# Rorisis/Co-Occ

Measured on AMD Instinct MI355X. Metric: samples/sec (6-cam frame + sweep -> occ+render), 200x200x16 grid, higher is better.
Workload: dtype f32 (split-f16 products, fp32 accumulate)

## Files before the change

### co_occ_amd/_lib.py

```python
import ctypes
import os
import threading
import time

import torch

_HERE = os.path.dirname(os.path.abspath(__file__))
LIB_PATH = os.path.join(_HERE, "libcoocc_hip.so")

c_int, c_float, c_void_p, c_size_t, c_int64 = (ctypes.c_int, ctypes.c_float, ctypes.c_void_p,
                                               ctypes.c_size_t, ctypes.c_int64)


class ConvDesc(ctypes.Structure):
    _fields_ = [(n, c_void_p) for n in ("in_", "w", "out", "scale", "bias", "res", "gather", "out_rows", "ws")] + \
               [("ws_floats", c_int64)] + \
               [(n, c_int) for n in ("M", "Cin", "Cout", "taps", "in_stride", "out_stride", "res_stride",
                                     "B", "Xi", "Yi", "Zi", "Xo", "Yo", "Zo", "ksize", "stride", "pad",
                                     "relu", "res_mode", "splitk", "tile_hint", "kx", "ky", "kz", "px", "py", "pz",
                                     "wgroup_rows", "mfma_dtype")] + [("alpha", ctypes.c_float), ("M_dev", c_void_p), ("gather_stride", c_int), ("out16", c_void_p), ("out16_stride", c_int), ("out_h2", c_int),
                                                                   ("out_h2_twin", c_void_p), ("tile_sem", c_void_p), ("tile_sem_ints", c_int),
                                                                  ("alpha_dev", c_void_p), ("sx", c_int), ("sy", c_int), ("sz", c_int)]


class SearchDesc(ctypes.Structure):
    _fields_ = [("cat4", c_void_p), ("pts", c_void_p), ("pts_rows", c_int), ("pts_stride", c_int)] + \
               [(n, c_int) for n in ("C", "X", "Y", "Z", "K", "fps_num", "max_cluster")] + \
               [("radius", ctypes.c_float), ("dist_thresh", ctypes.c_float), ("offsets", c_void_p), ("noff", c_int)] + \
               [(n, c_void_p) for n in ("lin", "counts", "near_img", "near_pts", "rows", "rows_p", "ws")] + \
               [("ws_bytes", ctypes.c_size_t), ("counts_host", c_void_p)]


P, I, F, Z, L = c_void_p, c_int, c_float, c_size_t, c_int64
SIGNATURES = {
    "coocc_last_error": (ctypes.c_char_p, []),
    "coocc_abi_version": (I, []),
    "coocc_device_cu_count": (I, [P]),
    "coocc_stream_create_cu_mask": (I, [P, I, P]),
    "coocc_stream_destroy": (I, [P]),
    "coocc_event_create": (I, [I, P]),
    "coocc_event_destroy": (I, [P]),
    "coocc_event_record": (I, [P, P]),
    "coocc_stream_wait_event": (I, [P, P]),
    "coocc_event_synchronize": (I, [P]),
    "coocc_event_query": (I, [P]),
    "coocc_event_elapsed_ms": (I, [P, P, P]),
    "coocc_ncdhw_to_ndhwc": (I, [P, P, I, I, I, I, I, P]),
    "coocc_rows_to_bf16": (I, [P, I, L, I, P, P]),
    "coocc_rows_to_h2": (I, [P, I, L, I, F, P, P]),
    "coocc_rows_to_h2_ex": (I, [P, I, L, I, F, P, P, P]),
    "coocc_rows_to_h2_gather": (I, [P, I, P, L, P, I, F, P, P]),
    "coocc_rows_to_f16": (I, [P, I, L, I, P, P]),
    "coocc_wino_input_h2": (I, [P, I, I, I, I, I, I, I, P, I, L, F, P]),
    "coocc_wino_input_h2_ex": (I, [P, I, I, I, I, I, I, I, P, I, L, F, P, P]),
    "coocc_ndhwc_to_ncdhw": (I, [P, P, I, I, I, I, I, P]),
    "coocc_fuser_prepare": (I, [P, P, P, P, P, I, I, I, P]),
    "coocc_fuser_prepare_rows": (I, [P, I, I, P, I, I, P, P, P, I, I, I, P]),
    "coocc_compact_flags": (I, [P, I, P, P, P, Z, P]),
    "coocc_compact_flags_ex": (I, [P, I, P, P, P, P, Z, P]),
    "coocc_lin_to_coords": (I, [P, I, I, I, I, P, P, P]),
    "coocc_furthest_point_sampling": (I, [I, I, I, P, P, P, P]),
    "coocc_fps_voxels_ws": (Z, [I, I, I]),
    "coocc_fps_voxels": (I, [P, I, I, I, I, I, P, P, Z, P]),
    "coocc_fps_voxels_pair": (I, [P, I, P, P, P, I, P, P, Z, I, I, I, I, P]),
    "coocc_ball_query": (I, [I, I, I, F, F, I, P, P, P, P]),
    "coocc_knn_topk": (I, [I, I, I, P, P, P, P, P]),
    "coocc_voxel_index_map": (I, [P, I, I, P, P]),
    "coocc_voxel_index_map_dev": (I, [P, I, P, I, P, P]),
    "coocc_fine_sample_voxel_dev": (I, [P, I, I, I, I, P, I, P, I, P, P, P, I, P]),
    "coocc_fine_sample_img_dev": (I, [P, I, I, I, I, P, P, L, P, P, I, I, P]),
    "coocc_fine_mlp_pre_dev": (I, [P, I, P, I, L, P, I, P, P, P, F, P, P, P, P, F, P, P, I, P, P]),
    "coocc_fine_fused": (I, [P, I, I, I, P, I, I, I, P, P, I, P, I, P, P, P, P, F, P, P, P, P, F, P, P, I, P, P, P]),
    "coocc_fine2_pack": (I, [P, P, I, P, P, P, P, P, P, P, P, P, P]),
    "coocc_fine2_h2": (I, [P, I, I, I, I, P, I, I, I, P, P, I, P, P, P, P, F, F, I, P, P, P, P]),
    "coocc_fine_sample_img_lin": (I, [P, I, I, I, I, P, P, I, I, I, P, P, I, I, P]),
    "coocc_scatter_fine_dev": (I, [P, L, P, I, I, I, P, P, I, I, I, F, P]),
    "coocc_scatter_fine_grouped": (I, [P, I, I, P, I, P, I, I, I, I, P, F, P, P]),
    "coocc_ball_query_voxels": (I, [I, F, F, I, I, I, I, P, P, P, P, P]),
    "coocc_knn_topk_voxels": (I, [I, I, I, I, I, I, P, P, P, P, I, P, P, P, P, P]),
    "coocc_knn_assign": (I, [I, I, I, I, F, P, P, P, P, P, P]),
    "coocc_knn_threshold": (I, [I, F, P, P, P, P]),
    "coocc_index_rows_i32": (I, [P, I, P, I, P, P]),
    "coocc_conv_pack_weights": (L, [P, I, I, I, I, P]),
    "coocc_conv_fwd": (I, [ctypes.POINTER(ConvDesc), P]),
    "coocc_fuser_search_ws": (Z, [ctypes.POINTER(SearchDesc)]),
    "coocc_fuser_search": (I, [ctypes.POINTER(SearchDesc), P, P]),
    "coocc_upsample_add_trilinear": (I, [P, P, I, I, I, I, I, I, I, I, P]),
    "coocc_upsample_add_trilinear_ex": (I, [P, P, I, I, I, I, I, I, I, I, P, P]),
    "coocc_occhead_mix": (I, [P, P, I, P, P, I, I, P]),
    "coocc_occhead_mix_ex": (I, [P, P, I, P, P, I, I, P, P]),
    "coocc_argmax_flags": (I, [P, I, I, I, I, P, P]),
    "coocc_fine_sample_voxel": (I, [P, I, I, I, I, P, I, I, P, P, P, I, P]),
    "coocc_fine_sample_img": (I, [P, I, I, I, I, P, P, L, P, I, I, P]),
    "coocc_fine_mlp_pre": (I, [P, I, P, I, L, P, P, P, F, P, P, P, P, F, P, P, I, P, P]),
    "coocc_fine_mlp": (I, [P, I, P, I, L, P, P, P, P, F, P, P, P, P, F, P, P, I, P, P]),
    "coocc_groupnorm_rows": (I, [P, L, I, I, I, P, P, F, I, P]),
    "coocc_groupnorm_nhwc": (I, [P, I, I, I, I, P, P, F, I, P]),
    "coocc_scatter_fine": (I, [P, L, I, I, P, P, I, I, I, F, P]),
    "coocc_camera_mats": (I, [P, P, P, P, P, P, I, I, I, I, P, P]),
    "coocc_get_geometry": (I, [P, P, P, P, I, I, I, I, P, P]),
    "coocc_bev_pool_forward": (I, [P, P, P, P, I, I, I, I, I, I, I, P, P]),
    "coocc_bev_pool_backward": (I, [P, P, P, P, I, I, I, I, I, I, I, P, P]),
    "coocc_voxel_pool_ws": (Z, [I, I]),
    "coocc_voxel_pool": (I, [P, P, I, I, I, P, I, I, I, I, P, I, P, Z, I, P]),
    "coocc_lift_splat": (I, [P, P, P, I, I, I, I, I, I, P, I, I, I, I, P, I, P, Z, I, P]),
    "coocc_lift_splat_cams": (I, [P, P, P, P, P, P, I, I, I, I, I, I, P, I, I, I, I, P, I, P, Z, I, P]),
    "coocc_lift_splat_reuse": (I, [P, P, I, I, I, I, I, I, I, I, I, P, I, P, Z, P]),
    "coocc_bev_pool_coords": (I, [P, P, I, I, I, I, I, I, P, I, P, Z, I, P]),
    "coocc_render_nearest": (I, [P, I, I, I, P, P, I, I, I, I, P, I, P, P]),
    "coocc_render_nearest_cams": (I, [P, I, I, I, P, P, P, P, P, I, I, I, I, P, I, P, P]),
    "coocc_render_activate_table": (I, [P, I, P]),
    "coocc_upsample_maps": (I, [P, I, I, I, I, P, P, P]),
    "coocc_volume_sampling": (I, [P, I, I, I, I, P, I, P, P, P, P]),
    "coocc_raw2outputs": (I, [P, P, I, I, I, F, F, P, P, P, P]),
    "coocc_render_losses": (I, [P, P, P, P, L, I, P, P, Z, P]),
    "coocc_conv_pack_weights_dev": (L, [P, I, I, I, I, P, P]),
    "coocc_wino_pack_weights_dev": (L, [P, I, I, I, I, P, P]),
    "coocc_wino_pack_weights_h2_dev": (L, [P, I, I, I, I, P, P]),
    "coocc_conv_pack_weights_h2_dev": (L, [P, I, I, I, I, P, P]),
    "coocc_wino_gradout": (I, [P, I, I, I, I, I, I, I, P, L, P]),
    "coocc_wino_ztap_table": (I, [L, I, P, P]),
    "coocc_wino_wgrad": (I, [P, P, L, I, I, I, I, P, P, I, P, L, P]),
    "coocc_rows_to_kh2": (I, [P, I, L, L, I, F, P, P, P]),
    "coocc_wino_operand_kh2": (I, [I, P, I, I, I, I, I, I, I, P, L, F, P, P]),
    "coocc_conv_wgrad_h2": (I, [P, P, L, I, I, F, P, P, I, P, L, P]),
    "coocc_wino_wgrad_h2": (I, [P, P, L, I, I, I, I, F, P, P, I, P, L, P]),
    "coocc_conv_tap_table": (I, [I, I, I, I, I, I, I, I, I, I, I, P, P]),
    "coocc_conv_epilogue_bwd": (I, [P, I, P, I, P, I, I, I, P, I, P, I, I, P, I, P, L, P]),
    "coocc_conv_epilogue_bwd_ex": (I, [P, I, P, I, P, I, I, I, P, I, P, I, I, P, I, P, L, P, P, F, P]),
    "coocc_conv_wgrad": (I, [P, I, I, P, I, P, I, I, I, I, P, I, P, L, P]),
    "coocc_conv_wgrad_h2t": (I, [P, I, I, P, I, P, I, I, I, I, P, P, I, P, L, P]),
    "coocc_gather_rows": (I, [P, I, P, I, I, P, I, P]),
    "coocc_scatter_add_rows": (I, [P, I, P, I, I, P, I, P]),
    "coocc_voxel_pool_bwd": (I, [P, I, P, I, I, I, P, I, I, I, I, P, P]),
    "coocc_lift_splat_bwd": (I, [P, I, P, P, P, I, I, I, I, I, I, P, I, I, I, I, P, P, P]),
    "coocc_render_nearest_bwd": (I, [P, I, I, I, P, P, I, I, I, I, P, P, P, P]),
    "coocc_upsample_maps_bwd": (I, [P, P, I, I, I, I, P, P]),
    "coocc_render_losses_bwd": (I, [P, P, P, P, L, I, P, P, P, P, P]),
    "coocc_upsample_trilinear_bwd": (I, [P, P, I, I, I, I, I, I, I, I, I, P]),
    "coocc_wino_input": (I, [P, I, I, I, I, I, I, I, P, L, P]),
    "coocc_wino_input_strided": (I, [P, I, I, I, I, I, I, I, P, I, L, P]),
    "coocc_sparse_tap_sum": (I, [P, P, I, I, I, I, I, P, P, I, I, P]),
    "coocc_wino_output": (I, [P, L, I, I, I, I, I, I, P, I, P, P, P, I, I, P]),
    "coocc_wino_output_ex": (I, [P, L, I, I, I, I, I, I, P, I, P, P, P, I, I, P, P]),
    "coocc_h2_overflow": (I, [I]),
    "coocc_device_fault": (I, [I]),
    "coocc_render_heads_h2": (I, [P, I, I, I, P, P, P, P, P, P, I, P, P, P, I, P]),
    "coocc_head_pred_h2": (I, [P, I, I, P, P, P, P, P, I, I, P, P, I, P, I, I, P, P]),
    "coocc_head_soft_h2": (I, [P, I, I, P, P, P, P, P, I, P, P, I, P, I, P]),
    "coocc_projection_params": (I, [P, P, P, P, P, P, I, P, P, P]),
    "coocc_occhead_mix_bwd": (I, [P, P, I, P, P, P, P, I, I, P]),
    "coocc_fine_sample_voxel_bwd": (I, [P, I, I, I, I, I, P, L, P, P, P]),
    "coocc_groupnorm_rows_bwd": (I, [P, P, P, L, I, I, I, P, F, I, P, P, P, P]),
    "coocc_fine_sample_img_bwd": (I, [P, I, I, I, I, I, P, P, L, P, P]),
    "coocc_groupnorm_nhwc_bwd": (I, [P, P, P, I, I, I, I, P, F, I, P, P, P, P]),
    "coocc_voxelize_ws": (Z, [I]),
    "coocc_voxelize_hard": (I, [P, I, I, P, P, I, I, P, P, P, P, P, Z, P]),
    "coocc_vfe_mean": (I, [P, P, I, I, I, I, P, I, P]),
    "coocc_sparse_index_map": (I, [P, I, I, I, I, P, P]),
    "coocc_sparse_conv_table": (I, [P, I, I, I, I, I, I, I, P, P, P]),
    "coocc_sparse_down_flags": (I, [P, I, I, I, I, I, I, I, P, P]),
    "coocc_sparse_conv_table3": (I, [P, I, I, I, I, I, I, I, I, I, I, I, I, I, P, P, P]),
    "coocc_sparse_down_flags3": (I, [P, I, I, I, I, I, I, I, I, I, I, I, I, I, I, I, I, P, P]),
    "coocc_sparse_lin_to_coors": (I, [P, I, I, I, I, P, P, P]),
    "coocc_bn_stats": (I, [P, I, I, I, P, P, P, Z, P]),
    "coocc_bn_apply": (I, [P, I, I, P, P, P, P, F, P, I, P, P]),
    "coocc_bn_backward": (I, [P, P, P, I, I, P, P, P, F, I, P, P, P, P, P, Z, P]),
    "coocc_bn_backward_sums": (I, [P, P, P, I, I, P, P, F, I, P, P, P, Z, P]),
    "coocc_bn_backward_dx": (I, [P, P, P, I, I, P, P, P, F, I, P, P, ctypes.c_double, P, P, P]),
    "coocc_predict_labels": (I, [P, L, L, L, L, I, I, I, I, I, I, I, P, P]),
    "coocc_eval_semantic": (I, [P, L, L, L, L, I, I, I, I, P, P, I, I, I, I, I, P, P]),
    "coocc_fpn_sum": (I, [P, P, I, I, I, I, I, I, P, I, P, P]),
    "coocc_zyx_to_rows": (I, [P, P, I, I, I, I, I, I, I, P]),
    "coocc_conv_tap_table3": (I, [I] * 17 + [P, P]),
    "coocc_fpn_sum_bwd": (I, [P, I, P, P, I, I, I, I, I, I, P]),
    "coocc_lidarseg_points": (I, [P, L, L, L, L, I, I, I, I, P, L, L, I, I, P, I, I, P, P, I, P, P]),
    "coocc_render_eval_stats": (L, [P, P, P, P, I, I, I, P, P, Z, P]),
    "coocc_render_panels": (I, [P, P, P, P, I, I, I, P, P]),
    "coocc_render_eval_ssim": (L, [P, P, I, I, I, ctypes.c_double, P, P, Z, P]),
    "coocc_sparse_dgrad_table3": (I, [P] + [I] * 16 + [P, P, P, P]),
    "coocc_bn_apply_ex": (I, [P, I, I, P, P, P, P, F, P, I, P, P, P]),
    "coocc_pool_labels": (I, [P, I, I, I, I, I, I, I, P, P]),
    "coocc_occ_loss_ws": (Z, [L, I]),
    "coocc_occ_loss_fwd": (I, [P, L, I, I, P, P, I, I, I, P, P, I, P, P, P, P, Z, P]),
    "coocc_occ_loss_bwd": (I, [P, L, I, I, P, P, I, P, P, P, P, I, P]),
    "coocc_depth_labels": (I, [P, I, I, I, I, F, F, I, P, P, P]),
    "coocc_depth_bce_ws": (Z, [L, I]),
    "coocc_depth_bce": (I, [P, P, I, I, I, I, F, P, P, P, Z, P]),
    "coocc_depth_bce_bwd": (I, [P, P, I, I, I, I, F, P, P, P, P]),
    "coocc_nbr_table2d": (I, [I, I, I, I, P, P]),
    "coocc_dcn_cols": (I, [P, I, P, I, I, I, I, I, I, I, I, P, P]),
    "coocc_se_gate2": (I, [P, I, I, I, I, P, P, P, P, P]),
    "coocc_cam_mean_ws": (Z, [I, I, I]),
    "coocc_cam_mean": (I, [P, I, I, I, I, P, P, Z, P]),
    "coocc_cam_bias_relu": (I, [P, I, I, I, I, P, I, P]),
    "coocc_dcn_cols_bwd": (I, [P, I, P, I, I, I, I, I, I, I, I, P, P, P, P]),
    "coocc_se_gate2_bwd_ws": (Z, [I, I, I]),
    "coocc_se_gate2_bwd": (I, [P, I, I, I, I, P, P, P, P, P, P, P, P, Z, P]),
    "coocc_cam_sum": (I, [P, I, I, I, I, P, P, Z, P]),
    "coocc_cam_add": (I, [P, P, I, I, I, P, F, P]),
    "coocc_dropout_rows": (I, [P, P, L, I, F, P, P]),
    "coocc_img_stem": (I, [P, I, I, I, P, P, P, I, I, I, P, I, P, P]),
    "coocc_maxpool2d_rows": (I, [P, I, I, I, I, I, P, I, P, P]),
    "coocc_maxpool2d_rows_bwd": (I, [P, I, P, I, I, I, I, I, P, I, P]),
    "coocc_img_stem_wgrad_ws": (Z, [I, I, I]),
    "coocc_img_stem_wgrad": (I, [P, I, I, I, P, I, I, P, P, Z, P]),
    "coocc_optim_chunk": (I, []),
    "coocc_optim_sumsq": (I, [P, P, I, P, I, P, P]),
    "coocc_optim_clip_coef": (I, [P, I, F, P, P, P, P]),
    "coocc_optim_adamw": (I, [P, P, I, P, I, P, I, P]),
    "coocc_optim_scale": (I, [P, P, I, P, I, P, P]),
    "coocc_optim_pack": (I, [P, P, I, P, I, P, L, I, P]),
    "coocc_optim_unpack": (I, [P, P, I, P, I, P, L, P]),
    "coocc_optim_flag_check": (I, [P, I, P, I, P, P]),
    "coocc_frames_to_imgs": (I, [P, P, I, I, I, P, P, P, L, I, I, P, P, P]),
    "coocc_points_to_depth_maps": (I, [P, L, I, P, I, I, I, P, P]),
    "coocc_occ_scatter_labels": (I, [P, L, I, I, I, I, P, P, P]),
    "coocc_occ_rows_to_voxels": (I, [P, L, P, P, I, I, I, P, P, P, P]),
    "coocc_occ_points_to_voxels": (I, [P, L, I, P, P, P, P, I, I, I, I, P, P, P, P]),
    "coocc_occ_vote_ws": (Z, [L]),
    "coocc_occ_vote_labels": (I, [P, P, L, L, I, I, P, P, Z, P]),
    "coocc_occ_visible_rows": (I, [P, L, P, I, I, I, P, P, P]),
    "coocc_occ_cloud_aabb": (I, [P, L, I, P, P, P, P]),
    "coocc_sweeps_merge_ws": (Z, [L]),
    "coocc_sweeps_merge": (I, [P, L, I, P, P, I, P, I, F, P, L, P, P, Z, P]),
}

_lib = None


class KernelTimer:

    def __init__(self):
        self.enabled = False
        self.only = None
        self.records = []

    class _Region:
        def __init__(self, owner, tag, work):
            self.o, self.tag, self.work = owner, tag, work

        def __enter__(self):
            lvl = int(self.o.enabled)
            self.on = lvl >= 2 or (lvl == 1 and self.work > 0 and (self.o.only is None or self.tag.startswith(self.o.only)))
            if self.on:
                self.s = torch.cuda.Event(enable_timing=True)
                self.e = torch.cuda.Event(enable_timing=True)
                self.s.record()
            return self

        def __exit__(self, *a):
            if self.on:
                self.e.record()
                self.o.records.append((self.tag, self.work, self.s, self.e))
            return False

    def region(self, tag, work=0.0):
        return KernelTimer._Region(self, tag, work)

    def summary(self):
        out = {}
        for tag, work, s, e in self.records:
            d = out.setdefault(tag, dict(launches=0, ms=0.0, work=0.0))
            d["launches"] += 1
            d["ms"] += s.elapsed_time(e)
            d["work"] += work
        return out

    def reset(self):
        self.records = []


TIMER = KernelTimer()



def load():
    global _lib
    if _lib is not None:
        return _lib
    if not os.path.exists(LIB_PATH):
        raise ImportError(
            "co_occ_amd: %s is missing -- build it with `python -c 'import __graft_entry__ as g; g.build()'` "
            "(hipcc --offload-arch=gfx950).  There is no CPU fallback." % LIB_PATH)
    lib = ctypes.CDLL(LIB_PATH)
    for name, (res, args) in SIGNATURES.items():
        fn = getattr(lib, name)
        fn.restype, fn.argtypes = res, args
    if os.environ.get("COOCC_FPS_THREADS"):
        lib.coocc_fps_voxels_set_threads(int(os.environ["COOCC_FPS_THREADS"]))
    _lib = lib
    return lib


class CooccError(RuntimeError):
    code = None


class CooccArgError(CooccError):
    """COOCC_EINVAL / COOCC_ENOMEM: the library REFUSED the call (an argument or shape an entry point does not take, a
    workspace that is too small) before launching anything -- nothing ran, the caller may take another route."""


class CooccRangeError(CooccError):
    """The split-f16 engine's range guard fired (``core.check_h2_overflow``): kernels ran and their result is not trustworthy.
    Never a reason to fall back silently."""


def check(rc):
    if rc != 0:
        cls = CooccArgError if rc in (-1, -3) else CooccError
        e = cls("libcoocc_hip: %s (code %d)" % (load().coocc_last_error().decode(), rc))
        e.code = rc
        raise e


def _device_of(args):
    for a in args:
        t = getattr(a, "_keep", None)
        if t is not None:
            return t.device
    return None


_fns = {}


def call(name, *args):
    fn = _fns.get(name)
    if fn is None:
        fn = _fns[name] = getattr(load(), name)
    dev = _device_of(args)
    if dev is not None and dev.index != torch.cuda.current_device():
        with torch.cuda.device(dev):
            with TIMER.region(name):
                check(fn(*args, stream(dev)))
        return
    if not TIMER.enabled:
        rc = fn(*args, stream(dev))
        if rc:
            check(rc)
        return
    with TIMER.region(name):
        check(fn(*args, stream(dev)))


def conv_fwd(desc, device):
    fn = load().coocc_conv_fwd
    if device.index != torch.cuda.current_device():
        with torch.cuda.device(device):
            check(fn(ctypes.byref(desc), stream(device)))
    else:
        check(fn(ctypes.byref(desc), stream(device)))


_raw_stream = getattr(torch._C, "_cuda_getCurrentRawStream", None)


def stream(device=None):
    if _raw_stream is not None:
        idx = device.index if device is not None and device.index is not None else torch.cuda.current_device()
        return c_void_p(_raw_stream(idx))
    return c_void_p(torch.cuda.current_stream(device).cuda_stream)


class DevPtr(ctypes.c_void_p):
    """c_void_p that keeps its tensor alive until the foreign call has been issued, so that
    temporaries such as ``ptr(x.contiguous())`` cannot be recycled by the caching allocator
    while later arguments of the same call are still being built."""


def require_gpu(what, name=None):
    if isinstance(what, torch.Tensor):
        if not what.is_cuda:
            raise CooccError("co_occ_amd ops run on the GPU only; %s a %s tensor (no CPU fallback)" % ("%s is" % name if name else "got", what.device))
    elif torch.device(what).type != "cuda":
        raise CooccError("co_occ_amd ops run on the GPU only; got device %s (no CPU fallback)" % (what,))


def ptr(t, dtype=None, strided=False, offset=0):
    if t is None:
        return c_void_p(0)
    if not t.is_cuda:
        require_gpu(t)
    if dtype is not None and t.dtype != dtype:
        raise CooccError("expected %s, got %s" % (dtype, t.dtype))
    if not strided and not t.is_contiguous():
        raise CooccError("tensor must be contiguous")
    p = DevPtr(t.data_ptr() + offset * t.element_size())
    p._keep = t
    return p


_blocked = threading.local()


def host_read(t):
    t0 = time.perf_counter()
    v = t.tolist()
    _blocked.s = getattr(_blocked, "s", 0.0) + time.perf_counter() - t0
    return v


def blocked_seconds():
    return getattr(_blocked, "s", 0.0)


def host_f32(vals):
    return (c_float * len(vals))(*[float(v) for v in vals])


def host_i32(vals):
    return (c_int * len(vals))(*[int(v) for v in vals])
```

### co_occ_amd/csrc/knn.hip

```cpp
#include "common.h"

typedef unsigned long long u64;

__device__ __forceinline__ u64 shfl_xor_u64(u64 v, int m) {
  unsigned lo = (unsigned)v, hi = (unsigned)(v >> 32);
  lo = __shfl_xor(lo, m);
  hi = __shfl_xor(hi, m);
  return ((u64)hi << 32) | lo;
}
template <int CTRL>
__device__ __forceinline__ u64 dpp_u64(u64 v) {
  int lo = (int)(unsigned)v, hi = (int)(unsigned)(v >> 32);
  lo = __builtin_amdgcn_update_dpp(lo, lo, CTRL, 0xF, 0xF, false);
  hi = __builtin_amdgcn_update_dpp(hi, hi, CTRL, 0xF, 0xF, false);
  return ((u64)(unsigned)hi << 32) | (unsigned)lo;
}
__device__ __forceinline__ u64 readlane_u64(u64 v, int l) {
  unsigned lo = __builtin_amdgcn_readlane((int)(unsigned)v, l);
  unsigned hi = __builtin_amdgcn_readlane((int)(unsigned)(v >> 32), l);
  return ((u64)hi << 32) | lo;
}
#define U64MAX(a, b) ((a) > (b) ? (a) : (b))
#define U64MIN(a, b) ((a) < (b) ? (a) : (b))
__device__ __forceinline__ u64 wave_max_u64(u64 v) {
  u64 o;
  o = dpp_u64<0xB1>(v); v = U64MAX(v, o);
  o = dpp_u64<0x4E>(v); v = U64MAX(v, o);
  o = dpp_u64<0x141>(v); v = U64MAX(v, o);
  o = dpp_u64<0x140>(v); v = U64MAX(v, o);
  u64 a = readlane_u64(v, 0), b = readlane_u64(v, 16), c = readlane_u64(v, 32), d = readlane_u64(v, 48);
  a = U64MAX(a, b); c = U64MAX(c, d);
  return U64MAX(a, c);
}
__device__ __forceinline__ u64 wave_min_u64(u64 v) {
  u64 o;
  o = dpp_u64<0xB1>(v); v = U64MIN(v, o);
  o = dpp_u64<0x4E>(v); v = U64MIN(v, o);
  o = dpp_u64<0x141>(v); v = U64MIN(v, o);
  o = dpp_u64<0x140>(v); v = U64MIN(v, o);
  u64 a = readlane_u64(v, 0), b = readlane_u64(v, 16), c = readlane_u64(v, 32), d = readlane_u64(v, 48);
  a = U64MIN(a, b); c = U64MIN(c, d);
  return U64MIN(a, c);
}

#define FPS_THREADS 1024
#define FPS_KBITS 22

__device__ __forceinline__ unsigned fps_tiebreak(int k, int L, unsigned blockmask) {
  unsigned r = L ? (__brev((unsigned)k & blockmask) >> (32 - L)) : 0u;
  return (r << FPS_KBITS) | (unsigned)k;
}

template <int PPT>
__global__ __launch_bounds__(FPS_THREADS) void k_fps_f32(int n, int m, const float* __restrict__ pts_all,
                                                          float* __restrict__ temp_all,
                                                          int32_t* __restrict__ idx_all, int L) {
  __shared__ u64 wbest[2][FPS_THREADS / 64];
  const int tid = threadIdx.x;
  const float* pts = pts_all + (size_t)blockIdx.x * n * 3;
  float* temp = temp_all + (size_t)blockIdx.x * n;
  int32_t* idx = idx_all + (size_t)blockIdx.x * m;
  const unsigned blockmask = (1u << L) - 1u;

  float px[PPT], py[PPT], pz[PPT], pt[PPT];
  unsigned ntb[PPT];
#pragma unroll
  for (int i = 0; i < PPT; ++i) {
    int k = tid + i * FPS_THREADS;
    bool v = k < n;
    px[i] = v ? pts[k * 3 + 0] : 0.f;
    py[i] = v ? pts[k * 3 + 1] : 0.f;
    pz[i] = v ? pts[k * 3 + 2] : 0.f;
    pt[i] = v ? 1e10f : 0.f;
    ntb[i] = v ? ~fps_tiebreak(k, L, blockmask) : 0u;
  }
  for (int k = tid + PPT * FPS_THREADS; k < n; k += FPS_THREADS) temp[k] = 1e10f;

  int old = 0;
  if (tid == 0) idx[0] = 0;
  for (int j = 1; j < m; ++j) {
    const float x1 = pts[old * 3 + 0], y1 = pts[old * 3 + 1], z1 = pts[old * 3 + 2];
    u64 best = 0;
#pragma unroll
    for (int i = 0; i < PPT; ++i) {
      float d = sqdist3(x1, y1, z1, px[i], py[i], pz[i]);
      float t = fminf(d, pt[i]);
      pt[i] = t;
      u64 key = ((u64)__float_as_uint(t) << 32) | (u64)ntb[i];
      best = key > best ? key : best;
    }
#pragma unroll 2
    for (int k = tid + PPT * FPS_THREADS; k < n; k += FPS_THREADS) {
      float d = sqdist3(x1, y1, z1, pts[k * 3 + 0], pts[k * 3 + 1], pts[k * 3 + 2]);
      float t = fminf(d, temp[k]);
      temp[k] = t;
      u64 key = ((u64)__float_as_uint(t) << 32) | (u64)(~fps_tiebreak(k, L, blockmask));
      best = key > best ? key : best;
    }
    best = wave_max_u64(best);
    if ((tid & 63) == 0) wbest[j & 1][tid >> 6] = best;
    __syncthreads();
    u64 b = wbest[j & 1][tid & 15];
#pragma unroll
    for (int mm = 8; mm > 0; mm >>= 1) {
      u64 o = shfl_xor_u64(b, mm);
      b = o > b ? o : b;
    }
    old = (int)((~(unsigned)b) & ((1u << FPS_KBITS) - 1u));
    if (tid == 0) idx[j] = old;
  }
}

extern "C" int coocc_furthest_point_sampling(int b, int n, int m, const float* points, float* temp,
                                             int32_t* idx, void* stream) {
  COOCC_CHECK_ARG(points && temp && idx && b > 0 && n > 0 && m >= 0, "fps: bad args");
  COOCC_CHECK_ARG(n < (1 << FPS_KBITS), "fps: n must be < 2^22");
  if (m == 0) return COOCC_OK;
  int L = 0;
  while ((2 << L) <= n && L < 10) ++L;
  if (n <= 8 * FPS_THREADS)
    hipLaunchKernelGGL(k_fps_f32<8>, dim3(b), dim3(FPS_THREADS), 0, as_stream(stream), n, m, points, temp, idx, L);
  else
    hipLaunchKernelGGL(k_fps_f32<10>, dim3(b), dim3(FPS_THREADS), 0, as_stream(stream), n, m, points, temp, idx, L);
  COOCC_LAUNCH_CHECK("k_fps_f32");
  return COOCC_OK;
}

#define FT_X 4
#define FT_Y 4
#define FT_Z 8
#define FT_P 128

struct FpsCell { int temp; int r; };

__global__ __launch_bounds__(256) void k_fpsv_scatter(const int32_t* __restrict__ lin, int n, int Y, int Z, int NBY,
                                                       int NBZ, int L, int q, int tinit, FpsCell* __restrict__ cell) {
  int k = blockIdx.x * blockDim.x + threadIdx.x;
  if (k >= n) return;
  int l = lin[k];
  int z = l % Z; l /= Z;
  int y = l % Y; int x = l / Y;
  int b = ((x / FT_X) * NBY + y / FT_Y) * NBZ + z / FT_Z;
  int p = ((x % FT_X) * FT_Y + (y % FT_Y)) * FT_Z + (z % FT_Z);
  unsigned rev = L ? (__brev((unsigned)k & ((1u << L) - 1u)) >> (32 - L)) : 0u;
  cell[(size_t)b * FT_P + p] = FpsCell{tinit, (int)(rev * (unsigned)q + ((unsigned)k >> L))};
}

__device__ __forceinline__ void lds_barrier() { asm volatile("s_waitcnt lgkmcnt(0)\n\ts_barrier" ::: "memory"); }

template <int CTRL>
__device__ __forceinline__ unsigned dpp_u32(unsigned v) {
  return (unsigned)__builtin_amdgcn_update_dpp((int)v, (int)v, CTRL, 0xF, 0xF, false);
}
__device__ __forceinline__ unsigned wave_max_key(unsigned v) {
  v = max(v, dpp_u32<0xB1>(v));
  v = max(v, dpp_u32<0x4E>(v));
  v = max(v, dpp_u32<0x141>(v));
  v = max(v, dpp_u32<0x140>(v));
  unsigned a = __builtin_amdgcn_readlane((int)v, 0), b = __builtin_amdgcn_readlane((int)v, 16);
  unsigned c = __builtin_amdgcn_readlane((int)v, 32), d = __builtin_amdgcn_readlane((int)v, 48);
  return max(max(a, b), max(c, d));
}
__device__ __forceinline__ u64 wave_max_key(u64 v) { return wave_max_u64(v); }
__device__ __forceinline__ unsigned row_max_key(unsigned v) {
  v = max(v, dpp_u32<0xB1>(v));
  v = max(v, dpp_u32<0x4E>(v));
  v = max(v, dpp_u32<0x141>(v));
  v = max(v, dpp_u32<0x140>(v));
  return v;
}
__device__ __forceinline__ u64 row_max_key(u64 v) {
  u64 o;
  o = dpp_u64<0xB1>(v); v = U64MAX(v, o);
  o = dpp_u64<0x4E>(v); v = U64MAX(v, o);
  o = dpp_u64<0x141>(v); v = U64MAX(v, o);
  o = dpp_u64<0x140>(v); v = U64MAX(v, o);
  return v;
}
__device__ __forceinline__ unsigned first_lane_key(unsigned v) { return (unsigned)__builtin_amdgcn_readfirstlane((int)v); }
__device__ __forceinline__ u64 first_lane_key(u64 v) {
  return ((u64)(unsigned)__builtin_amdgcn_readfirstlane((int)(v >> 32)) << 32) | (unsigned)__builtin_amdgcn_readfirstlane((int)(unsigned)v);
}

template <int THREADS, int FPS_RMAX, typename KT>
__global__ __launch_bounds__(THREADS) void k_fps_voxels(int n, int m, int Y, int Z, int NBY, int NBZ, int NB,
                                                         const int32_t* __restrict__ lin, FpsCell* __restrict__ cell,
                                                         int32_t* __restrict__ idx, int L, int q, int RB, long long* dbg) {
  constexpr int NW = THREADS / 64;
  __builtin_amdgcn_s_setprio(3);
  __shared__ KT wbest[2][NW];
  __shared__ int wloc[2][NW];
  const int tid = threadIdx.x, lane = tid & 63, wave = tid >> 6;
  const KT rmask = (KT)(((KT)1 << RB) - 1);
  const int tmax = sizeof(KT) == 4 ? (int)((1u << (32 - RB)) - 1u) : 0x7FFFFFFF;
  long long tA = 0, tM = 0, tB = 0, tT = 0, nd = 0;

  KT key[FPS_RMAX];
  int org[FPS_RMAX];
  int pos[FPS_RMAX];
#pragma unroll
  for (int r = 0; r < FPS_RMAX; ++r) {
    const int b = (lane + 64 * r) * NW + wave;
    key[r] = 0; pos[r] = 0; org[r] = 0;
    if (b < NB) {
      int bz = b % NBZ; int qq = b / NBZ;
      org[r] = ((qq / NBY) * FT_X) | (((qq % NBY) * FT_Y) << 10) | ((bz * FT_Z) << 20);
    }
  }
#pragma unroll
  for (int r = 0; r < FPS_RMAX; ++r) {
    for (int src = 0; src < 64; ++src) {
      const int b = (src + 64 * r) * NW + wave;
      if (b >= NB) break;
      KT best = 0;
      int bp = 0;
#pragma unroll
      for (int h = 0; h < 2; ++h) {
        int rr = cell[(size_t)b * FT_P + lane + 64 * h].r;
        KT kk = rr >= 0 ? (KT)(((KT)tmax << RB) | (rmask - (KT)rr)) : (KT)0;
        if (kk > best) { best = kk; bp = lane + 64 * h; }
      }
      KT wb = wave_max_key(best);
      u64 own = __ballot(best == wb);
      int wp = __builtin_amdgcn_readlane(bp, (int)__ffsll((long long)own) - 1);
      if (lane == src) { key[r] = wb; pos[r] = wp; }
    }
  }
  if (tid == 0) idx[0] = 0;
  int sx, sy, sz;
  {
    int l = lin[0];
    sz = l % Z; l /= Z;
    sy = l % Y; sx = l / Y;
  }

  auto refresh = [&](FpsCell* cp, const FpsCell& c0_, const FpsCell& c1_, int o, KT& best, int& bp) {
    const int x0 = o & 1023, y0 = (o >> 10) & 1023, z0 = o >> 20;
    best = 0; bp = 0;
#pragma unroll
    for (int h = 0; h < 2; ++h) {
      const FpsCell c = h ? c1_ : c0_;
      const int p = lane + 64 * h;
      if (c.r >= 0) {
        int ex = x0 + (p >> 5) - sx, ey = y0 + ((p >> 3) & 3) - sy, ez = z0 + (p & 7) - sz;
        int t = min(__mul24(ex, ex) + __mul24(ey, ey) + __mul24(ez, ez), c.temp);
        cp[p].temp = t;
        KT kk = (KT)(((KT)t << RB) | (rmask - (KT)c.r));
        if (kk > best) { best = kk; bp = p; }
      }
    }
  };

  for (int j = 1; j < m; ++j) {
    long long c0 = dbg ? clock64() : 0;
#pragma unroll
    for (int r = 0; r < FPS_RMAX; ++r) {
      if (r * 64 * NW >= NB) break;
      bool d = false;
      if (key[r]) {
        int x0 = org[r] & 1023, y0 = (org[r] >> 10) & 1023, z0 = org[r] >> 20;
        int dx = max(max(x0 - sx, sx - (x0 + FT_X - 1)), 0);
        int dy = max(max(y0 - sy, sy - (y0 + FT_Y - 1)), 0);
        int dz = max(max(z0 - sz, sz - (z0 + FT_Z - 1)), 0);
        d = (__mul24(dx, dx) + __mul24(dy, dy) + __mul24(dz, dz)) < (int)(key[r] >> RB);
      }
      u64 bal = __ballot(d);
      nd += __popcll(bal);
      while (bal) {
        const int s0 = (int)__ffsll((long long)bal) - 1;
        bal &= bal - 1;
        const bool two = bal != 0;
        const int s1 = two ? (int)__ffsll((long long)bal) - 1 : s0;
        bal &= bal - 1;
        FpsCell* cp0 = cell + (size_t)((s0 + 64 * r) * NW + wave) * FT_P;
        FpsCell* cp1 = cell + (size_t)((s1 + 64 * r) * NW + wave) * FT_P;
        const FpsCell a0 = cp0[lane], a1 = cp0[lane + 64];
        FpsCell b0 = a0, b1 = a1;
        if (two) { b0 = cp1[lane]; b1 = cp1[lane + 64]; }
        KT best0, best1 = 0;
        int bp0, bp1 = 0;
        refresh(cp0, a0, a1, __builtin_amdgcn_readlane(org[r], s0), best0, bp0);
        if (two) refresh(cp1, b0, b1, __builtin_amdgcn_readlane(org[r], s1), best1, bp1);
        const KT wb0 = wave_max_key(best0);
        const KT wb1 = two ? wave_max_key(best1) : (KT)0;
        const int wp0 = __builtin_amdgcn_readlane(bp0, (int)__ffsll((long long)__ballot(best0 == wb0)) - 1);
        if (lane == s0) { key[r] = wb0; pos[r] = wp0; }
        if (two) {
          const int wp1 = __builtin_amdgcn_readlane(bp1, (int)__ffsll((long long)__ballot(best1 == wb1)) - 1);
          if (lane == s1) { key[r] = wb1; pos[r] = wp1; }
        }
      }
    }
    long long c1 = dbg ? clock64() : 0;
    KT best = 0;
    int bo = 0, bpz = 0;
#pragma unroll
    for (int r = 0; r < FPS_RMAX; ++r) {
      if (key[r] > best) { best = key[r]; bo = org[r]; bpz = pos[r]; }
    }
    const int loc = bo + (bpz >> 5) + (((bpz >> 3) & 3) << 10) + ((bpz & 7) << 20);
    KT wb = wave_max_key(best);
    if (best == wb && wb) { wbest[j & 1][wave] = wb; wloc[j & 1][wave] = loc; }
    if (!wb && lane == 0) wbest[j & 1][wave] = 0;
    long long c2 = dbg ? clock64() : 0;
    lds_barrier();
    long long c3 = dbg ? clock64() : 0;
    KT g;
    int gl;
    if constexpr (NW <= 16) {
      const int li = lane & 15;
      const KT mine = li < NW ? wbest[j & 1][li] : (KT)0;
      const int ml = li < NW ? wloc[j & 1][li] : 0;
      g = first_lane_key(row_max_key(mine));
      const u64 own = __ballot(mine == g) & 0xFFFFull;
      gl = __builtin_amdgcn_readlane(ml, (int)__ffsll((long long)own) - 1);
    } else {
      g = wbest[j & 1][0];
      int gw = 0;
#pragma unroll
      for (int w = 1; w < NW; ++w) {
        KT o = wbest[j & 1][w];
        if (o > g) { g = o; gw = w; }
      }
      gl = wloc[j & 1][gw];
    }
    sx = gl & 1023; sy = (gl >> 10) & 1023; sz = gl >> 20;
    if (tid == 0) {
      const unsigned rr = (unsigned)(rmask - (g & rmask));
      const unsigned hi = rr / (unsigned)q, lo = rr - hi * (unsigned)q;
      const unsigned rev = L ? (__brev(hi) >> (32 - L)) : 0u;
      idx[j] = (int)((lo << L) | rev);
    }
    if (dbg) { long long c4 = clock64(); tA += c1 - c0; tM += c2 - c1; tB += c3 - c2; tT += c4 - c3; }
  }
  if (dbg && lane == 0) {
    long long* o = dbg + wave * 8;
    o[0] = tA; o[1] = tM; o[2] = tB; o[3] = tT; o[4] = 0; o[5] = nd;
  }
}

#define FPSR_SLOTS 40
struct FpsRegProblem { const int32_t* lin; const FpsCell* cell; int32_t* idx; int n, L, q, RB; };
struct FpsRegArgs { FpsRegProblem p[2]; int m, Y, Z, NBY, NBZ, NB; long long* dbg; };

__global__ __launch_bounds__(1024) void k_fps_voxels_reg(FpsRegArgs a) {
  constexpr int NW = 16;
  __builtin_amdgcn_s_setprio(3);
  __shared__ unsigned wbest[2][NW];
  __shared__ int wloc[2][NW];
  const FpsRegProblem pr = a.p[blockIdx.x];
  const int tid = threadIdx.x, lane = tid & 63, wave = __builtin_amdgcn_readfirstlane(tid >> 6);
  const int RB = pr.RB, Y = a.Y, Z = a.Z, NB = a.NB, m = a.m;
  const unsigned rmask = (1u << RB) - 1u;
  const unsigned tmax = (1u << (32 - RB)) - 1u;
  long long* dbg = a.dbg;
  long long tA = 0, tM = 0, tB = 0, tT = 0, nd = 0;

  typedef unsigned u32x32 __attribute__((ext_vector_type(32)));
  typedef unsigned u32x8 __attribute__((ext_vector_type(8)));
  u32x32 ca0, ca1;
  u32x8 cb0, cb1;
  unsigned key = 0;
  int org = 0, pos = 0;
  {
    const int b = lane * NW + wave;
    if (lane < FPSR_SLOTS && b < NB) {
      int bz = b % a.NBZ; int qq = b / a.NBZ;
      org = ((qq / a.NBY) * FT_X) | (((qq % a.NBY) * FT_Y) << 10) | ((bz * FT_Z) << 20);
    }
  }
#pragma unroll
  for (int i = 0; i < FPSR_SLOTS; ++i) {
    const int b = i * NW + wave;
    unsigned k0 = 0, k1 = 0;
    if (b < NB) {
      const int r0 = pr.cell[(size_t)b * FT_P + lane].r, r1 = pr.cell[(size_t)b * FT_P + lane + 64].r;
      k0 = r0 >= 0 ? ((tmax << RB) | (rmask - (unsigned)r0)) : 0u;
      k1 = r1 >= 0 ? ((tmax << RB) | (rmask - (unsigned)r1)) : 0u;
      const unsigned best = max(k0, k1);
      const int bp = k1 > k0 ? lane + 64 : lane;
      const unsigned wb = wave_max_key(best);
      const u64 own = __ballot(best == wb);
      const int wp = __builtin_amdgcn_readlane(bp, (int)__ffsll((long long)own) - 1);
      if (lane == i) { key = wb; pos = wp; }
    }
    if (i < 32) { ca0[i] = k0; ca1[i] = k1; }
    else { cb0[i - 32] = k0; cb1[i - 32] = k1; }
  }
  if (tid == 0) pr.idx[0] = 0;
  int sx, sy, sz;
  {
    int l = pr.lin[0];
    sz = l % Z; l /= Z;
    sy = l % Y; sx = l / Y;
  }

  for (int j = 1; j < m; ++j) {
    long long c0 = dbg ? clock64() : 0;
    bool d = false;
    if (key) {
      const int x0 = org & 1023, y0 = (org >> 10) & 1023, z0 = org >> 20;
      const int dx = max(max(x0 - sx, sx - (x0 + FT_X - 1)), 0);
      const int dy = max(max(y0 - sy, sy - (y0 + FT_Y - 1)), 0);
      const int dz = max(max(z0 - sz, sz - (z0 + FT_Z - 1)), 0);
      d = (unsigned)(__mul24(dx, dx) + __mul24(dy, dy) + __mul24(dz, dz)) < (key >> RB);
    }
    u64 bal = __ballot(d);
    nd += __popcll(bal);
    const int exb = (lane >> 5) - sx, eyb = ((lane >> 3) & 3) - sy, ezb = (lane & 7) - sz;
    while (bal) {
      const int s0 = __builtin_amdgcn_readfirstlane((int)__ffsll((long long)bal) - 1);
      bal &= bal - 1;
      const int o = __builtin_amdgcn_readlane(org, s0);
      const int ex = (o & 1023) + exb, ey = ((o >> 10) & 1023) + eyb, ez = (o >> 20) + ezb;
      const int yz = __mul24(ey, ey) + __mul24(ez, ez);
      const unsigned d0 = (unsigned)(__mul24(ex, ex) + yz), d1 = (unsigned)(__mul24(ex + 2, ex + 2) + yz);
      unsigned k0, k1;
      if (s0 < 32) { k0 = ca0[s0]; k1 = ca1[s0]; }
      else { k0 = cb0[s0 - 32]; k1 = cb1[s0 - 32]; }
      if (k0) k0 = (min(d0, k0 >> RB) << RB) | (k0 & rmask);
      if (k1) k1 = (min(d1, k1 >> RB) << RB) | (k1 & rmask);
      if (s0 < 32) { ca0[s0] = k0; ca1[s0] = k1; }
      else { cb0[s0 - 32] = k0; cb1[s0 - 32] = k1; }
      const unsigned best = max(k0, k1);
      const int bp = k1 > k0 ? lane + 64 : lane;
      const unsigned wb = wave_max_key(best);
      const int wp = __builtin_amdgcn_readlane(bp, (int)__ffsll((long long)__ballot(best == wb)) - 1);
      if (lane == s0) { key = wb; pos = wp; }
    }
    long long c1 = dbg ? clock64() : 0;
    const int loc = org + (pos >> 5) + (((pos >> 3) & 3) << 10) + ((pos & 7) << 20);
    const unsigned wb = wave_max_key(key);
    if (key == wb && wb) { wbest[j & 1][wave] = wb; wloc[j & 1][wave] = loc; }
    if (!wb && lane == 0) wbest[j & 1][wave] = 0;
    long long c2 = dbg ? clock64() : 0;
    lds_barrier();
    long long c3 = dbg ? clock64() : 0;
    const int li = lane & 15;
    const unsigned mine = wbest[j & 1][li];
    const int ml = wloc[j & 1][li];
    unsigned v = mine;
    v = max(v, dpp_u32<0xB1>(v));
    v = max(v, dpp_u32<0x4E>(v));
    v = max(v, dpp_u32<0x141>(v));
    v = max(v, dpp_u32<0x140>(v));
    const unsigned g = (unsigned)__builtin_amdgcn_readfirstlane((int)v);
    const u64 own = __ballot(mine == g) & 0xFFFFull;
    const int gl = __builtin_amdgcn_readlane(ml, (int)__ffsll((long long)own) - 1);
    sx = gl & 1023; sy = (gl >> 10) & 1023; sz = gl >> 20;
    if (tid == 0) pr.idx[j] = (int)(g & rmask);
    if (dbg) { long long c4 = clock64(); tA += c1 - c0; tM += c2 - c1; tB += c3 - c2; tT += c4 - c3; }
  }
  __syncthreads();
  for (int j = 1 + tid; j < m; j += 1024) {
    const unsigned rr = rmask - (unsigned)pr.idx[j];
    const unsigned hi = rr / (unsigned)pr.q, lo = rr - hi * (unsigned)pr.q;
    const unsigned rev = pr.L ? (__brev(hi) >> (32 - pr.L)) : 0u;
    pr.idx[j] = (int)((lo << pr.L) | rev);
  }
  if (dbg && lane == 0 && blockIdx.x == 0) {
    long long* o = dbg + wave * 8;
    o[0] = tA; o[1] = tM; o[2] = tB; o[3] = tT; o[4] = 0; o[5] = nd;
  }
}

extern "C" size_t coocc_fps_voxels_ws(int X, int Y, int Z) {
  size_t nb = (size_t)((X + FT_X - 1) / FT_X) * ((Y + FT_Y - 1) / FT_Y) * ((Z + FT_Z - 1) / FT_Z);
  return nb * FT_P * sizeof(FpsCell);
}

static int g_fps_threads = 1024;
static long long* g_fps_dbg = nullptr;
extern "C" void coocc_fps_voxels_set_debug(long long* p) { g_fps_dbg = p; }
extern "C" void coocc_fps_voxels_set_threads(int t) { g_fps_threads = t; }

struct FpsPrep { int NBX, NBY, NBZ, L, q, RB, tinit, threads, R; long long NB; bool key32; };

static int fps_prepare(const int32_t* lin, int n, int X, int Y, int Z, int m, const int32_t* idx, void* ws, size_t ws_bytes,
                       hipStream_t s, FpsPrep* o) {
  COOCC_CHECK_ARG(lin && idx && ws && n > 0 && m >= 0 && X > 0 && Y > 0 && Z > 0, "fps_voxels: bad args");
  COOCC_CHECK_ARG(n < (1 << FPS_KBITS), "fps_voxels: n must be < 2^22");
  COOCC_CHECK_ARG(X <= 1020 && Y <= 1020 && Z <= 1016, "fps_voxels: grid dims must fit 10-bit packed coordinates");
  o->NBX = (X + FT_X - 1) / FT_X; o->NBY = (Y + FT_Y - 1) / FT_Y; o->NBZ = (Z + FT_Z - 1) / FT_Z;
  o->NB = (long long)o->NBX * o->NBY * o->NBZ;
  int threads = g_fps_threads;
  while (o->NB > 8ll * threads && threads < 1024) threads *= 2;
  COOCC_CHECK_ARG(o->NB <= 8ll * threads, "fps_voxels: grid has too many buckets (use coocc_furthest_point_sampling)");
  if (ws_bytes < coocc_fps_voxels_ws(X, Y, Z)) return coocc_set_error(COOCC_ENOMEM, "fps_voxels: workspace too small");
  o->threads = threads;
  o->R = (int)((o->NB + threads - 1) / threads);
  int L = 0;
  while ((2 << L) <= n && L < 10) ++L;
  const int q = (n + (1 << L) - 1) >> L;
  int RB = L;
  while ((1ll << RB) <= ((long long)q << L)) ++RB;
  const long long d2max = (long long)(X - 1) * (X - 1) + (long long)(Y - 1) * (Y - 1) + (long long)(Z - 1) * (Z - 1);
  o->key32 = RB < 31 && d2max + 1 < (1ll << (32 - RB)) - 1;
  o->tinit = o->key32 ? (int)((1u << (32 - RB)) - 1u) : 0x7FFFFFFF;
  o->L = L; o->q = q; o->RB = RB;
  if (m == 0) return COOCC_OK;
  FpsCell* cell = (FpsCell*)ws;
  COOCC_HIP(hipMemsetAsync(cell, 0xFF, sizeof(FpsCell) * (size_t)o->NB * FT_P, s));
  hipLaunchKernelGGL(k_fpsv_scatter, dim3(cdiv(n, 256)), dim3(256), 0, s, lin, n, Y, Z, o->NBY, o->NBZ, L, q, o->tinit, cell);
  COOCC_LAUNCH_CHECK("k_fpsv_scatter");
  return COOCC_OK;
}

static int g_fps_reg = -1;
static bool fps_reg_ok(const FpsPrep& o) {
  if (g_fps_reg < 0) g_fps_reg = getenv("COOCC_FPS_REG") ? atoi(getenv("COOCC_FPS_REG")) : 1;
  return g_fps_reg && o.key32 && o.NB <= (long long)FPSR_SLOTS * 16;
}

extern "C" int coocc_fps_voxels(const int32_t* lin, int n, int X, int Y, int Z, int m, int32_t* idx, void* ws,
                                size_t ws_bytes, void* stream) {
  hipStream_t s = as_stream(stream);
  FpsPrep o;
  int rc = fps_prepare(lin, n, X, Y, Z, m, idx, ws, ws_bytes, s, &o);
  if (rc != COOCC_OK || m == 0) return rc;
  FpsCell* cell = (FpsCell*)ws;
  const int NBY = o.NBY, NBZ = o.NBZ, L = o.L, q = o.q, RB = o.RB, R = o.R, threads = o.threads;
  const long long NB = o.NB;
  const bool key32 = o.key32;
  if (fps_reg_ok(o)) {
    FpsRegArgs a = {};
    a.p[0] = FpsRegProblem{lin, cell, idx, n, L, q, RB};
    a.m = m; a.Y = Y; a.Z = Z; a.NBY = NBY; a.NBZ = NBZ; a.NB = (int)NB; a.dbg = g_fps_dbg;
    hipLaunchKernelGGL(k_fps_voxels_reg, dim3(1), dim3(1024), 0, s, a);
    COOCC_LAUNCH_CHECK("k_fps_voxels_reg");
    return COOCC_OK;
  }
#define FPS_LAUNCH(T, RM, KT) \
  hipLaunchKernelGGL((k_fps_voxels<T, RM, KT>), dim3(1), dim3(T), 0, s, n, m, Y, Z, NBY, NBZ, (int)NB, lin, cell, idx, L, q, \
                     key32 ? RB : 32, g_fps_dbg)
#define FPS_PICK_R(T, KT)                     \
  do {                                        \
    if (R <= 2) FPS_LAUNCH(T, 2, KT);         \
    else if (R <= 3) FPS_LAUNCH(T, 3, KT);    \
    else if (R <= 4) FPS_LAUNCH(T, 4, KT);    \
    else if (R <= 5) FPS_LAUNCH(T, 5, KT);    \
    else if (R <= 6) FPS_LAUNCH(T, 6, KT);    \
    else FPS_LAUNCH(T, 8, KT);                \
  } while (0)
#define FPS_PICK(T)                           \
  do {                                        \
    if (key32) FPS_PICK_R(T, unsigned);       \
    else FPS_PICK_R(T, u64);                  \
  } while (0)
  if (threads == 256) FPS_PICK(256);
  else if (threads == 512) FPS_PICK(512);
  else FPS_PICK(1024);
  COOCC_LAUNCH_CHECK("k_fps_voxels");
  return COOCC_OK;
}

extern "C" int coocc_fps_voxels_pair(const int32_t* lin0, int n0, int32_t* idx0, void* ws0, const int32_t* lin1, int n1, int32_t* idx1,
                                     void* ws1, size_t ws_bytes_each, int X, int Y, int Z, int m, void* stream) {
  COOCC_CHECK_ARG(X > 0 && Y > 0 && Z > 0 && n0 > 0 && n1 > 0, "fps_voxels_pair: bad args");
  {
    const long long NB = (long long)((X + FT_X - 1) / FT_X) * ((Y + FT_Y - 1) / FT_Y) * ((Z + FT_Z - 1) / FT_Z);
    if (NB > (long long)FPSR_SLOTS * 16) return 2;
    const long long d2max = (long long)(X - 1) * (X - 1) + (long long)(Y - 1) * (Y - 1) + (long long)(Z - 1) * (Z - 1);
    for (int n : {n0, n1}) {
      int L = 0;
      while ((2 << L) <= n && L < 10) ++L;
      const int q = (n + (1 << L) - 1) >> L;
      int RB = L;
      while ((1ll << RB) <= ((long long)q << L)) ++RB;
      if (!(RB < 31 && d2max + 1 < (1ll << (32 - RB)) - 1)) return 2;
    }
    if (g_fps_reg < 0) g_fps_reg = getenv("COOCC_FPS_REG") ? atoi(getenv("COOCC_FPS_REG")) : 1;
    if (!g_fps_reg) return 2;
  }
  hipStream_t s = as_stream(stream);
  FpsPrep o0, o1;
  int rc = fps_prepare(lin0, n0, X, Y, Z, m, idx0, ws0, ws_bytes_each, s, &o0);
  if (rc != COOCC_OK) return rc;
  rc = fps_prepare(lin1, n1, X, Y, Z, m, idx1, ws1, ws_bytes_each, s, &o1);
  if (rc != COOCC_OK || m == 0) return rc;
  FpsRegArgs a = {};
  a.p[0] = FpsRegProblem{lin0, (const FpsCell*)ws0, idx0, n0, o0.L, o0.q, o0.RB};
  a.p[1] = FpsRegProblem{lin1, (const FpsCell*)ws1, idx1, n1, o1.L, o1.q, o1.RB};
  a.m = m; a.Y = Y; a.Z = Z; a.NBY = o0.NBY; a.NBZ = o0.NBZ; a.NB = (int)o0.NB; a.dbg = g_fps_dbg;
  hipLaunchKernelGGL(k_fps_voxels_reg, dim3(2), dim3(1024), 0, s, a);
  COOCC_LAUNCH_CHECK("k_fps_voxels_reg");
  return COOCC_OK;
}

__global__ __launch_bounds__(256) void k_ball_query(int n, int m, float min_r2, float max_r2, int nsample,
                                                     const float* __restrict__ new_xyz_all,
                                                     const float* __restrict__ xyz_all,
                                                     int32_t* __restrict__ idx_all) {
  const int lane = threadIdx.x & 63;
  const int c = blockIdx.x * 4 + (threadIdx.x >> 6);
  if (c >= m) return;
  const float* new_xyz = new_xyz_all + ((size_t)blockIdx.y * m + c) * 3;
  const float* xyz = xyz_all + (size_t)blockIdx.y * n * 3;
  int32_t* idx = idx_all + ((size_t)blockIdx.y * m + c) * nsample;
  const float cx = new_xyz[0], cy = new_xyz[1], cz = new_xyz[2];
  int cnt = 0, first = 0;
  for (int base = 0; base < n && cnt < nsample; base += 64) {
    int k = base + lane;
    bool hit = false;
    if (k < n) {
      float d2 = sqdist3(xyz[k * 3 + 0], xyz[k * 3 + 1], xyz[k * 3 + 2], cx, cy, cz);
      hit = (d2 == 0.f) || (d2 >= min_r2 && d2 < max_r2);
    }
    u64 bal = __ballot(hit);
    if (bal) {
      if (cnt == 0) first = base + (int)__ffsll((long long)bal) - 1;
      int slot = cnt + __popcll(bal & ((1ull << lane) - 1ull));
      if (hit && slot < nsample) idx[slot] = k;
      cnt += __popcll(bal);
    }
  }
  if (cnt > nsample) cnt = nsample;
  for (int l = cnt + lane; l < nsample; l += 64) idx[l] = first;
}

extern "C" int coocc_ball_query(int b, int n, int m, float min_radius, float max_radius, int nsample,
                                const float* new_xyz, const float* xyz, int32_t* idx, void* stream) {
  COOCC_CHECK_ARG(new_xyz && xyz && idx && b > 0 && n > 0 && m > 0 && nsample > 0, "ball_query: bad args");
  dim3 grid(cdiv(m, 4), b);
  hipLaunchKernelGGL(k_ball_query, grid, dim3(256), 0, as_stream(stream), n, m, min_radius * min_radius,
                     max_radius * max_radius, nsample, new_xyz, xyz, idx);
  COOCC_LAUNCH_CHECK("k_ball_query");
  return COOCC_OK;
}

template <int K>
__global__ __launch_bounds__(256) void k_knn_topk(int nq, int nk, const float* __restrict__ q,
                                                   const float* __restrict__ key, float* __restrict__ val,
                                                   int32_t* __restrict__ idx) {
  const int lane = threadIdx.x & 63;
  const int r = blockIdx.x * 4 + (threadIdx.x >> 6);
  if (r >= nq) return;
  const float qx = q[r * 3 + 0], qy = q[r * 3 + 1], qz = q[r * 3 + 2];
  u64 best[K];
#pragma unroll
  for (int j = 0; j < K; ++j) best[j] = ~0ull;
  for (int k = lane; k < nk; k += 64) {
    float d2 = sqdist3(qx, qy, qz, key[k * 3 + 0], key[k * 3 + 1], key[k * 3 + 2]);
    u64 kk = ((u64)__float_as_uint(d2) << 32) | (unsigned)k;
    if (kk < best[K - 1]) {
      best[K - 1] = kk;
#pragma unroll
      for (int j = K - 1; j > 0; --j) {
        if (best[j] < best[j - 1]) { u64 t = best[j]; best[j] = best[j - 1]; best[j - 1] = t; }
      }
    }
  }
#pragma unroll
  for (int o = 0; o < K; ++o) {
    u64 mn = wave_min_u64(best[0]);
    if (best[0] == mn) {
#pragma unroll
      for (int j = 0; j < K - 1; ++j) best[j] = best[j + 1];
      best[K - 1] = ~0ull;
    }
    if (lane == 0) {
      val[(size_t)r * K + o] = (float)__dsqrt_rn((double)__uint_as_float((unsigned)(mn >> 32)));
      idx[(size_t)r * K + o] = (int32_t)(unsigned)mn;
    }
  }
}

extern "C" int coocc_knn_topk(int nq, int nk, int K, const float* q, const float* key, float* val,
                              int32_t* idx, void* stream) {
  COOCC_CHECK_ARG(q && key && val && idx && nq > 0 && nk > 0, "knn_topk: bad args");
  COOCC_CHECK_ARG(K >= 1 && K <= 8 && K <= nk, "knn_topk: need 1 <= K <= min(8, nk)");
  dim3 grid(cdiv(nq, 4)), block(256);
  hipStream_t s = as_stream(stream);
  switch (K) {
    case 1: hipLaunchKernelGGL(k_knn_topk<1>, grid, block, 0, s, nq, nk, q, key, val, idx); break;
    case 2: hipLaunchKernelGGL(k_knn_topk<2>, grid, block, 0, s, nq, nk, q, key, val, idx); break;
    case 3: hipLaunchKernelGGL(k_knn_topk<3>, grid, block, 0, s, nq, nk, q, key, val, idx); break;
    case 4: hipLaunchKernelGGL(k_knn_topk<4>, grid, block, 0, s, nq, nk, q, key, val, idx); break;
    case 5: hipLaunchKernelGGL(k_knn_topk<5>, grid, block, 0, s, nq, nk, q, key, val, idx); break;
    case 6: hipLaunchKernelGGL(k_knn_topk<6>, grid, block, 0, s, nq, nk, q, key, val, idx); break;
    case 7: hipLaunchKernelGGL(k_knn_topk<7>, grid, block, 0, s, nq, nk, q, key, val, idx); break;
    default: hipLaunchKernelGGL(k_knn_topk<8>, grid, block, 0, s, nq, nk, q, key, val, idx); break;
  }
  COOCC_LAUNCH_CHECK("k_knn_topk");
  return COOCC_OK;
}

__global__ __launch_bounds__(256) void k_index_map_scatter(const int32_t* __restrict__ lin, int n, int32_t* __restrict__ map,
                                                            const int32_t* __restrict__ n_dev) {
  if (n_dev) n = min(n, *n_dev);
  int i = blockIdx.x * blockDim.x + threadIdx.x;
  if (i < n) map[lin[i]] = i;
}

__global__ __launch_bounds__(256) void k_fill_i32(int32_t* __restrict__ p, int n, int32_t v) {
  const int i = blockIdx.x * blockDim.x + threadIdx.x;
  if (i < n) p[i] = v;
}

extern "C" int coocc_voxel_index_map_dev(const int32_t* lin, int n_cap, const int32_t* n_dev, int nvox, int32_t* map, void* stream) {
  COOCC_CHECK_ARG(map && nvox > 0 && n_cap > 0 && lin && n_dev, "voxel_index_map_dev: bad args");
  static const bool fill_kernel = !(getenv("COOCC_MAP_MEMSET") && atoi(getenv("COOCC_MAP_MEMSET")) == 1);
  if (fill_kernel) hipLaunchKernelGGL(k_fill_i32, dim3(cdiv(nvox, 256)), dim3(256), 0, as_stream(stream), map, nvox, -1);
  else COOCC_HIP(hipMemsetAsync(map, 0xFF, (size_t)nvox * 4, as_stream(stream)));
  hipLaunchKernelGGL(k_index_map_scatter, dim3(cdiv(n_cap, 256)), dim3(256), 0, as_stream(stream), lin, n_cap, map, n_dev);
  COOCC_LAUNCH_CHECK("k_index_map_scatter");
  return COOCC_OK;
}

extern "C" int coocc_voxel_index_map(const int32_t* lin, int n, int nvox, int32_t* map, void* stream) {
  COOCC_CHECK_ARG(map && nvox > 0 && n >= 0 && (lin || n == 0), "voxel_index_map: bad args");
  COOCC_HIP(hipMemsetAsync(map, 0xFF, (size_t)nvox * 4, as_stream(stream)));
  if (n) {
    hipLaunchKernelGGL(k_index_map_scatter, dim3(cdiv(n, 256)), dim3(256), 0, as_stream(stream), lin, n, map, (const int32_t*)nullptr);
    COOCC_LAUNCH_CHECK("k_index_map_scatter");
  }
  return COOCC_OK;
}

__global__ __launch_bounds__(256) void k_ball_query_vox(int m, float min_r2, float max_r2, int R, int nsample, int X, int Y, int Z,
                                                         const int32_t* __restrict__ centre_ord, const int32_t* __restrict__ lin_q,
                                                         const int32_t* __restrict__ map_q, int32_t* __restrict__ idx_all) {
  const int lane = threadIdx.x & 63;
  const int c = blockIdx.x * 4 + (threadIdx.x >> 6);
  if (c >= m) return;
  int32_t* idx = idx_all + (size_t)c * nsample;
  const int v0 = lin_q[centre_ord[c]];
  const int cz = v0 % Z, cy = (v0 / Z) % Y, cx = v0 / (Z * Y);
  const int x0 = max(cx - R, 0), x1 = min(cx + R, X - 1);
  const int y0 = max(cy - R, 0), y1 = min(cy + R, Y - 1);
  const int z0 = max(cz - R, 0), z1 = min(cz + R, Z - 1);
  const int wy = y1 - y0 + 1, wz = z1 - z0 + 1;
  const int total = (x1 - x0 + 1) * wy * wz;
  int cnt = 0, first = 0;
  for (int base = 0; base < total && cnt < nsample; base += 64) {
    const int t = base + lane;
    bool hit = false;
    int ord = -1;
    if (t < total) {
      const int iz = z0 + t % wz, r = t / wz;
      const int iy = y0 + r % wy, ix = x0 + r / wy;
      ord = map_q[(ix * Y + iy) * Z + iz];
      const float d2 = sqdist3((float)ix, (float)iy, (float)iz, (float)cx, (float)cy, (float)cz);
      hit = ord >= 0 && ((d2 == 0.f) || (d2 >= min_r2 && d2 < max_r2));
    }
    const u64 bal = __ballot(hit);
    if (bal) {
      if (cnt == 0) first = __shfl(ord, (int)__ffsll((long long)bal) - 1);
      const int slot = cnt + __popcll(bal & ((1ull << lane) - 1ull));
      if (hit && slot < nsample) idx[slot] = ord;
      cnt += __popcll(bal);
    }
  }
  if (cnt > nsample) cnt = nsample;
  for (int l = cnt + lane; l < nsample; l += 64) idx[l] = first;
}

extern "C" int coocc_ball_query_voxels(int m, float min_radius, float max_radius, int nsample, int X, int Y, int Z,
                                       const int32_t* centre_ord, const int32_t* lin_q, const int32_t* map_q, int32_t* idx,
                                       void* stream) {
  COOCC_CHECK_ARG(m > 0 && nsample > 0 && X > 0 && Y > 0 && Z > 0 && centre_ord && lin_q && map_q && idx, "ball_query_voxels: bad args");
  COOCC_CHECK_ARG(max_radius >= 0.f && max_radius < 4096.f, "ball_query_voxels: bad radius");
  const float max_r2 = max_radius * max_radius;
  int R = (int)ceilf(max_radius);
  while (R > 0 && (float)(R * R) >= max_r2) --R;
  hipLaunchKernelGGL(k_ball_query_vox, dim3(cdiv(m, 4)), dim3(256), 0, as_stream(stream), m, min_radius * min_radius, max_r2, R,
                     nsample, X, Y, Z, centre_ord, lin_q, map_q, idx);
  COOCC_LAUNCH_CHECK("k_ball_query_vox");
  return COOCC_OK;
}

template <int K>
__global__ __launch_bounds__(256) void k_knn_topk_vox(int nq, int X, int Y, int Z, const int32_t* __restrict__ rep_ord,
                                                       const int32_t* __restrict__ lin_q, const int32_t* __restrict__ map_k,
                                                       const uint32_t* __restrict__ offsets, int noff, float* __restrict__ val,
                                                       int32_t* __restrict__ idx) {
  const int lane = threadIdx.x & 63;
  const int r = blockIdx.x * 4 + (threadIdx.x >> 6);
  if (r >= nq) return;
  const int v0 = lin_q[rep_ord[r]];
  const int cz = v0 % Z, cy = (v0 / Z) % Y, cx = v0 / (Z * Y);
  int found = 0;
  for (int base = 0; base < noff && found < K; base += 64) {
    const int t = base + lane;
    int ord = -1;
    float d2 = 0.f;
    if (t < noff) {
      const uint32_t o = offsets[t];
      const int dx = (int)(o & 255u) - 128, dy = (int)((o >> 8) & 255u) - 128, dz = (int)((o >> 16) & 255u) - 128;
      const int ix = cx + dx, iy = cy + dy, iz = cz + dz;
      if ((unsigned)ix < (unsigned)X && (unsigned)iy < (unsigned)Y && (unsigned)iz < (unsigned)Z) {
        ord = map_k[(ix * Y + iy) * Z + iz];
        d2 = sqdist3((float)cx, (float)cy, (float)cz, (float)ix, (float)iy, (float)iz);
      }
    }
    const u64 bal = __ballot(ord >= 0);
    const int p = found + __popcll(bal & ((1ull << lane) - 1ull));
    if (ord >= 0 && p < K) {
      val[(size_t)r * K + p] = (float)__dsqrt_rn((double)d2);
      idx[(size_t)r * K + p] = ord;
    }
    found += __popcll(bal);
  }
  if (found < K && lane == 0) idx[(size_t)r * K] = -2;
}

template <int K>
__global__ __launch_bounds__(256) void k_knn_topk_unresolved(int nq, int nk, const float* __restrict__ q,
                                                              const float* __restrict__ key, float* __restrict__ val,
                                                              int32_t* __restrict__ idx) {
  const int lane = threadIdx.x & 63;
  const int r = blockIdx.x * 4 + (threadIdx.x >> 6);
  if (r >= nq || idx[(size_t)r * K] != -2) return;
  const float qx = q[r * 3 + 0], qy = q[r * 3 + 1], qz = q[r * 3 + 2];
  u64 best[K];
#pragma unroll
  for (int j = 0; j < K; ++j) best[j] = ~0ull;
  for (int k = lane; k < nk; k += 64) {
    float d2 = sqdist3(qx, qy, qz, key[k * 3 + 0], key[k * 3 + 1], key[k * 3 + 2]);
    u64 kk = ((u64)__float_as_uint(d2) << 32) | (unsigned)k;
    if (kk < best[K - 1]) {
      best[K - 1] = kk;
#pragma unroll
      for (int j = K - 1; j > 0; --j) {
        if (best[j] < best[j - 1]) { u64 t = best[j]; best[j] = best[j - 1]; best[j - 1] = t; }
      }
    }
  }
#pragma unroll
  for (int o = 0; o < K; ++o) {
    u64 mn = wave_min_u64(best[0]);
    if (best[0] == mn) {
#pragma unroll
      for (int j = 0; j < K - 1; ++j) best[j] = best[j + 1];
      best[K - 1] = ~0ull;
    }
    if (lane == 0) {
      val[(size_t)r * K + o] = (float)__dsqrt_rn((double)__uint_as_float((unsigned)(mn >> 32)));
      idx[(size_t)r * K + o] = (int32_t)(unsigned)mn;
    }
  }
}

template <int K>
static void launch_topk_vox(int nq, int nk, int X, int Y, int Z, const int32_t* rep_ord, const int32_t* lin_q, const int32_t* map_k,
                            const uint32_t* offsets, int noff, const float* q, const float* key, float* val, int32_t* idx,
                            hipStream_t s) {
  hipLaunchKernelGGL(k_knn_topk_vox<K>, dim3(cdiv(nq, 4)), dim3(256), 0, s, nq, X, Y, Z, rep_ord, lin_q, map_k, offsets, noff, val, idx);
  hipLaunchKernelGGL(k_knn_topk_unresolved<K>, dim3(cdiv(nq, 4)), dim3(256), 0, s, nq, nk, q, key, val, idx);
}

extern "C" int coocc_knn_topk_voxels(int nq, int nk, int K, int X, int Y, int Z, const int32_t* rep_ord, const int32_t* lin_q,
                                     const int32_t* map_k, const uint32_t* offsets, int noff, const float* q, const float* key,
                                     float* val, int32_t* idx, void* stream) {
  COOCC_CHECK_ARG(nq > 0 && nk > 0 && X > 0 && Y > 0 && Z > 0 && rep_ord && lin_q && map_k && offsets && noff > 0 && q && key &&
                      val && idx, "knn_topk_voxels: bad args");
  COOCC_CHECK_ARG(K >= 1 && K <= 8 && K <= nk, "knn_topk_voxels: need 1 <= K <= min(8, nk)");
  hipStream_t s = as_stream(stream);
  switch (K) {
    case 1: launch_topk_vox<1>(nq, nk, X, Y, Z, rep_ord, lin_q, map_k, offsets, noff, q, key, val, idx, s); break;
    case 2: launch_topk_vox<2>(nq, nk, X, Y, Z, rep_ord, lin_q, map_k, offsets, noff, q, key, val, idx, s); break;
    case 3: launch_topk_vox<3>(nq, nk, X, Y, Z, rep_ord, lin_q, map_k, offsets, noff, q, key, val, idx, s); break;
    case 4: launch_topk_vox<4>(nq, nk, X, Y, Z, rep_ord, lin_q, map_k, offsets, noff, q, key, val, idx, s); break;
    case 5: launch_topk_vox<5>(nq, nk, X, Y, Z, rep_ord, lin_q, map_k, offsets, noff, q, key, val, idx, s); break;
    case 6: launch_topk_vox<6>(nq, nk, X, Y, Z, rep_ord, lin_q, map_k, offsets, noff, q, key, val, idx, s); break;
    case 7: launch_topk_vox<7>(nq, nk, X, Y, Z, rep_ord, lin_q, map_k, offsets, noff, q, key, val, idx, s); break;
    default: launch_topk_vox<8>(nq, nk, X, Y, Z, rep_ord, lin_q, map_k, offsets, noff, q, key, val, idx, s); break;
  }
  COOCC_LAUNCH_CHECK("k_knn_topk_vox");
  return COOCC_OK;
}

__global__ void k_assign_winner(int nc, int K, int ns, int nq, float thresh, const float* __restrict__ val,
                                const int32_t* __restrict__ group, int32_t* __restrict__ winner) {
  int i = blockIdx.x * blockDim.x + threadIdx.x;
  if (i >= nc * ns) return;
  int c = i / ns;
  int qi = group[i];
  if (i != c * ns && qi == group[c * ns]) return;
  for (int k = 0; k < K; ++k)
    if (val[c * K + k] < thresh) atomicMax(&winner[(size_t)k * nq + qi], c);
}

__global__ void k_assign_lookup(int K, int nq, const int32_t* __restrict__ nn,
                                const int32_t* __restrict__ winner, int32_t* __restrict__ out) {
  int i = blockIdx.x * blockDim.x + threadIdx.x;
  if (i >= K * nq) return;
  int k = i / nq;
  int w = winner[i];
  out[i] = w >= 0 ? nn[w * K + k] : -1;
}

extern "C" int coocc_knn_assign(int nc, int K, int ns, int nq, float dist_thresh, const float* val,
                                const int32_t* nn, const int32_t* group, int32_t* winner, int32_t* out,
                                void* stream) {
  COOCC_CHECK_ARG(val && nn && group && winner && out && nc > 0 && K > 0 && ns > 0 && nq > 0, "knn_assign: bad args");
  hipStream_t s = as_stream(stream);
  COOCC_HIP(hipMemsetAsync(winner, 0xFF, sizeof(int32_t) * (size_t)K * nq, s));
  hipLaunchKernelGGL(k_assign_winner, dim3(cdiv((long long)nc * ns, 256)), dim3(256), 0, s, nc, K, ns, nq,
                     dist_thresh, val, group, winner);
  hipLaunchKernelGGL(k_assign_lookup, dim3(cdiv((long long)K * nq, 256)), dim3(256), 0, s, K, nq, nn, winner, out);
  COOCC_LAUNCH_CHECK("knn_assign");
  return COOCC_OK;
}

__global__ void k_knn_threshold(int nq, float thresh, const float* __restrict__ val,
                                const int32_t* __restrict__ nn, int32_t* __restrict__ out) {
  int i = blockIdx.x * blockDim.x + threadIdx.x;
  if (i < nq) out[i] = val[i] < thresh ? nn[i] : -1;
}

extern "C" int coocc_knn_threshold(int nq, float dist_thresh, const float* val, const int32_t* nn,
                                   int32_t* out, void* stream) {
  COOCC_CHECK_ARG(val && nn && out && nq > 0, "knn_threshold: bad args");
  hipLaunchKernelGGL(k_knn_threshold, dim3(cdiv(nq, 256)), dim3(256), 0, as_stream(stream), nq, dist_thresh, val, nn, out);
  COOCC_LAUNCH_CHECK("k_knn_threshold");
  return COOCC_OK;
}

__global__ void k_index_rows(const int32_t* __restrict__ base, int nbase, const int32_t* __restrict__ sel, int n,
                             int32_t* __restrict__ rows) {
  int i = blockIdx.x * blockDim.x + threadIdx.x;
  if (i >= n) return;
  int s = sel[i];
  if (s < 0) s += nbase;
  rows[i] = (s >= 0 && s < nbase) ? base[s] : -1;
}

extern "C" int coocc_index_rows_i32(const int32_t* base, int nbase, const int32_t* sel, int n, int32_t* rows,
                                    void* stream) {
  COOCC_CHECK_ARG(base && sel && rows && nbase > 0 && n >= 0, "index_rows: bad args");
  if (n == 0) return COOCC_OK;
  hipLaunchKernelGGL(k_index_rows, dim3(cdiv(n, 256)), dim3(256), 0, as_stream(stream), base, nbase, sel, n, rows);
  COOCC_LAUNCH_CHECK("k_index_rows");
  return COOCC_OK;
}
```

### co_occ_amd/csrc/layout.hip

```cpp
#include <stdarg.h>
#include <stdlib.h>

#include "common.h"

typedef float f32x4 __attribute__((ext_vector_type(4)));

static thread_local char g_err[512] = "";

int coocc_set_error(int code, const char* fmt, ...) {
  va_list ap;
  va_start(ap, fmt);
  vsnprintf(g_err, sizeof(g_err), fmt, ap);
  va_end(ap);
  return code;
}

extern "C" const char* coocc_last_error(void) { return g_err; }
extern "C" int coocc_abi_version(void) { return 1; }

#define TV 64
#define TC 128

__global__ __launch_bounds__(256) void k_ncdhw_to_ndhwc(const float* __restrict__ src,
                                                         float* __restrict__ dst, int C, int V,
                                                         int dst_stride, int dst_coff) {
  __shared__ float tile[TV][TC + 1];
  const int b = blockIdx.y;
  const int v0 = blockIdx.x * TV;
  const int t = threadIdx.x;
  const int c0 = blockIdx.z * TC;
  const int cn = min(TC, C - c0);
  if (cn == TC) {
    const int v = v0 + (t & 63);
    const float* sp = src + ((size_t)b * C + c0 + (t >> 6)) * V + v;
    float r[TC / 4];
#pragma unroll
    for (int k = 0; k < TC / 4; ++k) r[k] = v < V ? sp[(size_t)(4 * k) * V] : 0.f;
#pragma unroll
    for (int k = 0; k < TC / 4; ++k) tile[t & 63][(t >> 6) + 4 * k] = r[k];
    __syncthreads();
#pragma unroll 8
    for (int i = t; i < TV * TC; i += 256) {
      const int vv = i >> 7, c = i & (TC - 1);
      if (v0 + vv < V) dst[((size_t)b * V + v0 + vv) * dst_stride + dst_coff + c0 + c] = tile[vv][c];
    }
    return;
  }
  for (int c = t >> 6; c < cn; c += 4) {
    int v = v0 + (t & 63);
    tile[t & 63][c] = v < V ? src[((size_t)b * C + c0 + c) * V + v] : 0.f;
  }
  __syncthreads();
  for (int i = t; i < TV * cn; i += 256) {
    int v = i / cn, c = i - v * cn;
    if (v0 + v < V) dst[((size_t)b * V + v0 + v) * dst_stride + dst_coff + c0 + c] = tile[v][c];
  }
}

__global__ __launch_bounds__(256) void k_ndhwc_to_ncdhw(const float* __restrict__ src,
                                                         float* __restrict__ dst, int C, int V,
                                                         int src_stride, int src_coff) {
  __shared__ float tile[TV][TC + 1];
  const int b = blockIdx.y;
  const int v0 = blockIdx.x * TV;
  const int t = threadIdx.x;
  for (int c0 = 0; c0 < C; c0 += TC) {
    const int cn = min(TC, C - c0);
    for (int i = t; i < TV * cn; i += 256) {
      int v = i / cn, c = i - v * cn;
      tile[v][c] = (v0 + v < V) ? src[((size_t)b * V + v0 + v) * src_stride + src_coff + c0 + c] : 0.f;
    }
    __syncthreads();
    for (int c = t >> 6; c < cn; c += 4) {
      int v = v0 + (t & 63);
      if (v < V) dst[((size_t)b * C + c0 + c) * V + v] = tile[t & 63][c];
    }
    __syncthreads();
  }
}

extern "C" int coocc_ncdhw_to_ndhwc(const float* src, float* dst, int B, int C, int V, int dst_stride,
                                    int dst_coff, void* stream) {
  COOCC_CHECK_ARG(src && dst && B > 0 && C > 0 && V > 0 && dst_stride >= dst_coff + C, "ncdhw_to_ndhwc: bad args");
  dim3 grid(cdiv(V, TV), B, cdiv(C, TC));
  hipLaunchKernelGGL(k_ncdhw_to_ndhwc, grid, dim3(256), 0, as_stream(stream), src, dst, C, V, dst_stride, dst_coff);
  COOCC_LAUNCH_CHECK("k_ncdhw_to_ndhwc");
  return COOCC_OK;
}

extern "C" int coocc_ndhwc_to_ncdhw(const float* src, float* dst, int B, int C, int V, int src_stride,
                                    int src_coff, void* stream) {
  COOCC_CHECK_ARG(src && dst && B > 0 && C > 0 && V > 0 && src_stride >= src_coff + C, "ndhwc_to_ncdhw: bad args");
  dim3 grid(cdiv(V, TV), B);
  hipLaunchKernelGGL(k_ndhwc_to_ncdhw, grid, dim3(256), 0, as_stream(stream), src, dst, C, V, src_stride, src_coff);
  COOCC_LAUNCH_CHECK("k_ndhwc_to_ncdhw");
  return COOCC_OK;
}

__global__ __launch_bounds__(256) void k_fuser_prepare(const float* __restrict__ img,
                                                        const float* __restrict__ pts,
                                                        float* __restrict__ cat4,
                                                        uint8_t* __restrict__ flag_img,
                                                        uint8_t* __restrict__ flag_pts, int C, int V) {
  __shared__ float tile[TV][TC + 1];
  const int b = blockIdx.y;
  const int v0 = blockIdx.x * TV;
  const int t = threadIdx.x;
  const int stride = 4 * C;
  for (int mod = 0; mod < 2; ++mod) {
    const float* src = mod ? pts : img;
    uint8_t* flags = mod ? flag_pts : flag_img;
    float rsum = 0.f;
    for (int c0 = 0; c0 < C; c0 += TC) {
      const int cn = min(TC, C - c0);
      for (int c = t >> 6; c < cn; c += 4) {
        int v = v0 + (t & 63);
        tile[t & 63][c] = v < V ? src[((size_t)b * C + c0 + c) * V + v] : 0.f;
      }
      __syncthreads();
      if (t < TV)
        for (int c = 0; c < cn; ++c) rsum += tile[t][c];
      for (int i = t; i < TV * cn; i += 256) {
        int v = i / cn, c = i - v * cn;
        if (v0 + v < V) cat4[((size_t)b * V + v0 + v) * stride + mod * C + c0 + c] = tile[v][c];
      }
      __syncthreads();
    }
    if (t < TV && v0 + t < V) flags[(size_t)b * V + v0 + t] = rsum != 0.f ? 1 : 0;
  }
  for (int i = t; i < TV * 2 * C; i += 256) {
    int v = i / (2 * C), c = i - v * 2 * C;
    if (v0 + v < V) cat4[((size_t)b * V + v0 + v) * stride + 2 * C + c] = 0.f;
  }
}

extern "C" int coocc_fuser_prepare(const float* img, const float* pts, float* cat4, uint8_t* flag_img,
                                   uint8_t* flag_pts, int B, int C, int V, void* stream) {
  COOCC_CHECK_ARG(img && pts && cat4 && flag_img && flag_pts && B > 0 && C > 0 && V > 0, "fuser_prepare: bad args");
  dim3 grid(cdiv(V, TV), B);
  hipLaunchKernelGGL(k_fuser_prepare, grid, dim3(256), 0, as_stream(stream), img, pts, cat4, flag_img, flag_pts, C, V);
  COOCC_LAUNCH_CHECK("k_fuser_prepare");
  return COOCC_OK;
}

__global__ __launch_bounds__(256) void k_fuser_prepare_rows(const float* __restrict__ img, int img_rows, int img_stride,
                                                             const float* __restrict__ pts, int pts_rows, int pts_stride,
                                                             float* __restrict__ cat4, uint8_t* __restrict__ flag_img,
                                                             uint8_t* __restrict__ flag_pts, int C, int V) {
  __shared__ float tile[TV][TC + 1];
  const int b = blockIdx.y;
  const int v0 = blockIdx.x * TV;
  const int t = threadIdx.x;
  const int stride = 4 * C;
  for (int mod = 0; mod < 2; ++mod) {
    const float* src = mod ? pts : img;
    const int rows = mod ? pts_rows : img_rows, sstride = mod ? pts_stride : img_stride;
    uint8_t* flags = mod ? flag_pts : flag_img;
    const bool in_place = rows && src == cat4 + mod * C && sstride == stride;
    float rsum = 0.f;
    for (int c0 = 0; c0 < C; c0 += TC) {
      const int cn = min(TC, C - c0);
      if (rows) {
        if (cn == TC) {
          for (int i = t; i < TV * (TC / 4); i += 256) {
            const int v = i / (TC / 4), c = (i % (TC / 4)) * 4;
            f32x4 q = {0.f, 0.f, 0.f, 0.f};
            if (v0 + v < V) q = *(const f32x4*)(src + ((size_t)b * V + v0 + v) * sstride + c0 + c);
            tile[v][c] = q[0]; tile[v][c + 1] = q[1]; tile[v][c + 2] = q[2]; tile[v][c + 3] = q[3];
          }
        } else {
          for (int i = t; i < TV * cn; i += 256) {
            int v = i / cn, c = i - v * cn;
            tile[v][c] = v0 + v < V ? src[((size_t)b * V + v0 + v) * sstride + c0 + c] : 0.f;
          }
        }
      } else {
        for (int c = t >> 6; c < cn; c += 4) {
          int v = v0 + (t & 63);
          tile[t & 63][c] = v < V ? src[((size_t)b * C + c0 + c) * V + v] : 0.f;
        }
      }
      __syncthreads();
      if (t < TV)
        for (int c = 0; c < cn; ++c) rsum += tile[t][c];
      if (!in_place)
        for (int i = t; i < TV * cn; i += 256) {
          int v = i / cn, c = i - v * cn;
          if (v0 + v < V) cat4[((size_t)b * V + v0 + v) * stride + mod * C + c0 + c] = tile[v][c];
        }
      __syncthreads();
    }
    if (t < TV && v0 + t < V) flags[(size_t)b * V + v0 + t] = rsum != 0.f ? 1 : 0;
  }
  for (int i = t; i < TV * 2 * C; i += 256) {
    int v = i / (2 * C), c = i - v * 2 * C;
    if (v0 + v < V) cat4[((size_t)b * V + v0 + v) * stride + 2 * C + c] = 0.f;
  }
}

constexpr int FV = 256, FC = 32;
__global__ __launch_bounds__(256) void k_fuser_prepare_rows_fast(const float* __restrict__ img, int img_rows, int img_stride,
                                                                  const float* __restrict__ pts, int pts_rows, int pts_stride,
                                                                  float* __restrict__ cat4, uint8_t* __restrict__ flag_img,
                                                                  uint8_t* __restrict__ flag_pts, int C, int V) {
  __shared__ float tile[FV][FC + 1];
  const int b = blockIdx.y;
  const int v0 = blockIdx.x * FV;
  const int t = threadIdx.x;
  const int stride = 4 * C;
  const int rv = t >> 3, rc = (t & 7) * 4;
  for (int mod = 0; mod < 2; ++mod) {
    const float* src = mod ? pts : img;
    const int rows = mod ? pts_rows : img_rows, sstride = mod ? pts_stride : img_stride;
    uint8_t* flags = mod ? flag_pts : flag_img;
    const bool in_place = rows && src == cat4 + mod * C && sstride == stride;
    float rsum = 0.f;
    for (int c0 = 0; c0 < C; c0 += FC) {
      if (rows) {
#pragma unroll
        for (int ps = 0; ps < FV / 32; ++ps) {
          const int v = ps * 32 + rv;
          f32x4 q = {0.f, 0.f, 0.f, 0.f};
          if (v0 + v < V) q = *(const f32x4*)(src + ((size_t)b * V + v0 + v) * sstride + c0 + rc);
          tile[v][rc] = q[0]; tile[v][rc + 1] = q[1]; tile[v][rc + 2] = q[2]; tile[v][rc + 3] = q[3];
        }
        __syncthreads();
#pragma unroll
        for (int c = 0; c < FC; ++c) rsum += tile[t][c];
      } else {
#pragma unroll 8
        for (int c = 0; c < FC; ++c) {
          const float x = v0 + t < V ? src[((size_t)b * C + c0 + c) * V + v0 + t] : 0.f;
          rsum += x;
          tile[t][c] = x;
        }
        __syncthreads();
      }
      if (!in_place) {
#pragma unroll
        for (int ps = 0; ps < FV / 32; ++ps) {
          const int v = ps * 32 + rv;
          if (v0 + v < V) {
            const f32x4 q = {tile[v][rc], tile[v][rc + 1], tile[v][rc + 2], tile[v][rc + 3]};
            *(f32x4*)(cat4 + ((size_t)b * V + v0 + v) * stride + mod * C + c0 + rc) = q;
          }
        }
      }
      __syncthreads();
    }
    if (v0 + t < V) flags[(size_t)b * V + v0 + t] = rsum != 0.f ? 1 : 0;
  }
  const int vec_per_row = C >> 1;
  const f32x4 z = {0.f, 0.f, 0.f, 0.f};
  if (vec_per_row <= 256 && 256 % vec_per_row == 0) {
    const int vpp = 256 / vec_per_row, tv = t / vec_per_row, c = (t - tv * vec_per_row) * 4;
    for (int v = tv; v < FV; v += vpp)
      if (v0 + v < V) *(f32x4*)(cat4 + ((size_t)b * V + v0 + v) * stride + 2 * C + c) = z;
  } else {
    for (int i = t; i < FV * vec_per_row; i += 256) {
      const int v = i / vec_per_row, c = (i - v * vec_per_row) * 4;
      if (v0 + v < V) *(f32x4*)(cat4 + ((size_t)b * V + v0 + v) * stride + 2 * C + c) = z;
    }
  }
}

extern "C" int coocc_fuser_prepare_rows(const float* img, int img_rows, int img_stride, const float* pts, int pts_rows,
                                        int pts_stride, float* cat4, uint8_t* flag_img, uint8_t* flag_pts, int B, int C, int V,
                                        void* stream) {
  COOCC_CHECK_ARG(img && pts && cat4 && flag_img && flag_pts && B > 0 && C > 0 && V > 0, "fuser_prepare_rows: bad args");
  COOCC_CHECK_ARG((!img_rows || img_stride >= C) && (!pts_rows || pts_stride >= C), "fuser_prepare_rows: row stride < C");
  const bool vec_ok = C % FC == 0 && ((uintptr_t)cat4 & 15) == 0 && (!img_rows || (img_stride % 4 == 0 && ((uintptr_t)img & 15) == 0)) &&
                      (!pts_rows || (pts_stride % 4 == 0 && ((uintptr_t)pts & 15) == 0));
  if (vec_ok) {
    hipLaunchKernelGGL(k_fuser_prepare_rows_fast, dim3(cdiv(V, FV), B), dim3(256), 0, as_stream(stream), img, img_rows, img_stride,
                       pts, pts_rows, pts_stride, cat4, flag_img, flag_pts, C, V);
    COOCC_LAUNCH_CHECK("k_fuser_prepare_rows_fast");
    return COOCC_OK;
  }
  dim3 grid(cdiv(V, TV), B);
  hipLaunchKernelGGL(k_fuser_prepare_rows, grid, dim3(256), 0, as_stream(stream), img, img_rows, img_stride, pts, pts_rows,
                     pts_stride, cat4, flag_img, flag_pts, C, V);
  COOCC_LAUNCH_CHECK("k_fuser_prepare_rows");
  return COOCC_OK;
}

#define CB 1024

__global__ __launch_bounds__(256) void k_flag_count(const uint8_t* __restrict__ flags, int total,
                                                     int32_t* __restrict__ blk) {
  __shared__ int wsum[4];
  int base = blockIdx.x * CB + threadIdx.x * 4;
  int c = 0;
  for (int j = 0; j < 4; ++j)
    if (base + j < total) c += flags[base + j] != 0;
  for (int o = 32; o > 0; o >>= 1) c += __shfl_down(c, o);
  if ((threadIdx.x & 63) == 0) wsum[threadIdx.x >> 6] = c;
  __syncthreads();
  if (threadIdx.x == 0) blk[blockIdx.x] = wsum[0] + wsum[1] + wsum[2] + wsum[3];
}

__global__ __launch_bounds__(1024) void k_scan_blocks(int32_t* __restrict__ blk, int nblk,
                                                       int32_t* __restrict__ count) {
  __shared__ int wsum[16];
  __shared__ int carry_s;
  if (threadIdx.x == 0) carry_s = 0;
  __syncthreads();
  for (int base = 0; base < nblk; base += 1024) {
    int i = base + threadIdx.x;
    int v = i < nblk ? blk[i] : 0;
    int inc = v;
    for (int o = 1; o < 64; o <<= 1) {
      int n = __shfl_up(inc, o);
      if ((threadIdx.x & 63) >= o) inc += n;
    }
    if ((threadIdx.x & 63) == 63) wsum[threadIdx.x >> 6] = inc;
    __syncthreads();
    int woff = 0;
    for (int w = 0; w < (int)(threadIdx.x >> 6); ++w) woff += wsum[w];
    int carry = carry_s;
    if (i < nblk) blk[i] = carry + woff + inc - v;
    __syncthreads();
    if (threadIdx.x == 1023) carry_s = carry + woff + inc;
    __syncthreads();
  }
  if (threadIdx.x == 0) *count = carry_s;
}

__global__ __launch_bounds__(256) void k_flag_write(const uint8_t* __restrict__ flags, int total,
                                                     const int32_t* __restrict__ blk,
                                                     int32_t* __restrict__ lin, int32_t* __restrict__ map) {
  __shared__ int wsum[4];
  int base = blockIdx.x * CB + threadIdx.x * 4;
  int f[4], c = 0;
  for (int j = 0; j < 4; ++j) {
    f[j] = (base + j < total) && flags[base + j] != 0;
    c += f[j];
  }
  int inc = c;
  for (int o = 1; o < 64; o <<= 1) {
    int n = __shfl_up(inc, o);
    if ((threadIdx.x & 63) >= o) inc += n;
  }
  if ((threadIdx.x & 63) == 63) wsum[threadIdx.x >> 6] = inc;
  __syncthreads();
  int off = blk[blockIdx.x] + inc - c;
  for (int w = 0; w < (int)(threadIdx.x >> 6); ++w) off += wsum[w];
  for (int j = 0; j < 4; ++j) {
    if (map && base + j < total) map[base + j] = f[j] ? off : -1;
    if (f[j]) lin[off++] = base + j;
  }
}

__device__ __forceinline__ int block_sum256(int v, int* s) {
  for (int o = 32; o > 0; o >>= 1) v += __shfl_xor(v, o);
  __syncthreads();
  if ((threadIdx.x & 63) == 0) s[threadIdx.x >> 6] = v;
  __syncthreads();
  return s[0] + s[1] + s[2] + s[3];
}

__device__ __forceinline__ int nonzero_bytes(uint32_t x) {
  return __popc((((x & 0x7f7f7f7fu) + 0x7f7f7f7fu) | x) & 0x80808080u);
}

#define ONE_PASS_MAX (128 * CB)
#define TWO_PASS_MAX_BLOCKS 2048
template <bool FROM_FLAGS>
__global__ __launch_bounds__(256) void k_flag_write_px(const uint8_t* __restrict__ flags, int total,
                                                        const int32_t* __restrict__ blk, int32_t* __restrict__ count,
                                                        int32_t* __restrict__ lin, int32_t* __restrict__ map) {
  __shared__ int wsum[4], psum[4];
  int before = 0;
  if (FROM_FLAGS) {
    const uint4* w = (const uint4*)flags;
    const int nw = blockIdx.x * (CB / 16);
    for (int i0 = threadIdx.x; i0 < nw; i0 += 256 * 8) {
      uint4 x[8];
#pragma unroll
      for (int k = 0; k < 8; ++k) x[k] = i0 + k * 256 < nw ? w[i0 + k * 256] : make_uint4(0u, 0u, 0u, 0u);
#pragma unroll
      for (int k = 0; k < 8; ++k) before += nonzero_bytes(x[k].x) + nonzero_bytes(x[k].y) + nonzero_bytes(x[k].z) + nonzero_bytes(x[k].w);
    }
  } else {
    for (int i = threadIdx.x; i < (int)blockIdx.x; i += 256) before += blk[i];
  }
  before = block_sum256(before, psum);
  int base = blockIdx.x * CB + threadIdx.x * 4;
  int f[4], c = 0;
  for (int j = 0; j < 4; ++j) {
    f[j] = (base + j < total) && flags[base + j] != 0;
    c += f[j];
  }
  int inc = c;
  for (int o = 1; o < 64; o <<= 1) {
    int n = __shfl_up(inc, o);
    if ((threadIdx.x & 63) >= o) inc += n;
  }
  if ((threadIdx.x & 63) == 63) wsum[threadIdx.x >> 6] = inc;
  __syncthreads();
  int off = before + inc - c;
  for (int w = 0; w < (int)(threadIdx.x >> 6); ++w) off += wsum[w];
  if (blockIdx.x == gridDim.x - 1 && threadIdx.x == 255) *count = off + c;
  for (int j = 0; j < 4; ++j) {
    if (map && base + j < total) map[base + j] = f[j] ? off : -1;
    if (f[j]) lin[off++] = base + j;
  }
}

extern "C" int coocc_compact_flags_ex(const uint8_t* flags, int total, int32_t* lin, int32_t* count, int32_t* map, void* ws,
                                      size_t ws_bytes, void* stream);
extern "C" int coocc_compact_flags(const uint8_t* flags, int total, int32_t* lin, int32_t* count, void* ws,
                                   size_t ws_bytes, void* stream) {
  return coocc_compact_flags_ex(flags, total, lin, count, nullptr, ws, ws_bytes, stream);
}
extern "C" int coocc_compact_flags_ex(const uint8_t* flags, int total, int32_t* lin, int32_t* count, int32_t* map, void* ws,
                                      size_t ws_bytes, void* stream) {
  COOCC_CHECK_ARG(flags && lin && count && ws && total > 0, "compact_flags: bad args");
  int nblk = (int)cdiv(total, CB);
  if (ws_bytes < sizeof(int32_t) * (size_t)nblk) return coocc_set_error(COOCC_ENOMEM, "compact_flags: workspace too small");
  int32_t* blk = (int32_t*)ws;
  const char* e = getenv("COOCC_COMPACT_SCAN");
  if (e && e[0] == '1') {
    hipLaunchKernelGGL(k_flag_count, dim3(nblk), dim3(256), 0, as_stream(stream), flags, total, blk);
    hipLaunchKernelGGL(k_scan_blocks, dim3(1), dim3(1024), 0, as_stream(stream), blk, nblk, count);
    hipLaunchKernelGGL(k_flag_write, dim3(nblk), dim3(256), 0, as_stream(stream), flags, total, blk, lin, map);
  } else if (total <= ONE_PASS_MAX && ((uintptr_t)flags & 15) == 0) {
    hipLaunchKernelGGL(k_flag_write_px<true>, dim3(nblk), dim3(256), 0, as_stream(stream), flags, total, blk, count, lin, map);
  } else if (nblk <= TWO_PASS_MAX_BLOCKS) {
    hipLaunchKernelGGL(k_flag_count, dim3(nblk), dim3(256), 0, as_stream(stream), flags, total, blk);
    hipLaunchKernelGGL(k_flag_write_px<false>, dim3(nblk), dim3(256), 0, as_stream(stream), flags, total, blk, count, lin, map);
  } else {
    hipLaunchKernelGGL(k_flag_count, dim3(nblk), dim3(256), 0, as_stream(stream), flags, total, blk);
    hipLaunchKernelGGL(k_scan_blocks, dim3(1), dim3(1024), 0, as_stream(stream), blk, nblk, count);
    hipLaunchKernelGGL(k_flag_write, dim3(nblk), dim3(256), 0, as_stream(stream), flags, total, blk, lin, map);
  }
  COOCC_LAUNCH_CHECK("compact_flags");
  return COOCC_OK;
}

__global__ void k_lin_to_coords(const int32_t* __restrict__ lin, int n, int X, int Y, int Z,
                                float* __restrict__ xyz, int64_t* __restrict__ bxyz) {
  int i = blockIdx.x * blockDim.x + threadIdx.x;
  if (i >= n) return;
  int l = lin[i];
  int z = l % Z; l /= Z;
  int y = l % Y; l /= Y;
  int x = l % X; int b = l / X;
  if (xyz) { xyz[i * 3 + 0] = (float)x; xyz[i * 3 + 1] = (float)y; xyz[i * 3 + 2] = (float)z; }
  if (bxyz) { bxyz[i * 4 + 0] = b; bxyz[i * 4 + 1] = x; bxyz[i * 4 + 2] = y; bxyz[i * 4 + 3] = z; }
}

extern "C" int coocc_lin_to_coords(const int32_t* lin, int n, int X, int Y, int Z, float* xyz, int64_t* bxyz,
                                   void* stream) {
  COOCC_CHECK_ARG(lin && n >= 0 && X > 0 && Y > 0 && Z > 0, "lin_to_coords: bad args");
  if (n == 0) return COOCC_OK;
  hipLaunchKernelGGL(k_lin_to_coords, dim3(cdiv(n, 256)), dim3(256), 0, as_stream(stream), lin, n, X, Y, Z, xyz, bxyz);
  COOCC_LAUNCH_CHECK("k_lin_to_coords");
  return COOCC_OK;
}

extern "C" int coocc_device_cu_count(int* n) {
  COOCC_CHECK_ARG(n, "device_cu_count: null");
  int dev = 0;
  COOCC_HIP(hipGetDevice(&dev));
  hipDeviceProp_t prop;
  COOCC_HIP(hipGetDeviceProperties(&prop, dev));
  *n = prop.multiProcessorCount;
  return COOCC_OK;
}

extern "C" int coocc_stream_create_cu_mask(const uint32_t* mask_host, int nwords, void** stream_out) {
  COOCC_CHECK_ARG(mask_host && nwords > 0 && stream_out, "stream_create_cu_mask: bad args");
  hipStream_t s = nullptr;
  COOCC_HIP(hipExtStreamCreateWithCUMask(&s, (uint32_t)nwords, mask_host));
  *stream_out = (void*)s;
  return COOCC_OK;
}

extern "C" int coocc_stream_destroy(void* stream) {
  COOCC_CHECK_ARG(stream, "stream_destroy: null");
  COOCC_HIP(hipStreamDestroy(as_stream(stream)));
  return COOCC_OK;
}

extern "C" int coocc_event_create(int flags, void** event_out) {
  COOCC_CHECK_ARG(event_out && (flags & ~3) == 0, "event_create: bad args");
  hipEvent_t e = nullptr;
  COOCC_HIP(hipEventCreateWithFlags(&e, hipEventDisableSystemFence | ((flags & 1) ? 0u : hipEventDisableTiming) |
                                            ((flags & 2) ? hipEventBlockingSync : 0u)));
  *event_out = (void*)e;
  return COOCC_OK;
}
extern "C" int coocc_event_destroy(void* event) {
  COOCC_CHECK_ARG(event, "event_destroy: null");
  COOCC_HIP(hipEventDestroy((hipEvent_t)event));
  return COOCC_OK;
}
extern "C" int coocc_event_record(void* event, void* stream) {
  COOCC_CHECK_ARG(event, "event_record: null");
  COOCC_HIP(hipEventRecord((hipEvent_t)event, as_stream(stream)));
  return COOCC_OK;
}
extern "C" int coocc_stream_wait_event(void* stream, void* event) {
  COOCC_CHECK_ARG(event, "stream_wait_event: null");
  COOCC_HIP(hipStreamWaitEvent(as_stream(stream), (hipEvent_t)event, 0));
  return COOCC_OK;
}
extern "C" int coocc_event_synchronize(void* event) {
  COOCC_CHECK_ARG(event, "event_synchronize: null");
  COOCC_HIP(hipEventSynchronize((hipEvent_t)event));
  return COOCC_OK;
}
extern "C" int coocc_event_query(void* event) {
  COOCC_CHECK_ARG(event, "event_query: null");
  const hipError_t e = hipEventQuery((hipEvent_t)event);
  if (e == hipSuccess) return 1;
  if (e == hipErrorNotReady) { (void)hipGetLastError(); return 0; }
  return coocc_set_error(COOCC_EHIP, "hipEventQuery failed: %s", hipGetErrorString(e));
}
extern "C" int coocc_event_elapsed_ms(void* start, void* stop, float* ms) {
  COOCC_CHECK_ARG(start && stop && ms, "event_elapsed_ms: null");
  COOCC_HIP(hipEventElapsedTime(ms, (hipEvent_t)start, (hipEvent_t)stop));
  return COOCC_OK;
}
```

### co_occ_amd/csrc/search.hip

```cpp
#include <stdlib.h>
#include <string.h>

#include "common.h"

__global__ __launch_bounds__(256) void k_gather_xyz(const float* __restrict__ xyz, const int32_t* __restrict__ idx, int m,
                                                     float* __restrict__ out) {
  const int i = blockIdx.x * blockDim.x + threadIdx.x;
  if (i >= m) return;
  const int s = idx[i];
  out[i * 3 + 0] = xyz[s * 3 + 0]; out[i * 3 + 1] = xyz[s * 3 + 1]; out[i * 3 + 2] = xyz[s * 3 + 2];
}

struct SearchWs {
  uint8_t* flags;
  int32_t* cws;
  float* xyz;
  int32_t* maps;
  int32_t* rep[2];
  float* rep_xyz[2];
  float* val[2];
  int32_t* nn[2];
  int32_t* group[2];
  int32_t* winner[2];
  void* fps[2];
  size_t fps_bytes;
  size_t total;
};

static SearchWs carve(char* base, int V, int K, int fps_num, int max_cluster, int X, int Y, int Z) {
  SearchWs w;
  size_t o = 0;
  auto take = [&](size_t bytes) { char* p = base ? base + o : nullptr; o += al256(bytes); return p; };
  w.flags = (uint8_t*)take((size_t)2 * V);
  w.cws = (int32_t*)take((size_t)2 * (V / 1024 + 2) * 4);
  w.xyz = (float*)take((size_t)2 * V * 3 * 4);
  w.maps = (int32_t*)take((size_t)2 * V * 4);
  w.fps_bytes = coocc_fps_voxels_ws(X, Y, Z);
  for (int d = 0; d < 2; ++d) {
    w.rep[d] = (int32_t*)take((size_t)fps_num * 4);
    w.rep_xyz[d] = (float*)take((size_t)fps_num * 3 * 4);
    w.val[d] = (float*)take((size_t)fps_num * K * 4);
    w.nn[d] = (int32_t*)take((size_t)fps_num * K * 4);
    w.group[d] = (int32_t*)take((size_t)fps_num * max_cluster * 4);
    w.winner[d] = (int32_t*)take((size_t)K * V * 4);
    w.fps[d] = take(w.fps_bytes);
  }
  w.total = o;
  return w;
}

extern "C" size_t coocc_fuser_search_ws(const coocc_search_desc* d) {
  if (!d || d->X <= 0 || d->Y <= 0 || d->Z <= 0 || d->K <= 0) return 0;
  return carve(nullptr, d->X * d->Y * d->Z, d->K, d->fps_num, d->max_cluster, d->X, d->Y, d->Z).total;
}

#define SRC(call)                    \
  do {                               \
    int rc__ = (call);               \
    if (rc__ != COOCC_OK) return rc__; \
  } while (0)

extern "C" int coocc_fuser_search(coocc_search_desc* d, void* stream, void* side_stream) {
  COOCC_CHECK_ARG(d && d->cat4 && d->pts && d->lin && d->counts && d->rows && d->rows_p && d->near_img && d->near_pts && d->ws &&
                      d->offsets && d->counts_host, "fuser_search: null pointer");
  COOCC_CHECK_ARG(d->C > 0 && d->X > 0 && d->Y > 0 && d->Z > 0 && d->K >= 1 && d->K <= 8 && d->fps_num > 0 && d->max_cluster > 0 &&
                      d->noff > 0, "fuser_search: bad sizes");
  COOCC_CHECK_ARG(stream != side_stream && side_stream, "fuser_search: needs a second stream for the img <- pts direction");
  const int V = d->X * d->Y * d->Z, K = d->K, C = d->C;
  SearchWs w = carve((char*)d->ws, V, K, d->fps_num, d->max_cluster, d->X, d->Y, d->Z);
  COOCC_CHECK_ARG(d->ws_bytes >= w.total, "fuser_search: workspace smaller than coocc_fuser_search_ws()");
  hipStream_t s0 = as_stream(stream), s1 = as_stream(side_stream);
  static const int sdiag = [] { const char* e = getenv("COOCC_SEARCH_DIAG_SKIP"); return e ? atoi(e) : 0; }();
  int32_t* lin_img = d->lin;
  int32_t* lin_pts = d->lin + V;

  SRC(coocc_fuser_prepare_rows(d->cat4, 1, 4 * C, d->pts, d->pts_rows, d->pts_stride, d->cat4, w.flags, w.flags + V, 1, C, V, stream));
  SRC(coocc_compact_flags(w.flags, V, lin_img, d->counts, w.cws, (size_t)(V / 1024 + 2) * 4, stream));
  SRC(coocc_compact_flags(w.flags + V, V, lin_pts, d->counts + 1, w.cws + (V / 1024 + 2), (size_t)(V / 1024 + 2) * 4, stream));
  if (!((sdiag & 4) && d->counts_host[0] > 0)) COOCC_HIP(hipMemcpyAsync(d->counts_host, d->counts, 8, hipMemcpyDeviceToHost, s0));
  if (!((sdiag & 4) && d->counts_host[0] > 0)) {
    static const bool fence = [] { const char* e = getenv("COOCC_SEARCH_COUNT_FENCE"); return e && e[0] == '1'; }();
    hipEvent_t got;
    COOCC_HIP(hipEventCreateWithFlags(&got, hipEventBlockingSync | hipEventDisableTiming | (fence ? 0u : hipEventDisableSystemFence)));
    const hipError_t e1 = hipEventRecord(got, s0);
    const hipError_t e2 = e1 == hipSuccess ? hipEventSynchronize(got) : e1;
    (void)hipEventDestroy(got);
    if (e2 != hipSuccess) return coocc_set_error(COOCC_EHIP, "fuser_search: waiting for the voxel counts failed: %s", hipGetErrorString(e2));
  }
  const int Ni = d->counts_host[0], Np = d->counts_host[1];
  if (Ni <= d->fps_num || Np <= d->fps_num) return COOCC_SEARCH_SMALL;

  float* xyz_img = w.xyz;
  float* xyz_pts = w.xyz + (size_t)V * 3;
  SRC(coocc_lin_to_coords(lin_img, Ni, d->X, d->Y, d->Z, xyz_img, nullptr, stream));
  SRC(coocc_lin_to_coords(lin_pts, Np, d->X, d->Y, d->Z, xyz_pts, nullptr, stream));
  int32_t* map_img = w.maps;
  int32_t* map_pts = w.maps + V;
  SRC(coocc_voxel_index_map(lin_img, Ni, V, map_img, stream));
  SRC(coocc_voxel_index_map(lin_pts, Np, V, map_pts, stream));

  const int pair_rc = (sdiag & 1) ? COOCC_OK
                                  : coocc_fps_voxels_pair(lin_pts, Np, w.rep[0], w.fps[0], lin_img, Ni, w.rep[1], w.fps[1], w.fps_bytes, d->X, d->Y,
                                                          d->Z, d->fps_num, stream);
  if (pair_rc != COOCC_OK && pair_rc != 2) return pair_rc;
  const bool paired = pair_rc == COOCC_OK;
  hipEvent_t fork = nullptr, join = nullptr;
  COOCC_HIP(hipEventCreateWithFlags(&fork, hipEventDisableTiming | hipEventDisableSystemFence));
  if (hipEventCreateWithFlags(&join, hipEventDisableTiming | hipEventDisableSystemFence) != hipSuccess) {
    (void)hipEventDestroy(fork);
    return coocc_set_error(COOCC_EHIP, "fuser_search: hipEventCreate failed");
  }
  bool forked = false;
  auto finish = [&](int rc) -> int {
    if (forked) {
      if (hipEventRecord(join, s1) != hipSuccess || hipStreamWaitEvent(s0, join, 0) != hipSuccess) {
        if (rc == COOCC_OK) rc = coocc_set_error(COOCC_EHIP, "fuser_search: joining the side stream failed");
      }
    }
    (void)hipEventDestroy(fork);
    (void)hipEventDestroy(join);
    return rc;
  };
#define SRF(call)                                \
  do {                                           \
    int rc__ = (call);                           \
    if (rc__ != COOCC_OK) return finish(rc__);   \
  } while (0)
  void* side_q = paired ? stream : side_stream;
  if (!paired) {
    if (hipEventRecord(fork, s0) != hipSuccess || hipStreamWaitEvent(s1, fork, 0) != hipSuccess)
      return finish(coocc_set_error(COOCC_EHIP, "fuser_search: forking the side stream failed"));
    forked = true;
  }

  auto direction = [&](int dd, void* st, const int32_t* lin_q, int Q, const float* xyz_q, const int32_t* map_q, int Nk,
                       const float* xyz_k, const int32_t* map_k, int32_t* near) -> int {
    if (sdiag & 2) return COOCC_OK;
    if (!paired) SRC(coocc_fps_voxels(lin_q, Q, d->X, d->Y, d->Z, d->fps_num, w.rep[dd], w.fps[dd], w.fps_bytes, st));
    hipLaunchKernelGGL(k_gather_xyz, dim3(cdiv(d->fps_num, 256)), dim3(256), 0, as_stream(st), xyz_q, w.rep[dd], d->fps_num, w.rep_xyz[dd]);
    COOCC_LAUNCH_CHECK("k_gather_xyz");
    SRC(coocc_knn_topk_voxels(d->fps_num, Nk, K, d->X, d->Y, d->Z, w.rep[dd], lin_q, map_k, d->offsets, d->noff, w.rep_xyz[dd], xyz_k,
                              w.val[dd], w.nn[dd], st));
    SRC(coocc_ball_query_voxels(d->fps_num, 0.f, d->radius, d->max_cluster, d->X, d->Y, d->Z, w.rep[dd], lin_q, map_q, w.group[dd], st));
    SRC(coocc_knn_assign(d->fps_num, K, d->max_cluster, Q, d->dist_thresh, w.val[dd], w.nn[dd], w.group[dd], w.winner[dd], near, st));
    return COOCC_OK;
  };
  SRF(direction(1, side_q, lin_img, Ni, xyz_img, map_img, Np, xyz_pts, map_pts, d->near_pts));
  for (int k = 0; k < K && !(sdiag & 2); ++k)
    SRF(coocc_index_rows_i32(K == 1 ? lin_pts : lin_img, K == 1 ? Np : Ni, d->near_pts + (size_t)k * Ni, Ni, d->rows_p + (size_t)k * V, side_q));
  SRF(direction(0, stream, lin_pts, Np, xyz_pts, map_pts, Ni, xyz_img, map_img, d->near_img));
  for (int k = 0; k < K && !(sdiag & 2); ++k)
    SRF(coocc_index_rows_i32(lin_img, Ni, d->near_img + (size_t)k * Np, Np, d->rows + (size_t)k * V, stream));
#undef SRF
  return finish(COOCC_OK);
}
```

### include/coocc_hip.h

```cpp
#ifndef COOCC_HIP_H
#define COOCC_HIP_H

#include <stddef.h>
#include <stdint.h>

#ifdef __cplusplus
extern "C" {
#endif

#define COOCC_OK 0
#define COOCC_EINVAL (-1)
#define COOCC_EHIP (-2)
#define COOCC_ENOMEM (-3)

const char* coocc_last_error(void);
int coocc_abi_version(void);

int coocc_device_cu_count(int* n);
int coocc_stream_create_cu_mask(const uint32_t* mask_host, int nwords, void** stream_out);
int coocc_stream_destroy(void* stream);

int coocc_event_create(int flags, void** event_out);
int coocc_event_destroy(void* event);
int coocc_event_record(void* event, void* stream);
int coocc_stream_wait_event(void* stream, void* event);
int coocc_event_synchronize(void* event);
int coocc_event_query(void* event);
int coocc_event_elapsed_ms(void* start, void* stop, float* ms);


int coocc_ncdhw_to_ndhwc(const float* src, float* dst, int B, int C, int V, int dst_stride,
                         int dst_coff, void* stream);
int coocc_ndhwc_to_ncdhw(const float* src, float* dst, int B, int C, int V, int src_stride,
                         int src_coff, void* stream);

int coocc_fuser_prepare(const float* img, const float* pts, float* cat4, uint8_t* flag_img,
                        uint8_t* flag_pts, int B, int C, int V, void* stream);
int coocc_fuser_prepare_rows(const float* img, int img_rows, int img_stride, const float* pts, int pts_rows,
                             int pts_stride, float* cat4, uint8_t* flag_img, uint8_t* flag_pts, int B, int C, int V,
                             void* stream);

int coocc_compact_flags(const uint8_t* flags, int total, int32_t* lin, int32_t* count, void* ws,
                        size_t ws_bytes, void* stream);
int coocc_compact_flags_ex(const uint8_t* flags, int total, int32_t* lin, int32_t* count, int32_t* map, void* ws,
                           size_t ws_bytes, void* stream);
int coocc_lin_to_coords(const int32_t* lin, int n, int X, int Y, int Z, float* xyz, int64_t* bxyz,
                        void* stream);


int coocc_furthest_point_sampling(int b, int n, int m, const float* points, float* temp,
                                  int32_t* idx, void* stream);

size_t coocc_fps_voxels_ws(int X, int Y, int Z);
int coocc_fps_voxels(const int32_t* lin, int n, int X, int Y, int Z, int m, int32_t* idx, void* ws,
                     size_t ws_bytes, void* stream);
int coocc_fps_voxels_pair(const int32_t* lin0, int n0, int32_t* idx0, void* ws0, const int32_t* lin1, int n1, int32_t* idx1,
                          void* ws1, size_t ws_bytes_each, int X, int Y, int Z, int m, void* stream);

int coocc_ball_query(int b, int n, int m, float min_radius, float max_radius, int nsample,
                     const float* new_xyz, const float* xyz, int32_t* idx, void* stream);

#define COOCC_SEARCH_SMALL 1
typedef struct coocc_search_desc {
  float* cat4;
  const float* pts;
  int pts_rows, pts_stride;
  int C, X, Y, Z, K;
  int fps_num, max_cluster;
  float radius, dist_thresh;
  const uint32_t* offsets;
  int noff;
  int32_t* lin;
  int32_t* counts;
  int32_t* near_img;
  int32_t* near_pts;
  int32_t* rows;
  int32_t* rows_p;
  void* ws;
  size_t ws_bytes;
  int32_t* counts_host;
} coocc_search_desc;
size_t coocc_fuser_search_ws(const coocc_search_desc* d);
int coocc_fuser_search(coocc_search_desc* d, void* stream, void* side_stream);

int coocc_voxel_index_map(const int32_t* lin, int n, int nvox, int32_t* map, void* stream);
int coocc_voxel_index_map_dev(const int32_t* lin, int n_cap, const int32_t* n_dev, int nvox, int32_t* map, void* stream);
int coocc_ball_query_voxels(int m, float min_radius, float max_radius, int nsample, int X, int Y, int Z,
                            const int32_t* centre_ord, const int32_t* lin_q, const int32_t* map_q, int32_t* idx,
                            void* stream);
int coocc_knn_topk_voxels(int nq, int nk, int K, int X, int Y, int Z, const int32_t* rep_ord, const int32_t* lin_q,
                          const int32_t* map_k, const uint32_t* offsets, int noff, const float* q, const float* key,
                          float* val, int32_t* idx, void* stream);

int coocc_knn_topk(int nq, int nk, int K, const float* q, const float* key, float* val,
                   int32_t* idx, void* stream);

int coocc_knn_assign(int nc, int K, int ns, int nq, float dist_thresh, const float* val,
                     const int32_t* nn, const int32_t* group, int32_t* winner, int32_t* out,
                     void* stream);
int coocc_knn_threshold(int nq, float dist_thresh, const float* val, const int32_t* nn,
                        int32_t* out, void* stream);
int coocc_index_rows_i32(const int32_t* base, int nbase, const int32_t* sel, int n, int32_t* rows,
                         void* stream);


int64_t coocc_conv_pack_weights(const float* w_host, int Cout, int Cin, int taps, int tap_major,
                                float* packed_host);

typedef struct coocc_conv_desc {
  const float* in;
  const float* w;
  float* out;
  const float* scale;
  const float* bias;
  const float* res;
  const int32_t* gather;
  const int32_t* out_rows;
  float* ws;
  int64_t ws_floats;
  int M, Cin, Cout, taps;
  int in_stride, out_stride, res_stride;
  int B, Xi, Yi, Zi, Xo, Yo, Zo, ksize, stride, pad;
  int relu, res_mode;
  int splitk;
  int tile_hint;
  int kx, ky, kz;
  int px, py, pz;
  int wgroup_rows;
  int mfma_dtype;
  float alpha;
  const int32_t* M_dev;
  int gather_stride;
  void* out16;
  int out16_stride;
  int out_h2;
  void* out_h2_twin;
  int32_t* tile_sem;
  int tile_sem_ints;
  const float* alpha_dev;
  int sx, sy, sz;
} coocc_conv_desc;

int coocc_conv_fwd(const coocc_conv_desc* d, void* stream);

int coocc_rows_to_bf16(const float* in, int in_stride, int64_t rows, int C, void* out_bf16, void* stream);

int coocc_rows_to_h2(const float* in, int in_stride, int64_t rows, int C, float scale, void* out_h2, void* stream);
int coocc_rows_to_h2_ex(const float* in, int in_stride, int64_t rows, int C, float scale, const float* scale_dev, void* out_h2,
                        void* stream);
int coocc_rows_to_f16(const float* in, int in_stride, int64_t rows, int C, void* out_f16, void* stream);
int coocc_rows_to_h2_gather(const float* in, int in_stride, const int32_t* row_ids, int64_t n_cap, const int32_t* n_dev,
                            int C, float scale, void* out_h2, void* stream);

int coocc_wino_input(const float* in, int in_stride, int B, int X, int Y, int Z, int C, int tile, float* V,
                     int64_t group_rows, void* stream);
int coocc_wino_input_strided(const float* in, int in_stride, int B, int X, int Y, int Z, int C, int tile, float* V,
                             int vstride, int64_t group_rows, void* stream);
int coocc_wino_input_h2(const float* in, int in_stride, int B, int X, int Y, int Z, int C, int tile, void* V,
                        int vstride, int64_t group_rows, float scale, void* stream);
int coocc_wino_input_h2_ex(const float* in, int in_stride, int B, int X, int Y, int Z, int C, int tile, void* V,
                           int vstride, int64_t group_rows, float scale, const float* scale_dev, void* stream);
int coocc_sparse_tap_sum(const float* P, const int32_t* map, int B, int X, int Y, int Z, int Cout, const float* scale,
                         float* S, int s_stride, int p_rows, void* stream);
int coocc_wino_output(const float* Mb, int64_t group_rows, int B, int X, int Y, int Z, int C, int tile, float* out,
                      int out_stride, const float* scale, const float* bias, const float* res, int res_stride,
                      int relu, void* stream);
int coocc_wino_output_ex(const float* Mb, int64_t group_rows, int B, int X, int Y, int Z, int C, int tile, float* out,
                         int out_stride, const float* scale, const float* bias, const float* res, int res_stride,
                         int relu, void* out_h2_twin, void* stream);
int coocc_render_heads_h2(const void* x_h2, int V, int Cin, int width, const void* ws0_pack, const float* bs0,
                          const float* ws1, const float* bs1, const void* const* wr_packs_host,
                          const float* const* br_host, int n_rgb_hidden, const float* wr_out, const float* br_out,
                          float* table, int activate, void* stream);
int coocc_head_pred_h2(const void* x_h2, int in_stride, int rows, const int32_t* rows_dev, const void* w1_pack,
                       const float* scale1, const float* bias1, float* hq, int hq_stride, int write_hidden,
                       const void* w2_pack, const float* bias2, int ncls, float* logits, int logit_stride,
                       int empty_idx, uint8_t* flags, void* stream);
int coocc_head_soft_h2(const void* x_h2, int in_stride, int rows, const int32_t* rows_dev, const void* w1_pack,
                       const float* scale1, const float* bias1, float* hidden, int hidden_stride, const void* w2_pack,
                       const float* bias2, int L, float* wlogit, int wlogit_stride, void* stream);
int64_t coocc_wino_pack_weights_h2_dev(const float* w, int Cout, int Cin, int tile, int dgrad, void* packed, void* stream);
int64_t coocc_conv_pack_weights_h2_dev(const float* w, int Cout, int Cin, int taps, int mode, void* packed, void* stream);
int coocc_h2_overflow(int reset);
#define COOCC_FAULT_SPARSE_ORDINAL 1
int coocc_device_fault(int reset);
int64_t coocc_wino_pack_weights_dev(const float* w, int Cout, int Cin, int tile, int dgrad, float* packed, void* stream);
int coocc_wino_gradout(const float* dy, int dy_stride, int B, int X, int Y, int Z, int C, int tile, float* dM,
                       int64_t group_rows, void* stream);
int coocc_wino_ztap_table(int64_t rows_total, int Z, int32_t* table, void* stream);
int coocc_wino_wgrad(const float* V, const float* dM, int64_t group_rows, int Z, int Cin, int Cout, int tile,
                     const int32_t* ztap_table, float* dw, int accumulate, float* ws, int64_t ws_floats,
                     void* stream);
int coocc_rows_to_kh2(const float* x, int stride, int64_t rows, int64_t rows_pad, int C, float scale, const float* scale_dev,
                      void* out_kh2, void* stream);
int coocc_wino_operand_kh2(int which, const float* x, int x_stride, int B, int X, int Y, int Z, int C, int tile, void* out_kh2,
                           int64_t group_rows, float scale, const float* scale_dev, void* stream);
int coocc_conv_wgrad_h2(const void* x_kh2, const void* dy_kh2, int64_t rows_pad, int Cin, int Cout, float alpha,
                        const float* alpha_dev, float* dw, int accumulate, float* ws, int64_t ws_floats, void* stream);
int coocc_wino_wgrad_h2(const void* V_kh2, const void* dM_kh2, int64_t group_rows, int Z, int Cin, int Cout, int tile,
                        float alpha, const float* alpha_dev, float* dw, int accumulate, float* ws, int64_t ws_floats,
                        void* stream);

int64_t coocc_conv_pack_weights_dev(const float* w, int Cout, int Cin, int taps, int mode, float* packed,
                                    void* stream);
int coocc_conv_tap_table(int B, int Xi, int Yi, int Zi, int Xo, int Yo, int Zo, int ksize, int stride, int pad,
                         int dgrad, int32_t* table, void* stream);
int coocc_conv_epilogue_bwd(const float* dout, int dout_stride, const float* out, int out_stride,
                            const float* scale, int M, int C, int relu, float* dacc, int dacc_stride,
                            float* dres, int dres_stride, int dres_accumulate, float* dbias,
                            int dbias_accumulate, float* ws, int64_t ws_floats, void* stream);
#define COOCC_AMAX_WORDS 2048
int coocc_conv_epilogue_bwd_ex(const float* dout, int dout_stride, const float* out, int out_stride,
                               const float* scale, int M, int C, int relu, float* dacc, int dacc_stride,
                               float* dres, int dres_stride, int dres_accumulate, float* dbias,
                               int dbias_accumulate, float* ws, int64_t ws_floats, uint32_t* amax_word, float* scale2,
                               float target, void* stream);
int coocc_conv_wgrad(const float* in, int in_rows, int in_stride, const float* dacc, int dacc_stride,
                     const int32_t* table, int M, int Cin, int Cout, int taps, float* dw, int accumulate,
                     float* ws, int64_t ws_floats, void* stream);
int coocc_conv_wgrad_h2t(const float* in, int in_rows, int in_stride, const float* dacc, int dacc_stride,
                         const int32_t* table, int M, int Cin, int Cout, int taps, const float* scale2,
                         float* dw, int accumulate, float* ws, int64_t ws_floats, void* stream);

int coocc_gather_rows(const float* src, int src_stride, const int32_t* idx, int n, int C, float* dst,
                      int dst_stride, void* stream);
int coocc_scatter_add_rows(const float* src, int src_stride, const int32_t* idx, int n, int C, float* dst,
                           int dst_stride, void* stream);
int coocc_voxel_pool_bwd(const float* dout, int dout_stride, const float* geom, int npts, int pts_per_batch,
                         int C, const float* lo_dx_host, int B, int X, int Y, int Z, float* dx, void* stream);
int coocc_lift_splat_bwd(const float* dout, int dout_stride, const float* depth, const float* feat_nhwc,
                         const float* geom, int N, int D, int H, int W, int C, int pts_per_batch,
                         const float* lo_dx_host, int B, int X, int Y, int Z, float* d_depth,
                         float* d_feat_nhwc, void* stream);
int coocc_render_nearest_bwd(const float* table, int X, int Y, int Z, const float* geom, const float* zvals,
                             int N, int D, int H, int W, const float* bounds_host, const float* dmaps,
                             float* dtable, void* stream);
int coocc_upsample_maps_bwd(const float* drgbs, const float* ddepths, int N, int H, int W, int scale,
                            float* dmaps, void* stream);
int coocc_render_losses_bwd(const float* rgbs, const float* depths, const float* rgb_gt, const float* depth_gt,
                            int64_t npix, int D, const float* losses_out, const float* gl, float* drgbs,
                            float* ddepths, void* stream);

int coocc_upsample_trilinear_bwd(const float* dfine, float* dcoarse, int B, int C, int Xc, int Yc, int Zc, int Xf,
                                 int Yf, int Zf, int accumulate, void* stream);

int coocc_occhead_mix_bwd(const float* const* levels_host, const int* dims_host, int L, const float* wlogit,
                          const float* dout, float* const* glevels_host, float* dwlogit, int B, int C,
                          void* stream);

int coocc_fine_sample_voxel_bwd(const float* dfeat, int dfeat_stride, int C, int X, int Y, int Z,
                                const int64_t* fine_xyz, int64_t nfine, const int* final_size_host, float* dvol,
                                void* stream);
int coocc_groupnorm_rows_bwd(const float* x, const float* y, const float* dy, int64_t n, int C, int stride, int groups,
                             const float* gamma, float eps, int relu, float* dx, float* dgamma, float* dbeta,
                             void* stream);

int coocc_fine_sample_img_bwd(const float* dfeat, int dfeat_stride, int ncam, int Ci, int Hf, int Wf,
                              const float* params, const int64_t* fine_xyz, int64_t nfine, float* dimg,
                              void* stream);
int coocc_groupnorm_nhwc_bwd(const float* x, const float* y, const float* dy, int N, int HW, int C, int groups,
                             const float* gamma, float eps, int relu, float* dx, float* dgamma, float* dbeta,
                             void* stream);

int coocc_bn_stats(const float* x, int stride, int M, int C, float* mean, float* var, void* ws, size_t ws_bytes,
                   void* stream);
int coocc_bn_apply(const float* x, int M, int C, const float* mean, const float* var, const float* gamma,
                   const float* beta, float eps, const float* res, int relu, float* y, void* stream);
int coocc_bn_backward(const float* x, const float* y, const float* dy, int M, int C, const float* mean, const float* var,
                      const float* gamma, float eps, int relu, float* dx, float* dres, float* dgamma, float* dbeta,
                      void* ws, size_t ws_bytes, void* stream);
int coocc_bn_backward_sums(const float* x, const float* y, const float* dy, int M, int C, const float* mean,
                           const float* var, float eps, int relu, float* dgamma, float* dbeta, void* ws,
                           size_t ws_bytes, void* stream);
int coocc_bn_backward_dx(const float* x, const float* y, const float* dy, int M, int C, const float* mean,
                         const float* var, const float* gamma, float eps, int relu, const float* sum_dgamma,
                         const float* sum_dbeta, double count, float* dx, float* dres, void* stream);

int coocc_upsample_add_trilinear(const float* coarse, float* fine, int B, int C, int Xc, int Yc,
                                 int Zc, int Xf, int Yf, int Zf, void* stream);
int coocc_upsample_add_trilinear_ex(const float* coarse, float* fine, int B, int C, int Xc, int Yc,
                                    int Zc, int Xf, int Yf, int Zf, void* fine_h2_twin, void* stream);

int coocc_occhead_mix(const float* const* levels_host, const int* dims_host , int L,
                      const float* wlogit , float* out, int B, int C, void* stream);
int coocc_occhead_mix_ex(const float* const* levels_host, const int* dims_host , int L,
                         const float* wlogit , float* out, int B, int C, void* out_h2_twin, void* stream);

int coocc_argmax_flags(const float* logits, int V, int ncls, int stride, int empty_idx,
                       uint8_t* flags, void* stream);
int coocc_fine_sample_voxel(const float* vol, int C, int X, int Y, int Z, const int32_t* coarse_lin,
                            int n, int ratio, const int* final_size_host, int64_t* fine_xyz,
                            float* feat, int out_stride, void* stream);
int coocc_fine_sample_img(const float* img_nhwc, int ncam, int Ci, int Hf, int Wf,
                          const float* params, const int64_t* fine_xyz, int64_t nfine, float* feat,
                          int out_stride, int group, void* stream);
int coocc_projection_params(const float* rots, const float* trans, const float* intrins, const float* post_rots,
                            const float* post_trans, const float* bda, int ncam, const float* hdr_host,
                            float* params, void* stream);
int coocc_fine_mlp(const float* samp, int samp_stride, const float* vox, int vox_stride, int64_t nfine,
                   const float* w_img, const float* b_img, const float* gn_img_w, const float* gn_img_b,
                   float eps_img, const float* w_f0, const float* b_f0, const float* gn_f0_w,
                   const float* gn_f0_b, float eps_f0, const float* w_f3, const float* b_f3, int ncls,
                   float* out, void* stream);
int coocc_fine_mlp_pre(const float* samp64, int samp_stride, const float* vox64, int vox_stride, int64_t nfine,
                       const float* b_img, const float* gn_img_w, const float* gn_img_b, float eps_img,
                       const float* w_f0, const float* b_f0, const float* gn_f0_w, const float* gn_f0_b,
                       float eps_f0, const float* w_f3, const float* b_f3, int ncls, float* out, void* stream);
int coocc_fine_sample_voxel_dev(const float* vol, int C, int X, int Y, int Z, const int32_t* coarse_lin, int n_cap,
                                const int32_t* n_dev, int ratio, const int* final_size_host, int64_t* fine_xyz,
                                float* feat, int out_stride, void* stream);
int coocc_fine_sample_img_dev(const float* img_nhwc, int ncam, int Ci, int Hf, int Wf, const float* params,
                              const int64_t* fine_xyz, int64_t nfine_cap, const int32_t* n_dev, float* feat,
                              int out_stride, int group, void* stream);
int coocc_fine_mlp_pre_dev(const float* samp64, int samp_stride, const float* vox64, int vox_stride, int64_t nfine_cap,
                           const int32_t* n_dev, int n_mul, const float* b_img, const float* gn_img_w,
                           const float* gn_img_b, float eps_img, const float* w_f0, const float* b_f0,
                           const float* gn_f0_w, const float* gn_f0_b, float eps_f0, const float* w_f3, const float* b_f3,
                           int ncls, float* out, void* stream);
int coocc_scatter_fine_dev(const float* fine_logits, int64_t nfine_cap, const int32_t* n_dev, int n_mul, int ncls, int stride,
                           const int64_t* fine_xyz, float* grid, int Xf, int Yf, int Zf, float empty_val, void* stream);
int coocc_scatter_fine_grouped(const float* fine_logits, int ncls, int stride, const int32_t* coarse_lin, int n_cap,
                               const int32_t* n_dev, int R, int Xc, int Yc, int Zc, float* grid, float empty_val,
                               int32_t* map_ws, void* stream);
int coocc_groupnorm_rows(float* x, int64_t n, int C, int stride, int groups, const float* gamma,
                         const float* beta, float eps, int relu, void* stream);
int coocc_groupnorm_nhwc(float* x, int N, int HW, int C, int groups, const float* gamma,
                         const float* beta, float eps, int relu, void* stream);
int coocc_scatter_fine(const float* fine_logits, int64_t nfine, int ncls, int stride,
                       const int64_t* fine_xyz, float* grid, int Xf, int Yf, int Zf, float empty_val,
                       void* stream);

#define COOCC_CAM_FLOATS 39
int coocc_camera_mats(const float* rots, const float* trans, const float* intrins, const float* post_rots,
                      const float* post_trans, const float* bda, int B, int N, int intrin_dim, int bda_dim,
                      float* mats, void* stream);
int coocc_get_geometry(const float* mats, const float* xs, const float* ys, const float* ds, int BN,
                       int D, int fH, int fW, float* geom, void* stream);

int coocc_bev_pool_forward(const float* x, const int32_t* geom, const int32_t* interval_lengths,
                           const int32_t* interval_starts, int b, int d, int h, int w, int n, int c,
                           int n_intervals, float* out, void* stream);
int coocc_bev_pool_backward(const float* out_grad, const int32_t* geom,
                            const int32_t* interval_lengths, const int32_t* interval_starts, int b,
                            int d, int h, int w, int n, int c, int n_intervals, float* x_grad,
                            void* stream);
size_t coocc_voxel_pool_ws(int npts, int nvox);
int coocc_voxel_pool(const float* x, const float* geom, int npts, int pts_per_batch, int C,
                     const float* lo_dx_host, int B, int X, int Y, int Z, float* out, int out_stride,
                     void* ws, size_t ws_bytes, int ws_clean, void* stream);
int coocc_lift_splat(const float* depth, const float* feat_nhwc, const float* geom, int N, int D, int H, int W,
                     int C, int pts_per_batch, const float* lo_dx_host, int B, int X, int Y, int Z, float* out,
                     int out_stride, void* ws, size_t ws_bytes, int ws_clean, void* stream);
int coocc_lift_splat_cams(const float* depth, const float* feat_nhwc, const float* mats, const float* xs,
                          const float* ys, const float* ds, int N, int D, int H, int W, int C,
                          int pts_per_batch, const float* lo_dx_host, int B, int X, int Y, int Z, float* out,
                          int out_stride, void* ws, size_t ws_bytes, int ws_clean, void* stream);
int coocc_lift_splat_reuse(const float* depth, const float* feat_nhwc, int N, int D, int H, int W, int C, int B, int X,
                           int Y, int Z, float* out, int out_stride, void* ws, size_t ws_bytes, void* stream);
int coocc_bev_pool_coords(const float* x, const int64_t* coords, int n, int C, int B, int X, int Y,
                          int Z, float* out, int out_stride, void* ws, size_t ws_bytes, int ws_clean, void* stream);

int coocc_fine_fused(const float* Q, int X, int Y, int Z, const float* P, int ncam, int Hf, int Wf, const float* params,
                     const int32_t* coarse_lin, int n_cap, const int32_t* n_dev, int ratio, const int* final_size_host,
                     const float* b_img, const float* gn_img_w, const float* gn_img_b, float eps_img, const float* w_f0,
                     const float* b_f0, const float* gn_f0_w, const float* gn_f0_b, float eps_f0, const float* w_f3,
                     const float* b_f3, int ncls, int64_t* fine_xyz, float* out, void* stream);

int coocc_fine2_pack(const float* w_f0, const float* w_f3, int ncls, const float* b_img, const float* gn_img_w,
                     const float* gn_img_b, const float* b_f0, const float* gn_f0_w, const float* gn_f0_b, const float* b_f3,
                     void* wpack, float* consts, void* stream);
int coocc_fine2_h2(const float* Q, int q_stride, int X, int Y, int Z, const float* P, int ncam, int Hf, int Wf, const float* params,
                   const int32_t* coarse_lin, int n_cap, const int32_t* n_dev, const int* final_size_host, const void* wpack,
                   const float* consts, float eps_img, float eps_f0, int ncls, int64_t* fine_xyz, float* out,
                   const float* img_samples, void* stream);
int coocc_fine_sample_img_lin(const float* img_nhwc, int ncam, int Ci, int Hf, int Wf, const float* params,
                              const int32_t* coarse_lin, int Yc, int Zc, int n_cap, const int32_t* n_dev, float* feat,
                              int out_stride, int ratio, void* stream);

int coocc_render_nearest(const float* table, int X, int Y, int Z, const float* geom,
                         const float* zvals, int N, int D, int H, int W, const float* bounds_host,
                         int activated, float* maps, void* stream);
int coocc_render_nearest_cams(const float* table, int X, int Y, int Z, const float* mats, const float* xs, const float* ys,
                              const float* ds, const float* zvals, int N, int D, int H, int W,
                              const float* bounds_host, int activated, float* maps, void* stream);
int coocc_render_activate_table(float* table, int V, void* stream);
int coocc_upsample_maps(const float* maps, int N, int H, int W, int scale, float* rgbs,
                        float* depths, void* stream);
int coocc_volume_sampling(const float* vol, int C, int d0, int d1, int d2, const float* pts, int n,
                          const float* aabb_host, float* feat, uint8_t* mask, void* stream);
int coocc_raw2outputs(const float* raw, const float* z, int R, int S, int white_bkgd, float zmin,
                      float zmax, float* rgb, float* depth, float* weights, void* stream);
int coocc_render_losses(const float* rgbs, const float* depths, const float* rgb_gt,
                        const float* depth_gt, int64_t npix, int D, float* out, void* ws, size_t ws_bytes,
                        void* stream);

int coocc_eval_semantic(const float* pred, int64_t stride_c, int64_t stride_x, int64_t stride_y,
                        int64_t stride_z, int C, int h, int w, int d, const uint8_t* gt,
                        const uint8_t* visible, int H, int W, int D, int empty_idx, int accumulate,
                        int64_t* hist, void* stream);
int coocc_predict_labels(const float* pred, int64_t stride_c, int64_t stride_x, int64_t stride_y,
                         int64_t stride_z, int C, int h, int w, int d, int H, int W, int D, uint8_t* labels,
                         void* stream);

int coocc_lidarseg_points(const float* logits, int64_t stride_c, int64_t stride_x, int64_t stride_y, int64_t stride_z,
                          int C, int X, int Y, int Z, const float* points, int64_t n, int64_t point_stride, int point_cols,
                          int label_col, const float* range_host, int padding_mode, int mode, float* probs, int64_t* labels,
                          int accumulate, int64_t* hist, void* stream);

int64_t coocc_render_eval_stats(const float* rgbs, const float* depths, const float* gt_img, const float* gt_depth, int N, int H,
                                int W, double* block, void* ws, size_t ws_bytes, void* stream);
int coocc_render_panels(const float* rgbs, const float* depths, const float* gt_img, const double* block, int N, int H, int W,
                        uint8_t* panels, void* stream);
int64_t coocc_render_eval_ssim(const float* rgbs, const float* gt_img, int N, int H, int W, double data_range, double* block,
                               void* ws, size_t ws_bytes, void* stream);

size_t coocc_voxelize_ws(int n);
int coocc_voxelize_hard(const float* points, int n, int F, const float* range_host, const float* voxel_size_host,
                        int max_points, int max_voxels, float* voxels, int32_t* coors, int32_t* num_points,
                        int32_t* count, void* ws, size_t ws_bytes, void* stream);
int coocc_vfe_mean(const float* voxels, const int32_t* num_points, int M, int max_points, int F, int nf, float* out,
                   int out_stride, void* stream);
int coocc_sparse_index_map(const int32_t* coors, int M, int D, int H, int W, int32_t* map ,
                           void* stream);
int coocc_sparse_conv_table(const int32_t* out_coors, int Mo, int Di, int Hi, int Wi, int ksize, int stride, int pad,
                            const int32_t* in_map, int32_t* table , void* stream);
int coocc_sparse_down_flags(const int32_t* coors, int M, int ksize, int stride, int pad, int Do, int Ho, int Wo,
                            uint8_t* flags , void* stream);
int coocc_sparse_conv_table3(const int32_t* out_coors, int Mo, int Di, int Hi, int Wi, int kz, int ky, int kx, int sz, int sy,
                             int sx, int pz, int py, int px, const int32_t* in_map, int32_t* table, void* stream);
int coocc_sparse_down_flags3(const int32_t* coors, int M, int Di, int Hi, int Wi, int kz, int ky, int kx, int sz, int sy, int sx,
                             int pz, int py, int px, int Do, int Ho, int Wo, uint8_t* flags, void* stream);
int coocc_sparse_lin_to_coors(const int32_t* lin, int n, int D, int H, int W, int32_t* coors, int32_t* dense_rows,
                              void* stream);


int coocc_fpn_sum(const float* const* ups, const int* strides, int levels, int B, int X, int Y, int Z, int C, float* out,
                  int out_stride, void* out_h2_twin, void* stream);
int coocc_zyx_to_rows(const float* src, float* dst, int B, int C, int Z, int Y, int X, int dst_stride, int dst_coff,
                      void* stream);

int coocc_conv_tap_table3(int B, int Xi, int Yi, int Zi, int Xo, int Yo, int Zo, int kx, int ky, int kz, int sx, int sy, int sz,
                          int px, int py, int pz, int dgrad, int32_t* table, void* stream);
int coocc_fpn_sum_bwd(const float* dout, int dout_stride, float* const* dups, const int* strides, int levels, int B, int X, int Y,
                      int Z, int C, void* stream);

int coocc_sparse_dgrad_table3(const int32_t* in_coors, int Mi, int Di, int Hi, int Wi, int kz, int ky, int kx, int sz, int sy, int sx,
                              int pz, int py, int px, int Do, int Ho, int Wo, const int32_t* out_map, int32_t* table, int32_t* classes,
                              void* stream);
int coocc_bn_apply_ex(const float* x, int M, int C, const float* mean, const float* var, const float* gamma, const float* beta,
                      float eps, const float* res, int relu, float* y, void* out_h2, void* stream);

#define COOCC_OCC_LOSS_STATS 208
int coocc_pool_labels(const uint8_t* vol, int B, int H, int W, int D, int ratio, int empty_idx, int num_cls, uint8_t* out,
                      void* stream);
size_t coocc_occ_loss_ws(int64_t P, int C);
int coocc_occ_loss_fwd(const float* logits, int64_t P, int C, int ld, const uint8_t* labels, const int64_t* coords, int VX, int VY,
                       int VZ, uint8_t* row_labels, const float* class_w, int empty_idx, float* out, double* stats, float* lov_w,
                       void* ws, size_t ws_bytes, void* stream);
int coocc_occ_loss_bwd(const float* logits, int64_t P, int C, int ld, const uint8_t* row_labels, const float* class_w, int empty_idx,
                       const double* stats, const float* lov_w, const float* gout, float* dlogits, int ldg, void* stream);

#define COOCC_DEPTH_BCE_STATS 2
int coocc_depth_labels(const float* gt, int BN, int H, int W, int ds, float c0, float step, int D, float* vals, int32_t* labels,
                       void* stream);
size_t coocc_depth_bce_ws(int64_t P, int D);
int coocc_depth_bce(const float* prob, const int32_t* labels, int BN, int D, int h, int w, float weight, float* loss, double* stats,
                    void* ws, size_t ws_bytes, void* stream);
int coocc_depth_bce_bwd(const float* prob, const int32_t* labels, int BN, int D, int h, int w, float weight, const double* stats,
                        const float* gout, float* dprob, void* stream);

int coocc_nbr_table2d(int BN, int H, int W, int dil, int32_t* table, void* stream);
int coocc_dcn_cols(const float* x, int x_stride, const float* off, int off_stride, int BN, int H, int W, int C, int groups, int m0,
                   int n, float* cols, void* stream);
int coocc_se_gate2(const float* x, int x_stride, int BN, int rows_per_cam, int C, const float* gate_a, const float* gate_b,
                   float* out_a, float* out_b, void* stream);
size_t coocc_cam_mean_ws(int BN, int HW, int C);
int coocc_cam_mean(const float* x, int stride, int BN, int HW, int C, float* mean, void* ws, size_t ws_bytes, void* stream);
int coocc_cam_bias_relu(float* y, int y_stride, int BN, int rows_per_cam, int C, const float* bias, int relu, void* stream);

int coocc_dcn_cols_bwd(const float* x, int x_stride, const float* off, int off_stride, int BN, int H, int W, int C, int groups,
                       int m0, int n, const float* dcols, float* dx, float* doff, void* stream);
size_t coocc_se_gate2_bwd_ws(int BN, int HW, int C);
int coocc_se_gate2_bwd(const float* x, int x_stride, int BN, int rows_per_cam, int C, const float* gate_a, const float* gate_b,
                       const float* d_out_a, const float* d_out_b, float* dx, float* dgate_a, float* dgate_b, void* ws,
                       size_t ws_bytes, void* stream);
int coocc_cam_sum(const float* x, int stride, int BN, int HW, int C, float* sum, void* ws, size_t ws_bytes, void* stream);
int coocc_cam_add(const float* x, float* y, int BN, int rows_per_cam, int C, const float* v, float scale, void* stream);
int coocc_dropout_rows(const float* x, const uint8_t* mask, int64_t M, int C, float scale, float* y, void* stream);

int coocc_img_stem(const float* img, int BN, int H, int W, const float* w, const float* scale, const float* bias, int C0, int relu,
                   int pool, float* out, int out_stride, void* out_h2_twin, void* stream);

int coocc_maxpool2d_rows(const float* x, int x_stride, int BN, int Hc, int Wc, int C, float* out, int out_stride, void* out_h2_twin,
                         void* stream);
int coocc_maxpool2d_rows_bwd(const float* x, int x_stride, const float* dy, int dy_stride, int BN, int Hc, int Wc, int C, float* dx,
                             int dx_stride, void* stream);
size_t coocc_img_stem_wgrad_ws(int BN, int H, int W);
int coocc_img_stem_wgrad(const float* img, int BN, int H, int W, const float* dy, int dy_stride, int C0, float* dw, void* ws,
                         size_t ws_bytes, void* stream);

typedef struct coocc_optim_tensor {
  float* p;
  float* g;
  float* exp_avg;
  float* exp_avg_sq;
  int64_t numel;
  double lr, weight_decay, beta1, beta2, eps;
  double bias_correction1;
  double bias_correction2;
} coocc_optim_tensor;
int coocc_optim_chunk(void);
int coocc_optim_sumsq(const coocc_optim_tensor* tensors, const coocc_optim_tensor* tensors_host, int ntensors, const int64_t* chunks,
                      int nchunks, double* partials, void* stream);
int coocc_optim_clip_coef(const double* partials, int nchunks, float max_norm, double* norm64, float* norm32, float* coef,
                          void* stream);
int coocc_optim_adamw(const coocc_optim_tensor* tensors, const coocc_optim_tensor* tensors_host, int ntensors, const int64_t* chunks,
                      int nchunks, const float* coef, int write_grad, void* stream);
int coocc_optim_scale(const coocc_optim_tensor* tensors, const coocc_optim_tensor* tensors_host, int ntensors, const int64_t* chunks,
                      int nchunks, const float* coef, void* stream);
int coocc_optim_pack(const coocc_optim_tensor* tensors, const coocc_optim_tensor* tensors_host, int ntensors, const int64_t* chunks,
                     int nchunks, float* arena, int64_t arena_numel, int world, void* stream);
int coocc_optim_unpack(const coocc_optim_tensor* tensors, const coocc_optim_tensor* tensors_host, int ntensors, const int64_t* chunks,
                       int nchunks, const float* arena, int64_t arena_numel, void* stream);
int coocc_optim_flag_check(const coocc_optim_tensor* tensors, int ntensors, const float* header, int world, int* sticky,
                           void* stream);

int coocc_frames_to_imgs(const uint8_t* frames, const void* const* frame_ptrs, int N, int Hs, int Ws, const int32_t* params,
                         const int32_t* params_host, const int32_t* tables, int64_t table_ints, int fH, int fW, float* imgs,
                         uint8_t* canvas, void* stream);

int coocc_points_to_depth_maps(const float* points, int64_t P, int point_stride, const float* cams, int N, int H, int W, float* maps,
                               void* stream);

int coocc_occ_scatter_labels(const uint16_t* rows, int64_t N, int G0, int G1, int G2, int use_semantic, uint32_t* win, uint8_t* vol,
                             void* stream);
int coocc_occ_rows_to_voxels(const uint16_t* rows, int64_t N, const double* grid, const float* bda, int G0, int G1, int G2, int32_t* vox,
                             uint8_t* labels, float* centres, void* stream);
int coocc_occ_points_to_voxels(const float* points, int64_t P, int point_stride, const uint8_t* seg, const uint8_t* table, const float* bda,
                               const double* grid, int G0, int G1, int G2, int mode, int32_t* vox, uint8_t* labels, float* points_occ,
                               void* stream);
size_t coocc_occ_vote_ws(int64_t N);
int coocc_occ_vote_labels(const int32_t* vox, const uint8_t* labels, int64_t N, int64_t V, int fill, int post_empty, uint8_t* vol, void* ws,
                          size_t ws_bytes, void* stream);
int coocc_occ_visible_rows(const float* centres, int64_t N, const float* cams, int ncam, int H, int W, uint64_t* canvas, uint8_t* flags,
                           void* stream);
int coocc_occ_cloud_aabb(const float* points, int64_t P, int point_stride, const double* transforms, uint64_t* slots, float* aabb,
                         void* stream);

#define COOCC_SWEEPS_MAX_SEGS 65
#define COOCC_SWEEPS_MAX_USE 16
#define COOCC_SWEEP_TRANSFORM 1
#define COOCC_SWEEP_FILTER 2
typedef struct coocc_sweep_seg {
  int64_t in_row0, n_rows, out_row0;
  double R[9], t[3];
  float dt;
  int32_t flags;
} coocc_sweep_seg;
size_t coocc_sweeps_merge_ws(int64_t rows);
int coocc_sweeps_merge(const float* raw, int64_t in_rows, int load_dim, const coocc_sweep_seg* segs, const coocc_sweep_seg* segs_host,
                       int nseg, const int32_t* use_dim_host, int n_use, float radius, float* out, int64_t out_rows, int32_t* count,
                       void* ws, size_t ws_bytes, void* stream);

#ifdef __cplusplus
}
#endif
#endif
```

Baseline: 266.7.

## Enqueue fuser search with device-side counts to overlap host count readback

Adds device-count variants of the search kernels (FPS pair, kNN top-k, ball query, assign, index rows, coords, index map). These read the voxel counts from device memory and size or skip their work there. The fuser search now enqueues the whole pipeline right away and copies the counts to pinned host memory in parallel, so it no longer stalls on a host sync before launching. The price is kernels launched at capacity that exit early when there is no work, a per-call event creation, and a more complex code path that the oneshot setting controls.

Measured after the change: 276.3, median of 6. +3.6%, better.

```diff
diff --git a/co_occ_amd/_lib.py b/co_occ_amd/_lib.py
--- a/co_occ_amd/_lib.py
+++ b/co_occ_amd/_lib.py
@@ -85,6 +85,14 @@
     "coocc_conv_fwd": (I, [ctypes.POINTER(ConvDesc), P]),
     "coocc_fuser_search_ws": (Z, [ctypes.POINTER(SearchDesc)]),
     "coocc_fuser_search": (I, [ctypes.POINTER(SearchDesc), P, P]),
+    "coocc_fuser_search_oneshot": (I, [I]),
+    "coocc_lin_to_coords_dev": (I, [P, I, P, I, I, I, I, I, P, P]),
+    "coocc_fps_voxels_pair_ok": (I, [I, I, I, I]),
+    "coocc_fps_voxels_pair_dev": (I, [P, I, P, P, P, I, P, P, Z, I, P, I, I, I, I, I, P]),
+    "coocc_knn_topk_voxels_dev": (I, [I, I, I, I, I, P, P, P, P, I, P, P, P, P, P, I, I, P]),
+    "coocc_ball_query_voxels_dev": (I, [I, F, F, I, I, I, I, P, P, P, P, P, I, P]),
+    "coocc_knn_assign_dev": (I, [I, I, I, I, F, P, P, P, P, P, P, I, I, P]),
+    "coocc_index_rows_i32_dev": (I, [P, I, P, I, I, I, P, P, I, P]),
     "coocc_upsample_add_trilinear": (I, [P, P, I, I, I, I, I, I, I, I, P]),
     "coocc_upsample_add_trilinear_ex": (I, [P, P, I, I, I, I, I, I, I, I, P, P]),
     "coocc_occhead_mix": (I, [P, P, I, P, P, I, I, P]),
diff --git a/co_occ_amd/csrc/knn.hip b/co_occ_amd/csrc/knn.hip
--- a/co_occ_amd/csrc/knn.hip
+++ b/co_occ_amd/csrc/knn.hip
@@ -133,8 +133,36 @@
 
 struct FpsCell { int temp; int r; };
 
+struct FpsRank { int L, q, RB, tinit; bool key32; };
+__host__ __device__ inline FpsRank fps_rank_layout(int n, long long d2max) {
+  FpsRank r;
+  int L = 0;
+  while ((2 << L) <= n && L < 10) ++L;
+  const int q = (n + (1 << L) - 1) >> L;
+  int RB = L;
+  while ((1ll << RB) <= ((long long)q << L)) ++RB;
+  r.key32 = RB < 31 && d2max + 1 < (1ll << (32 - RB)) - 1;
+  r.tinit = r.key32 ? (int)((1u << (32 - RB)) - 1u) : 0x7FFFFFFF;
+  r.L = L; r.q = q; r.RB = RB;
+  return r;
+}
+static inline long long fps_d2max(int X, int Y, int Z) {
+  return (long long)(X - 1) * (X - 1) + (long long)(Y - 1) * (Y - 1) + (long long)(Z - 1) * (Z - 1);
+}
+
+__device__ __forceinline__ bool dev_counts_small(const int32_t* __restrict__ cnt, int small_m) {
+  return cnt[0] <= small_m || cnt[1] <= small_m;
+}
+
 __global__ __launch_bounds__(256) void k_fpsv_scatter(const int32_t* __restrict__ lin, int n, int Y, int Z, int NBY,
-                                                       int NBZ, int L, int q, int tinit, FpsCell* __restrict__ cell) {
+                                                       int NBZ, int L, int q, int tinit, FpsCell* __restrict__ cell,
+                                                       const int32_t* __restrict__ cnt, int which, int small_m, long long d2max) {
+  if (cnt) {
+    if (dev_counts_small(cnt, small_m)) return;
+    n = min(n, cnt[which]);
+    const FpsRank r = fps_rank_layout(n, d2max);
+    L = r.L; q = r.q; tinit = r.tinit;
+  }
   int k = blockIdx.x * blockDim.x + threadIdx.x;
   if (k >= n) return;
   int l = lin[k];
@@ -340,17 +368,23 @@
 }
 
 #define FPSR_SLOTS 40
-struct FpsRegProblem { const int32_t* lin; const FpsCell* cell; int32_t* idx; int n, L, q, RB; };
-struct FpsRegArgs { FpsRegProblem p[2]; int m, Y, Z, NBY, NBZ, NB; long long* dbg; };
+struct FpsRegProblem { const int32_t* lin; const FpsCell* cell; int32_t* idx; int n, L, q, RB, which; };
+struct FpsRegArgs { FpsRegProblem p[2]; int m, Y, Z, NBY, NBZ, NB; long long* dbg; const int32_t* cnt; int small_m; long long d2max; };
 
 __global__ __launch_bounds__(1024) void k_fps_voxels_reg(FpsRegArgs a) {
   constexpr int NW = 16;
+  if (a.cnt && dev_counts_small(a.cnt, a.small_m)) return;
   __builtin_amdgcn_s_setprio(3);
   __shared__ unsigned wbest[2][NW];
   __shared__ int wloc[2][NW];
   const FpsRegProblem pr = a.p[blockIdx.x];
   const int tid = threadIdx.x, lane = tid & 63, wave = __builtin_amdgcn_readfirstlane(tid >> 6);
-  const int RB = pr.RB, Y = a.Y, Z = a.Z, NB = a.NB, m = a.m;
+  int pL = pr.L, pq = pr.q, pRB = pr.RB;
+  if (a.cnt) {
+    const FpsRank rk = fps_rank_layout(a.cnt[pr.which], a.d2max);
+    pL = rk.L; pq = rk.q; pRB = rk.RB;
+  }
+  const int RB = pRB, Y = a.Y, Z = a.Z, NB = a.NB, m = a.m;
   const unsigned rmask = (1u << RB) - 1u;
   const unsigned tmax = (1u << (32 - RB)) - 1u;
   long long* dbg = a.dbg;
@@ -454,9 +488,9 @@
   __syncthreads();
   for (int j = 1 + tid; j < m; j += 1024) {
     const unsigned rr = rmask - (unsigned)pr.idx[j];
-    const unsigned hi = rr / (unsigned)pr.q, lo = rr - hi * (unsigned)pr.q;
-    const unsigned rev = pr.L ? (__brev(hi) >> (32 - pr.L)) : 0u;
-    pr.idx[j] = (int)((lo << pr.L) | rev);
+    const unsigned hi = rr / (unsigned)pq, lo = rr - hi * (unsigned)pq;
+    const unsigned rev = pL ? (__brev(hi) >> (32 - pL)) : 0u;
+    pr.idx[j] = (int)((lo << pL) | rev);
   }
   if (dbg && lane == 0 && blockIdx.x == 0) {
     long long* o = dbg + wave * 8;
@@ -477,7 +511,7 @@
 struct FpsPrep { int NBX, NBY, NBZ, L, q, RB, tinit, threads, R; long long NB; bool key32; };
 
 static int fps_prepare(const int32_t* lin, int n, int X, int Y, int Z, int m, const int32_t* idx, void* ws, size_t ws_bytes,
-                       hipStream_t s, FpsPrep* o) {
+                       hipStream_t s, FpsPrep* o, const int32_t* cnt = nullptr, int which = 0, int small_m = 0) {
   COOCC_CHECK_ARG(lin && idx && ws && n > 0 && m >= 0 && X > 0 && Y > 0 && Z > 0, "fps_voxels: bad args");
   COOCC_CHECK_ARG(n < (1 << FPS_KBITS), "fps_voxels: n must be < 2^22");
   COOCC_CHECK_ARG(X <= 1020 && Y <= 1020 && Z <= 1016, "fps_voxels: grid dims must fit 10-bit packed coordinates");
@@ -489,19 +523,17 @@
   if (ws_bytes < coocc_fps_voxels_ws(X, Y, Z)) return coocc_set_error(COOCC_ENOMEM, "fps_voxels: workspace too small");
   o->threads = threads;
   o->R = (int)((o->NB + threads - 1) / threads);
-  int L = 0;
-  while ((2 << L) <= n && L < 10) ++L;
-  const int q = (n + (1 << L) - 1) >> L;
-  int RB = L;
-  while ((1ll << RB) <= ((long long)q << L)) ++RB;
-  const long long d2max = (long long)(X - 1) * (X - 1) + (long long)(Y - 1) * (Y - 1) + (long long)(Z - 1) * (Z - 1);
-  o->key32 = RB < 31 && d2max + 1 < (1ll << (32 - RB)) - 1;
-  o->tinit = o->key32 ? (int)((1u << (32 - RB)) - 1u) : 0x7FFFFFFF;
-  o->L = L; o->q = q; o->RB = RB;
+  const long long d2max = fps_d2max(X, Y, Z);
+  const FpsRank rk = fps_rank_layout(n, d2max);
+  const int L = rk.L, q = rk.q;
+  o->key32 = rk.key32;
+  o->tinit = rk.tinit;
+  o->L = L; o->q = q; o->RB = rk.RB;
   if (m == 0) return COOCC_OK;
   FpsCell* cell = (FpsCell*)ws;
   COOCC_HIP(hipMemsetAsync(cell, 0xFF, sizeof(FpsCell) * (size_t)o->NB * FT_P, s));
-  hipLaunchKernelGGL(k_fpsv_scatter, dim3(cdiv(n, 256)), dim3(256), 0, s, lin, n, Y, Z, o->NBY, o->NBZ, L, q, o->tinit, cell);
+  hipLaunchKernelGGL(k_fpsv_scatter, dim3(cdiv(n, 256)), dim3(256), 0, s, lin, n, Y, Z, o->NBY, o->NBZ, L, q, o->tinit, cell, cnt, which,
+                     small_m, d2max);
   COOCC_LAUNCH_CHECK("k_fpsv_scatter");
   return COOCC_OK;
 }
@@ -510,6 +542,15 @@
 static bool fps_reg_ok(const FpsPrep& o) {
   if (g_fps_reg < 0) g_fps_reg = getenv("COOCC_FPS_REG") ? atoi(getenv("COOCC_FPS_REG")) : 1;
   return g_fps_reg && o.key32 && o.NB <= (long long)FPSR_SLOTS * 16;
+}
+
+extern "C" int coocc_fps_voxels_pair_ok(int n, int X, int Y, int Z) {
+  if (n <= 0 || X <= 0 || Y <= 0 || Z <= 0 || n >= (1 << FPS_KBITS)) return 0;
+  const long long NB = (long long)((X + FT_X - 1) / FT_X) * ((Y + FT_Y - 1) / FT_Y) * ((Z + FT_Z - 1) / FT_Z);
+  if (NB > (long long)FPSR_SLOTS * 16) return 0;
+  if (!fps_rank_layout(n, fps_d2max(X, Y, Z)).key32) return 0;
+  if (g_fps_reg < 0) g_fps_reg = getenv("COOCC_FPS_REG") ? atoi(getenv("COOCC_FPS_REG")) : 1;
+  return g_fps_reg ? 1 : 0;
 }
 
 extern "C" int coocc_fps_voxels(const int32_t* lin, int n, int X, int Y, int Z, int m, int32_t* idx, void* ws,
@@ -557,21 +598,7 @@
 extern "C" int coocc_fps_voxels_pair(const int32_t* lin0, int n0, int32_t* idx0, void* ws0, const int32_t* lin1, int n1, int32_t* idx1,
                                      void* ws1, size_t ws_bytes_each, int X, int Y, int Z, int m, void* stream) {
   COOCC_CHECK_ARG(X > 0 && Y > 0 && Z > 0 && n0 > 0 && n1 > 0, "fps_voxels_pair: bad args");
-  {
-    const long long NB = (long long)((X + FT_X - 1) / FT_X) * ((Y + FT_Y - 1) / FT_Y) * ((Z + FT_Z - 1) / FT_Z);
-    if (NB > (long long)FPSR_SLOTS * 16) return 2;
-    const long long d2max = (long long)(X - 1) * (X - 1) + (long long)(Y - 1) * (Y - 1) + (long long)(Z - 1) * (Z - 1);
-    for (int n : {n0, n1}) {
-      int L = 0;
-      while ((2 << L) <= n && L < 10) ++L;
-      const int q = (n + (1 << L) - 1) >> L;
-      int RB = L;
-      while ((1ll << RB) <= ((long long)q << L)) ++RB;
-      if (!(RB < 31 && d2max + 1 < (1ll << (32 - RB)) - 1)) return 2;
-    }
-    if (g_fps_reg < 0) g_fps_reg = getenv("COOCC_FPS_REG") ? atoi(getenv("COOCC_FPS_REG")) : 1;
-    if (!g_fps_reg) return 2;
-  }
+  if (!coocc_fps_voxels_pair_ok(n0, X, Y, Z) || !coocc_fps_voxels_pair_ok(n1, X, Y, Z)) return 2;
   hipStream_t s = as_stream(stream);
   FpsPrep o0, o1;
   int rc = fps_prepare(lin0, n0, X, Y, Z, m, idx0, ws0, ws_bytes_each, s, &o0);
@@ -582,6 +609,28 @@
   a.p[0] = FpsRegProblem{lin0, (const FpsCell*)ws0, idx0, n0, o0.L, o0.q, o0.RB};
   a.p[1] = FpsRegProblem{lin1, (const FpsCell*)ws1, idx1, n1, o1.L, o1.q, o1.RB};
   a.m = m; a.Y = Y; a.Z = Z; a.NBY = o0.NBY; a.NBZ = o0.NBZ; a.NB = (int)o0.NB; a.dbg = g_fps_dbg;
+  hipLaunchKernelGGL(k_fps_voxels_reg, dim3(2), dim3(1024), 0, s, a);
+  COOCC_LAUNCH_CHECK("k_fps_voxels_reg");
+  return COOCC_OK;
+}
+
+extern "C" int coocc_fps_voxels_pair_dev(const int32_t* lin0, int which0, int32_t* idx0, void* ws0, const int32_t* lin1, int which1,
+                                         int32_t* idx1, void* ws1, size_t ws_bytes_each, int n_cap, const int32_t* cnt, int small_m,
+                                         int X, int Y, int Z, int m, void* stream) {
+  COOCC_CHECK_ARG(X > 0 && Y > 0 && Z > 0 && n_cap > 0 && cnt && (unsigned)which0 < 2u && (unsigned)which1 < 2u && small_m >= m,
+                  "fps_voxels_pair_dev: bad args");
+  if (!coocc_fps_voxels_pair_ok(n_cap, X, Y, Z)) return 2;
+  hipStream_t s = as_stream(stream);
+  FpsPrep o0, o1;
+  int rc = fps_prepare(lin0, n_cap, X, Y, Z, m, idx0, ws0, ws_bytes_each, s, &o0, cnt, which0, small_m);
+  if (rc != COOCC_OK) return rc;
+  rc = fps_prepare(lin1, n_cap, X, Y, Z, m, idx1, ws1, ws_bytes_each, s, &o1, cnt, which1, small_m);
+  if (rc != COOCC_OK || m == 0) return rc;
+  FpsRegArgs a = {};
+  a.p[0] = FpsRegProblem{lin0, (const FpsCell*)ws0, idx0, 0, 0, 0, 0, which0};
+  a.p[1] = FpsRegProblem{lin1, (const FpsCell*)ws1, idx1, 0, 0, 0, 0, which1};
+  a.m = m; a.Y = Y; a.Z = Z; a.NBY = o0.NBY; a.NBZ = o0.NBZ; a.NB = (int)o0.NB; a.dbg = g_fps_dbg;
+  a.cnt = cnt; a.small_m = small_m; a.d2max = fps_d2max(X, Y, Z);
   hipLaunchKernelGGL(k_fps_voxels_reg, dim3(2), dim3(1024), 0, s, a);
   COOCC_LAUNCH_CHECK("k_fps_voxels_reg");
   return COOCC_OK;
@@ -719,7 +768,9 @@
 
 __global__ __launch_bounds__(256) void k_ball_query_vox(int m, float min_r2, float max_r2, int R, int nsample, int X, int Y, int Z,
                                                          const int32_t* __restrict__ centre_ord, const int32_t* __restrict__ lin_q,
-                                                         const int32_t* __restrict__ map_q, int32_t* __restrict__ idx_all) {
+                                                         const int32_t* __restrict__ map_q, int32_t* __restrict__ idx_all,
+                                                         const int32_t* __restrict__ dcnt, int small_m) {
+  if (dcnt && dev_counts_small(dcnt, small_m)) return;
   const int lane = threadIdx.x & 63;
   const int c = blockIdx.x * 4 + (threadIdx.x >> 6);
   if (c >= m) return;
@@ -755,25 +806,38 @@
   for (int l = cnt + lane; l < nsample; l += 64) idx[l] = first;
 }
 
-extern "C" int coocc_ball_query_voxels(int m, float min_radius, float max_radius, int nsample, int X, int Y, int Z,
-                                       const int32_t* centre_ord, const int32_t* lin_q, const int32_t* map_q, int32_t* idx,
-                                       void* stream) {
+static int ball_query_voxels(int m, float min_radius, float max_radius, int nsample, int X, int Y, int Z, const int32_t* centre_ord,
+                             const int32_t* lin_q, const int32_t* map_q, int32_t* idx, const int32_t* cnt, int small_m, void* stream) {
   COOCC_CHECK_ARG(m > 0 && nsample > 0 && X > 0 && Y > 0 && Z > 0 && centre_ord && lin_q && map_q && idx, "ball_query_voxels: bad args");
   COOCC_CHECK_ARG(max_radius >= 0.f && max_radius < 4096.f, "ball_query_voxels: bad radius");
   const float max_r2 = max_radius * max_radius;
   int R = (int)ceilf(max_radius);
   while (R > 0 && (float)(R * R) >= max_r2) --R;
   hipLaunchKernelGGL(k_ball_query_vox, dim3(cdiv(m, 4)), dim3(256), 0, as_stream(stream), m, min_radius * min_radius, max_r2, R,
-                     nsample, X, Y, Z, centre_ord, lin_q, map_q, idx);
+                     nsample, X, Y, Z, centre_ord, lin_q, map_q, idx, cnt, small_m);
   COOCC_LAUNCH_CHECK("k_ball_query_vox");
   return COOCC_OK;
+}
+
+extern "C" int coocc_ball_query_voxels(int m, float min_radius, float max_radius, int nsample, int X, int Y, int Z,
+                                       const int32_t* centre_ord, const int32_t* lin_q, const int32_t* map_q, int32_t* idx,
+                                       void* stream) {
+  return ball_query_voxels(m, min_radius, max_radius, nsample, X, Y, Z, centre_ord, lin_q, map_q, idx, nullptr, 0, stream);
+}
+
+extern "C" int coocc_ball_query_voxels_dev(int m, float min_radius, float max_radius, int nsample, int X, int Y, int Z,
+                                           const int32_t* centre_ord, const int32_t* lin_q, const int32_t* map_q, int32_t* idx,
+                                           const int32_t* cnt, int small_m, void* stream) {
+  COOCC_CHECK_ARG(cnt, "ball_query_voxels_dev: null counts");
+  return ball_query_voxels(m, min_radius, max_radius, nsample, X, Y, Z, centre_ord, lin_q, map_q, idx, cnt, small_m, stream);
 }
 
 template <int K>
 __global__ __launch_bounds__(256) void k_knn_topk_vox(int nq, int X, int Y, int Z, const int32_t* __restrict__ rep_ord,
                                                        const int32_t* __restrict__ lin_q, const int32_t* __restrict__ map_k,
                                                        const uint32_t* __restrict__ offsets, int noff, float* __restrict__ val,
-                                                       int32_t* __restrict__ idx) {
+                                                       int32_t* __restrict__ idx, const int32_t* __restrict__ cnt, int small_m) {
+  if (cnt && dev_counts_small(cnt, small_m)) return;
   const int lane = threadIdx.x & 63;
   const int r = blockIdx.x * 4 + (threadIdx.x >> 6);
   if (r >= nq) return;
@@ -807,7 +871,12 @@
 template <int K>
 __global__ __launch_bounds__(256) void k_knn_topk_unresolved(int nq, int nk, const float* __restrict__ q,
                                                               const float* __restrict__ key, float* __restrict__ val,
-                                                              int32_t* __restrict__ idx) {
+                                                              int32_t* __restrict__ idx, const int32_t* __restrict__ cnt, int which,
+                                                              int small_m) {
+  if (cnt) {
+    if (dev_counts_small(cnt, small_m)) return;
+    nk = cnt[which];
+  }
   const int lane = threadIdx.x & 63;
   const int r = blockIdx.x * 4 + (threadIdx.x >> 6);
   if (r >= nq || idx[(size_t)r * K] != -2) return;
@@ -844,34 +913,53 @@
 template <int K>
 static void launch_topk_vox(int nq, int nk, int X, int Y, int Z, const int32_t* rep_ord, const int32_t* lin_q, const int32_t* map_k,
                             const uint32_t* offsets, int noff, const float* q, const float* key, float* val, int32_t* idx,
-                            hipStream_t s) {
-  hipLaunchKernelGGL(k_knn_topk_vox<K>, dim3(cdiv(nq, 4)), dim3(256), 0, s, nq, X, Y, Z, rep_ord, lin_q, map_k, offsets, noff, val, idx);
-  hipLaunchKernelGGL(k_knn_topk_unresolved<K>, dim3(cdiv(nq, 4)), dim3(256), 0, s, nq, nk, q, key, val, idx);
-}
-
-extern "C" int coocc_knn_topk_voxels(int nq, int nk, int K, int X, int Y, int Z, const int32_t* rep_ord, const int32_t* lin_q,
-                                     const int32_t* map_k, const uint32_t* offsets, int noff, const float* q, const float* key,
-                                     float* val, int32_t* idx, void* stream) {
+                            const int32_t* cnt, int which, int small_m, hipStream_t s) {
+  hipLaunchKernelGGL(k_knn_topk_vox<K>, dim3(cdiv(nq, 4)), dim3(256), 0, s, nq, X, Y, Z, rep_ord, lin_q, map_k, offsets, noff, val, idx,
+                     cnt, small_m);
+  hipLaunchKernelGGL(k_knn_topk_unresolved<K>, dim3(cdiv(nq, 4)), dim3(256), 0, s, nq, nk, q, key, val, idx, cnt, which, small_m);
+}
+
+static int knn_topk_voxels(int nq, int nk, int K, int X, int Y, int Z, const int32_t* rep_ord, const int32_t* lin_q,
+                           const int32_t* map_k, const uint32_t* offsets, int noff, const float* q, const float* key, float* val,
+                           int32_t* idx, const int32_t* cnt, int which, int small_m, void* stream) {
   COOCC_CHECK_ARG(nq > 0 && nk > 0 && X > 0 && Y > 0 && Z > 0 && rep_ord && lin_q && map_k && offsets && noff > 0 && q && key &&
                       val && idx, "knn_topk_voxels: bad args");
   COOCC_CHECK_ARG(K >= 1 && K <= 8 && K <= nk, "knn_topk_voxels: need 1 <= K <= min(8, nk)");
   hipStream_t s = as_stream(stream);
   switch (K) {
-    case 1: launch_topk_vox<1>(nq, nk, X, Y, Z, rep_ord, lin_q, map_k, offsets, noff, q, key, val, idx, s); break;
-    case 2: launch_topk_vox<2>(nq, nk, X, Y, Z, rep_ord, lin_q, map_k, offsets, noff, q, key, val, idx, s); break;
-    case 3: launch_topk_vox<3>(nq, nk, X, Y, Z, rep_ord, lin_q, map_k, offsets, noff, q, key, val, idx, s); break;
-    case 4: launch_topk_vox<4>(nq, nk, X, Y, Z, rep_ord, lin_q, map_k, offsets, noff, q, key, val, idx, s); break;
-    case 5: launch_topk_vox<5>(nq, nk, X, Y, Z, rep_ord, lin_q, map_k, offsets, noff, q, key, val, idx, s); break;
-    case 6: launch_topk_vox<6>(nq, nk, X, Y, Z, rep_ord, lin_q, map_k, offsets, noff, q, key, val, idx, s); break;
-    case 7: launch_topk_vox<7>(nq, nk, X, Y, Z, rep_ord, lin_q, map_k, offsets, noff, q, key, val, idx, s); break;
-    default: launch_topk_vox<8>(nq, nk, X, Y, Z, rep_ord, lin_q, map_k, offsets, noff, q, key, val, idx, s); break;
+    case 1: launch_topk_vox<1>(nq, nk, X, Y, Z, rep_ord, lin_q, map_k, offsets, noff, q, key, val, idx, cnt, which, small_m, s); break;
+    case 2: launch_topk_vox<2>(nq, nk, X, Y, Z, rep_ord, lin_q, map_k, offsets, noff, q, key, val, idx, cnt, which, small_m, s); break;
+    case 3: launch_topk_vox<3>(nq, nk, X, Y, Z, rep_ord, lin_q, map_k, offsets, noff, q, key, val, idx, cnt, which, small_m, s); break;
+    case 4: launch_topk_vox<4>(nq, nk, X, Y, Z, rep_ord, lin_q, map_k, offsets, noff, q, key, val, idx, cnt, which, small_m, s); break;
+    case 5: launch_topk_vox<5>(nq, nk, X, Y, Z, rep_ord, lin_q, map_k, offsets, noff, q, key, val, idx, cnt, which, small_m, s); break;
+    case 6: launch_topk_vox<6>(nq, nk, X, Y, Z, rep_ord, lin_q, map_k, offsets, noff, q, key, val, idx, cnt, which, small_m, s); break;
+    case 7: launch_topk_vox<7>(nq, nk, X, Y, Z, rep_ord, lin_q, map_k, offsets, noff, q, key, val, idx, cnt, which, small_m, s); break;
+    default: launch_topk_vox<8>(nq, nk, X, Y, Z, rep_ord, lin_q, map_k, offsets, noff, q, key, val, idx, cnt, which, small_m, s); break;
   }
   COOCC_LAUNCH_CHECK("k_knn_topk_vox");
   return COOCC_OK;
 }
 
+extern "C" int coocc_knn_topk_voxels(int nq, int nk, int K, int X, int Y, int Z, const int32_t* rep_ord, const int32_t* lin_q,
+                                     const int32_t* map_k, const uint32_t* offsets, int noff, const float* q, const float* key,
+                                     float* val, int32_t* idx, void* stream) {
+  return knn_topk_voxels(nq, nk, K, X, Y, Z, rep_ord, lin_q, map_k, offsets, noff, q, key, val, idx, nullptr, 0, 0, stream);
+}
+
+extern "C" int coocc_knn_topk_voxels_dev(int nq, int K, int X, int Y, int Z, const int32_t* rep_ord, const int32_t* lin_q,
+                                         const int32_t* map_k, const uint32_t* offsets, int noff, const float* q, const float* key,
+                                         float* val, int32_t* idx, const int32_t* cnt, int which, int small_m, void* stream) {
+  COOCC_CHECK_ARG(cnt && (unsigned)which < 2u && small_m >= K, "knn_topk_voxels_dev: bad counts");
+  return knn_topk_voxels(nq, small_m + 1, K, X, Y, Z, rep_ord, lin_q, map_k, offsets, noff, q, key, val, idx, cnt, which, small_m, stream);
+}
+
 __global__ void k_assign_winner(int nc, int K, int ns, int nq, float thresh, const float* __restrict__ val,
-                                const int32_t* __restrict__ group, int32_t* __restrict__ winner) {
+                                const int32_t* __restrict__ group, int32_t* __restrict__ winner, const int32_t* __restrict__ cnt,
+                                int which, int small_m) {
+  if (cnt) {
+    if (dev_counts_small(cnt, small_m)) return;
+    nq = cnt[which];
+  }
   int i = blockIdx.x * blockDim.x + threadIdx.x;
   if (i >= nc * ns) return;
   int c = i / ns;
@@ -882,7 +970,12 @@
 }
 
 __global__ void k_assign_lookup(int K, int nq, const int32_t* __restrict__ nn,
-                                const int32_t* __restrict__ winner, int32_t* __restrict__ out) {
+                                const int32_t* __restrict__ winner, int32_t* __restrict__ out, const int32_t* __restrict__ cnt,
+                                int which, int small_m) {
+  if (cnt) {
+    if (dev_counts_small(cnt, small_m)) return;
+    nq = cnt[which];
+  }
   int i = blockIdx.x * blockDim.x + threadIdx.x;
   if (i >= K * nq) return;
   int k = i / nq;
@@ -890,17 +983,29 @@
   out[i] = w >= 0 ? nn[w * K + k] : -1;
 }
 
-extern "C" int coocc_knn_assign(int nc, int K, int ns, int nq, float dist_thresh, const float* val,
-                                const int32_t* nn, const int32_t* group, int32_t* winner, int32_t* out,
-                                void* stream) {
+static int knn_assign(int nc, int K, int ns, int nq, float dist_thresh, const float* val, const int32_t* nn, const int32_t* group,
+                      int32_t* winner, int32_t* out, const int32_t* cnt, int which, int small_m, void* stream) {
   COOCC_CHECK_ARG(val && nn && group && winner && out && nc > 0 && K > 0 && ns > 0 && nq > 0, "knn_assign: bad args");
   hipStream_t s = as_stream(stream);
   COOCC_HIP(hipMemsetAsync(winner, 0xFF, sizeof(int32_t) * (size_t)K * nq, s));
   hipLaunchKernelGGL(k_assign_winner, dim3(cdiv((long long)nc * ns, 256)), dim3(256), 0, s, nc, K, ns, nq,
-                     dist_thresh, val, group, winner);
-  hipLaunchKernelGGL(k_assign_lookup, dim3(cdiv((long long)K * nq, 256)), dim3(256), 0, s, K, nq, nn, winner, out);
+                     dist_thresh, val, group, winner, cnt, which, small_m);
+  hipLaunchKernelGGL(k_assign_lookup, dim3(cdiv((long long)K * nq, 256)), dim3(256), 0, s, K, nq, nn, winner, out, cnt, which, small_m);
   COOCC_LAUNCH_CHECK("knn_assign");
   return COOCC_OK;
+}
+
+extern "C" int coocc_knn_assign(int nc, int K, int ns, int nq, float dist_thresh, const float* val,
+                                const int32_t* nn, const int32_t* group, int32_t* winner, int32_t* out,
+                                void* stream) {
+  return knn_assign(nc, K, ns, nq, dist_thresh, val, nn, group, winner, out, nullptr, 0, 0, stream);
+}
+
+extern "C" int coocc_knn_assign_dev(int nc, int K, int ns, int nq_cap, float dist_thresh, const float* val, const int32_t* nn,
+                                    const int32_t* group, int32_t* winner, int32_t* out, const int32_t* cnt, int which, int small_m,
+                                    void* stream) {
+  COOCC_CHECK_ARG(cnt && (unsigned)which < 2u, "knn_assign_dev: bad counts");
+  return knn_assign(nc, K, ns, nq_cap, dist_thresh, val, nn, group, winner, out, cnt, which, small_m, stream);
 }
 
 __global__ void k_knn_threshold(int nq, float thresh, const float* __restrict__ val,
@@ -918,7 +1023,14 @@
 }
 
 __global__ void k_index_rows(const int32_t* __restrict__ base, int nbase, const int32_t* __restrict__ sel, int n,
-                             int32_t* __restrict__ rows) {
+                             int32_t* __restrict__ rows, const int32_t* __restrict__ cnt, int which_base, int which_n, int k,
+                             int small_m) {
+  if (cnt) {
+    if (dev_counts_small(cnt, small_m)) return;
+    nbase = cnt[which_base];
+    n = cnt[which_n];
+    sel += (size_t)k * n;
+  }
   int i = blockIdx.x * blockDim.x + threadIdx.x;
   if (i >= n) return;
   int s = sel[i];
@@ -930,7 +1042,18 @@
                                     void* stream) {
   COOCC_CHECK_ARG(base && sel && rows && nbase > 0 && n >= 0, "index_rows: bad args");
   if (n == 0) return COOCC_OK;
-  hipLaunchKernelGGL(k_index_rows, dim3(cdiv(n, 256)), dim3(256), 0, as_stream(stream), base, nbase, sel, n, rows);
+  hipLaunchKernelGGL(k_index_rows, dim3(cdiv(n, 256)), dim3(256), 0, as_stream(stream), base, nbase, sel, n, rows, (const int32_t*)nullptr, 0,
+                     0, 0, 0);
   COOCC_LAUNCH_CHECK("k_index_rows");
   return COOCC_OK;
 }
+
+extern "C" int coocc_index_rows_i32_dev(const int32_t* base, int which_base, const int32_t* sel, int k, int which_n, int n_cap,
+                                        int32_t* rows, const int32_t* cnt, int small_m, void* stream) {
+  COOCC_CHECK_ARG(base && sel && rows && cnt && n_cap > 0 && k >= 0 && (unsigned)which_base < 2u && (unsigned)which_n < 2u,
+                  "index_rows_dev: bad args");
+  hipLaunchKernelGGL(k_index_rows, dim3(cdiv(n_cap, 256)), dim3(256), 0, as_stream(stream), base, 0, sel, 0, rows, cnt, which_base, which_n, k,
+                     small_m);
+  COOCC_LAUNCH_CHECK("k_index_rows");
+  return COOCC_OK;
+}
diff --git a/co_occ_amd/csrc/layout.hip b/co_occ_amd/csrc/layout.hip
--- a/co_occ_amd/csrc/layout.hip
+++ b/co_occ_amd/csrc/layout.hip
@@ -439,7 +439,12 @@
 }
 
 __global__ void k_lin_to_coords(const int32_t* __restrict__ lin, int n, int X, int Y, int Z,
-                                float* __restrict__ xyz, int64_t* __restrict__ bxyz) {
+                                float* __restrict__ xyz, int64_t* __restrict__ bxyz, const int32_t* __restrict__ cnt, int which,
+                                int small_m) {
+  if (cnt) {
+    if (cnt[0] <= small_m || cnt[1] <= small_m) return;
+    n = min(n, cnt[which]);
+  }
   int i = blockIdx.x * blockDim.x + threadIdx.x;
   if (i >= n) return;
   int l = lin[i];
@@ -454,7 +459,17 @@
                                    void* stream) {
   COOCC_CHECK_ARG(lin && n >= 0 && X > 0 && Y > 0 && Z > 0, "lin_to_coords: bad args");
   if (n == 0) return COOCC_OK;
-  hipLaunchKernelGGL(k_lin_to_coords, dim3(cdiv(n, 256)), dim3(256), 0, as_stream(stream), lin, n, X, Y, Z, xyz, bxyz);
+  hipLaunchKernelGGL(k_lin_to_coords, dim3(cdiv(n, 256)), dim3(256), 0, as_stream(stream), lin, n, X, Y, Z, xyz, bxyz,
+                     (const int32_t*)nullptr, 0, 0);
+  COOCC_LAUNCH_CHECK("k_lin_to_coords");
+  return COOCC_OK;
+}
+
+extern "C" int coocc_lin_to_coords_dev(const int32_t* lin, int n_cap, const int32_t* cnt, int which, int small_m, int X, int Y, int Z,
+                                       float* xyz, void* stream) {
+  COOCC_CHECK_ARG(lin && xyz && cnt && n_cap > 0 && (unsigned)which < 2u && X > 0 && Y > 0 && Z > 0, "lin_to_coords_dev: bad args");
+  hipLaunchKernelGGL(k_lin_to_coords, dim3(cdiv(n_cap, 256)), dim3(256), 0, as_stream(stream), lin, n_cap, X, Y, Z, xyz, (int64_t*)nullptr,
+                     cnt, which, small_m);
   COOCC_LAUNCH_CHECK("k_lin_to_coords");
   return COOCC_OK;
 }
diff --git a/co_occ_amd/csrc/search.hip b/co_occ_amd/csrc/search.hip
--- a/co_occ_amd/csrc/search.hip
+++ b/co_occ_amd/csrc/search.hip
@@ -1,10 +1,13 @@
 #include <stdlib.h>
 #include <string.h>
 
+#include <atomic>
+
 #include "common.h"
 
 __global__ __launch_bounds__(256) void k_gather_xyz(const float* __restrict__ xyz, const int32_t* __restrict__ idx, int m,
-                                                     float* __restrict__ out) {
+                                                     float* __restrict__ out, const int32_t* __restrict__ cnt, int small_m) {
+  if (cnt && (cnt[0] <= small_m || cnt[1] <= small_m)) return;
   const int i = blockIdx.x * blockDim.x + threadIdx.x;
   if (i >= m) return;
   const int s = idx[i];
@@ -60,6 +63,68 @@
     if (rc__ != COOCC_OK) return rc__; \
   } while (0)
 
+static std::atomic<int> g_oneshot{-1};
+static int oneshot_setting() {
+  int v = g_oneshot.load(std::memory_order_relaxed);
+  if (v < 0) {
+    const char* e = getenv("COOCC_SEARCH_ONESHOT");
+    v = !(e && e[0] == '0');
+    int expect = -1;
+    if (!g_oneshot.compare_exchange_strong(expect, v)) v = expect;
+  }
+  return v;
+}
+extern "C" int coocc_fuser_search_oneshot(int on) {
+  const int prev = oneshot_setting();
+  if (on >= 0) g_oneshot.store(on ? 1 : 0);
+  return prev;
+}
+
+static int32_t* pinned_counts() {
+  static thread_local int32_t* p = nullptr;
+  if (!p && hipHostMalloc((void**)&p, 8, hipHostMallocDefault) != hipSuccess) p = nullptr;
+  return p;
+}
+
+static int search_enqueue_dev(const coocc_search_desc* d, const SearchWs& w, int V, void* stream, int sdiag) {
+  const int K = d->K, m = d->fps_num, X = d->X, Y = d->Y, Z = d->Z;
+  const int32_t* cnt = d->counts;
+  int32_t* lin_img = d->lin;
+  int32_t* lin_pts = d->lin + V;
+  float* xyz_img = w.xyz;
+  float* xyz_pts = w.xyz + (size_t)V * 3;
+  int32_t* map_img = w.maps;
+  int32_t* map_pts = w.maps + V;
+  SRC(coocc_lin_to_coords_dev(lin_img, V, cnt, 0, m, X, Y, Z, xyz_img, stream));
+  SRC(coocc_lin_to_coords_dev(lin_pts, V, cnt, 1, m, X, Y, Z, xyz_pts, stream));
+  SRC(coocc_voxel_index_map_dev(lin_img, V, cnt, V, map_img, stream));
+  SRC(coocc_voxel_index_map_dev(lin_pts, V, cnt + 1, V, map_pts, stream));
+  if (!(sdiag & 1)) {
+    const int rc = coocc_fps_voxels_pair_dev(lin_pts, 1, w.rep[0], w.fps[0], lin_img, 0, w.rep[1], w.fps[1], w.fps_bytes, V, cnt, m, X, Y, Z, m,
+                                             stream);
+    if (rc == 2) return coocc_set_error(COOCC_EINVAL, "fuser_search: the paired FPS refused a grid it had accepted");
+    SRC(rc);
+  }
+  auto direction = [&](int dd, const int32_t* lin_q, int wq, const float* xyz_q, const int32_t* map_q, int wk, const float* xyz_k,
+                       const int32_t* map_k, int32_t* near) -> int {
+    if (sdiag & 2) return COOCC_OK;
+    hipLaunchKernelGGL(k_gather_xyz, dim3(cdiv(m, 256)), dim3(256), 0, as_stream(stream), xyz_q, w.rep[dd], m, w.rep_xyz[dd], cnt, m);
+    COOCC_LAUNCH_CHECK("k_gather_xyz");
+    SRC(coocc_knn_topk_voxels_dev(m, K, X, Y, Z, w.rep[dd], lin_q, map_k, d->offsets, d->noff, w.rep_xyz[dd], xyz_k, w.val[dd], w.nn[dd], cnt,
+                                  wk, m, stream));
+    SRC(coocc_ball_query_voxels_dev(m, 0.f, d->radius, d->max_cluster, X, Y, Z, w.rep[dd], lin_q, map_q, w.group[dd], cnt, m, stream));
+    SRC(coocc_knn_assign_dev(m, K, d->max_cluster, V, d->dist_thresh, w.val[dd], w.nn[dd], w.group[dd], w.winner[dd], near, cnt, wq, m, stream));
+    return COOCC_OK;
+  };
+  SRC(direction(1, lin_img, 0, xyz_img, map_img, 1, xyz_pts, map_pts, d->near_pts));
+  for (int k = 0; k < K && !(sdiag & 2); ++k)
+    SRC(coocc_index_rows_i32_dev(K == 1 ? lin_pts : lin_img, K == 1 ? 1 : 0, d->near_pts, k, 0, V, d->rows_p + (size_t)k * V, cnt, m, stream));
+  SRC(direction(0, lin_pts, 1, xyz_pts, map_pts, 0, xyz_img, map_img, d->near_img));
+  for (int k = 0; k < K && !(sdiag & 2); ++k)
+    SRC(coocc_index_rows_i32_dev(lin_img, 0, d->near_img, k, 1, V, d->rows + (size_t)k * V, cnt, m, stream));
+  return COOCC_OK;
+}
+
 extern "C" int coocc_fuser_search(coocc_search_desc* d, void* stream, void* side_stream) {
   COOCC_CHECK_ARG(d && d->cat4 && d->pts && d->lin && d->counts && d->rows && d->rows_p && d->near_img && d->near_pts && d->ws &&
                       d->offsets && d->counts_host, "fuser_search: null pointer");
@@ -77,6 +142,35 @@
   SRC(coocc_fuser_prepare_rows(d->cat4, 1, 4 * C, d->pts, d->pts_rows, d->pts_stride, d->cat4, w.flags, w.flags + V, 1, C, V, stream));
   SRC(coocc_compact_flags(w.flags, V, lin_img, d->counts, w.cws, (size_t)(V / 1024 + 2) * 4, stream));
   SRC(coocc_compact_flags(w.flags + V, V, lin_pts, d->counts + 1, w.cws + (V / 1024 + 2), (size_t)(V / 1024 + 2) * 4, stream));
+  if (oneshot_setting() && d->fps_num >= K && coocc_fps_voxels_pair_ok(V, d->X, d->Y, d->Z)) {
+    const bool read = !((sdiag & 4) && d->counts_host[0] > 0);
+    volatile int32_t* pin = read ? pinned_counts() : nullptr;
+    if (read && !pin) return coocc_set_error(COOCC_ENOMEM, "fuser_search: no pinned host memory for the voxel counts");
+    hipEvent_t got = nullptr;
+    if (read) {
+      static const bool fence = [] { const char* e = getenv("COOCC_SEARCH_COUNT_FENCE"); return e && e[0] == '1'; }();
+      pin[0] = pin[1] = -1;
+      COOCC_HIP(hipMemcpyAsync((void*)pin, d->counts, 8, hipMemcpyDeviceToHost, s0));
+      COOCC_HIP(hipEventCreateWithFlags(&got, hipEventBlockingSync | hipEventDisableTiming | (fence ? 0u : hipEventDisableSystemFence)));
+      if (hipEventRecord(got, s0) != hipSuccess) {
+        (void)hipEventDestroy(got);
+        return coocc_set_error(COOCC_EHIP, "fuser_search: recording the count event failed");
+      }
+    }
+    const int rc = search_enqueue_dev(d, w, V, stream, sdiag);
+    if (read) {
+      const hipError_t e2 = hipEventSynchronize(got);
+      (void)hipEventDestroy(got);
+      if (e2 != hipSuccess) return coocc_set_error(COOCC_EHIP, "fuser_search: waiting for the voxel counts failed: %s", hipGetErrorString(e2));
+      if (pin[0] < 0 || pin[1] < 0) {
+        COOCC_HIP(hipStreamSynchronize(s0));
+        if (pin[0] < 0 || pin[1] < 0) return coocc_set_error(COOCC_EHIP, "fuser_search: the voxel counts did not reach the host");
+      }
+      d->counts_host[0] = pin[0]; d->counts_host[1] = pin[1];
+    }
+    if (rc != COOCC_OK) return rc;
+    return (d->counts_host[0] <= d->fps_num || d->counts_host[1] <= d->fps_num) ? COOCC_SEARCH_SMALL : COOCC_OK;
+  }
   if (!((sdiag & 4) && d->counts_host[0] > 0)) COOCC_HIP(hipMemcpyAsync(d->counts_host, d->counts, 8, hipMemcpyDeviceToHost, s0));
   if (!((sdiag & 4) && d->counts_host[0] > 0)) {
     static const bool fence = [] { const char* e = getenv("COOCC_SEARCH_COUNT_FENCE"); return e && e[0] == '1'; }();
@@ -137,7 +231,8 @@
                        const float* xyz_k, const int32_t* map_k, int32_t* near) -> int {
     if (sdiag & 2) return COOCC_OK;
     if (!paired) SRC(coocc_fps_voxels(lin_q, Q, d->X, d->Y, d->Z, d->fps_num, w.rep[dd], w.fps[dd], w.fps_bytes, st));
-    hipLaunchKernelGGL(k_gather_xyz, dim3(cdiv(d->fps_num, 256)), dim3(256), 0, as_stream(st), xyz_q, w.rep[dd], d->fps_num, w.rep_xyz[dd]);
+    hipLaunchKernelGGL(k_gather_xyz, dim3(cdiv(d->fps_num, 256)), dim3(256), 0, as_stream(st), xyz_q, w.rep[dd], d->fps_num, w.rep_xyz[dd],
+                       (const int32_t*)nullptr, 0);
     COOCC_LAUNCH_CHECK("k_gather_xyz");
     SRC(coocc_knn_topk_voxels(d->fps_num, Nk, K, d->X, d->Y, d->Z, w.rep[dd], lin_q, map_k, d->offsets, d->noff, w.rep_xyz[dd], xyz_k,
                               w.val[dd], w.nn[dd], st));
diff --git a/include/coocc_hip.h b/include/coocc_hip.h
--- a/include/coocc_hip.h
+++ b/include/coocc_hip.h
@@ -82,6 +82,25 @@
 } coocc_search_desc;
 size_t coocc_fuser_search_ws(const coocc_search_desc* d);
 int coocc_fuser_search(coocc_search_desc* d, void* stream, void* side_stream);
+int coocc_fuser_search_oneshot(int on);
+
+int coocc_lin_to_coords_dev(const int32_t* lin, int n_cap, const int32_t* cnt, int which, int small_m, int X, int Y, int Z,
+                            float* xyz, void* stream);
+int coocc_fps_voxels_pair_ok(int n, int X, int Y, int Z);
+int coocc_fps_voxels_pair_dev(const int32_t* lin0, int which0, int32_t* idx0, void* ws0, const int32_t* lin1, int which1,
+                              int32_t* idx1, void* ws1, size_t ws_bytes_each, int n_cap, const int32_t* cnt, int small_m,
+                              int X, int Y, int Z, int m, void* stream);
+int coocc_knn_topk_voxels_dev(int nq, int K, int X, int Y, int Z, const int32_t* rep_ord, const int32_t* lin_q,
+                              const int32_t* map_k, const uint32_t* offsets, int noff, const float* q, const float* key,
+                              float* val, int32_t* idx, const int32_t* cnt, int which, int small_m, void* stream);
+int coocc_ball_query_voxels_dev(int m, float min_radius, float max_radius, int nsample, int X, int Y, int Z,
+                                const int32_t* centre_ord, const int32_t* lin_q, const int32_t* map_q, int32_t* idx,
+                                const int32_t* cnt, int small_m, void* stream);
+int coocc_knn_assign_dev(int nc, int K, int ns, int nq_cap, float dist_thresh, const float* val, const int32_t* nn,
+                         const int32_t* group, int32_t* winner, int32_t* out, const int32_t* cnt, int which, int small_m,
+                         void* stream);
+int coocc_index_rows_i32_dev(const int32_t* base, int which_base, const int32_t* sel, int k, int which_n, int n_cap,
+                             int32_t* rows, const int32_t* cnt, int small_m, void* stream);
 
 int coocc_voxel_index_map(const int32_t* lin, int n, int nvox, int32_t* map, void* stream);
 int coocc_voxel_index_map_dev(const int32_t* lin, int n_cap, const int32_t* n_dev, int nvox, int32_t* map, void* stream);
```
